# nsirons/DL-unet

Measured on AMD Instinct MI355X. Metric: 572x572 tiles/sec fwd+bwd, higher is better.
Workload: dtype f32; 1 GPU; batch=8/GPU 572x572x1 fwd+bwd+SGD fp32, 64-base-ch U-Net (BASELINE configs[1]); arithmetic=fp32 MFMA; 3x3 fwd/dgrad/wgrad as Winograd F(2x2,3x3), global_batch=8, tile=572, parallelism=dp1, loss=unweighted BCE-with-logits

## Files before the change

dl-unet_amd/_hip.py:

```python
import ctypes as C
import os
import subprocess

import torch

_HERE = os.path.dirname(os.path.abspath(__file__))
_SO = os.environ.get("UNET_SO") or os.path.join(_HERE, "libunet_hip.so")
_lib = None

N_PARAMS = 46
MAX_CLASSES = 16

vp = C.c_void_p
_SIGS = {
    "unet_last_error": (C.c_char_p, []),
    "unet_abi_version": (C.c_int, []),
    "unet_set_math": (C.c_int, [C.c_int]),
    "unet_get_math": (C.c_int, []),
    "unet_set_lds_dma": (C.c_int, [C.c_int]),
    "unet_set_grad_scale": (C.c_int, [vp, C.c_float]),
    "unet_set_overlap": (C.c_int, [C.c_int]),
    "unet_dp_unique_id": (C.c_int, [vp]),
    "unet_dp_init": (C.c_int, [vp, C.c_int, C.c_int, vp]),
    "unet_dp_destroy": (C.c_int, [vp]),
    "unet_dp_world": (C.c_int, [vp]),
    "unet_dp_rccl_version": (C.c_int, []),
    "unet_dp_allreduce": (C.c_int, [vp, vp, C.c_size_t, vp]),
    "unet_dp_broadcast": (C.c_int, [vp, vp, C.c_size_t, C.c_int, vp]),
    "unet_dp_join": (C.c_int, [vp, vp]),
    "unet_create": (C.c_int, [C.POINTER(vp), vp]),
    "unet_create_classes": (C.c_int, [C.POINTER(vp), vp, C.c_int]),
    "unet_n_classes": (C.c_int, [vp]),
    "unet_destroy": (C.c_int, [vp]),
    "unet_output_size": (C.c_int, [C.c_int, C.POINTER(C.c_int)]),
    "unet_param_count": (C.c_int, [vp, C.c_int, C.POINTER(C.c_size_t)]),
    "unet_workspace_bytes": (C.c_size_t, [vp, C.c_int, C.c_int, C.c_int]),
    "unet_forward": (C.c_int, [vp, vp, vp, vp, C.c_int, C.c_int, vp, C.c_size_t, C.c_int, vp]),
    "unet_backward": (C.c_int, [vp, vp, vp, vp, vp, C.c_size_t, vp]),
    "unet_backward_stages": (C.c_int, []),
    "unet_backward_stage": (C.c_int, [vp, C.c_int, vp, vp, vp, vp, C.c_size_t, vp]),
    "unet_backward_stage_params": (C.c_int, [C.c_int, C.POINTER(C.c_int), C.c_int]),
    "unet_backward_input": (C.c_int, [vp, vp, vp, vp, C.c_size_t, vp]),
    "unet_flops": (C.c_double, [vp, C.c_int, C.c_int, C.c_int]),
    "unet_activation_bytes": (C.c_int, [vp]),
    "unet_debug_buffer": (C.c_int, [vp, C.c_int, C.c_int, C.c_int, C.c_char_p, C.POINTER(C.c_size_t), C.POINTER(C.c_int), C.POINTER(C.c_int)]),
    "unet_profile_enable": (C.c_int, [C.c_int]),
    "unet_profile_select": (C.c_int, [C.c_uint]),
    "unet_profile_reset": (C.c_int, []),
    "unet_profile_read": (C.c_int, [C.c_int, C.POINTER(C.c_double), C.POINTER(C.c_long), C.POINTER(C.c_double),
                                    C.POINTER(C.c_double), C.POINTER(C.c_double)]),
    "unet_profile_dump": (C.c_int, [C.c_char_p]),
    "unet_bce_scratch_bytes": (C.c_size_t, [C.c_size_t]),
    "unet_bce_logits": (C.c_int, [vp, vp, vp, C.c_long, C.c_long, C.c_long, C.c_long, C.c_int, C.c_int, C.c_int,
                                  vp, vp, C.c_float, vp, vp]),
    "unet_bce_step_scratch_bytes": (C.c_size_t, [C.c_size_t]),
    "unet_bce_step": (C.c_int, [vp, C.c_long, C.c_long, C.c_long, vp, vp, C.c_long, C.c_long, C.c_long, C.c_long, C.c_int, C.c_int, C.c_int,
                                vp, vp, C.c_float, vp, vp, vp]),
    "unet_onehot2": (C.c_int, [vp, vp, C.c_int, C.c_int, C.c_int, vp]),
    "unet_argmax2": (C.c_int, [vp, C.c_long, C.c_long, C.c_long, vp, C.c_int, C.c_int, C.c_int, vp]),
    "unet_softmax_ce_scratch_bytes": (C.c_size_t, [C.c_size_t]),
    "unet_softmax_ce_step": (C.c_int, [vp, C.c_long, C.c_long, C.c_long, C.c_int, vp, vp, C.c_long, C.c_long, C.c_long, C.c_int, C.c_int,
                                       C.c_int, vp, vp, C.c_float, vp, vp, vp, vp]),
    "unet_argmaxk": (C.c_int, [vp, C.c_long, C.c_long, C.c_long, C.c_int, vp, C.c_int, C.c_int, C.c_int, vp]),
    "unet_sgd_momentum": (C.c_int, [vp, vp, vp, C.POINTER(C.c_size_t), C.c_int, C.c_float, C.c_float, C.c_int, vp]),
    "unet_minmax": (C.c_int, [vp, C.c_int, C.c_size_t, vp, vp]),
    "unet_mirror_pad": (C.c_int, [vp, C.c_int, C.c_int, C.c_int, vp, vp, vp]),
    "unet_tile_gather": (C.c_int, [vp, C.c_int, C.c_int, C.c_int, vp, C.c_int, C.c_int, C.c_int, C.c_int, C.c_int, C.c_long,
                                   C.c_int, vp, vp]),
    "unet_tile_stitch": (C.c_int, [vp, C.c_int, C.c_int, C.c_int, C.c_int, C.c_int, C.c_long, C.c_int, C.c_int, C.c_int, C.c_int,
                                   vp, vp, vp]),
    "unet_tile_stitch_k": (C.c_int, [vp, C.c_int, C.c_int, C.c_int, C.c_int, C.c_int, C.c_int, C.c_long, C.c_int, C.c_int, C.c_int,
                                     C.c_int, vp, vp, vp]),
    "unet_eval_masks": (C.c_int, [vp, C.c_long, C.c_long, C.c_long, C.c_int, vp, vp, C.c_int, C.c_int, vp, vp]),
    "unet_eval_confusion": (C.c_int, [vp, C.c_long, C.c_long, C.c_long, C.c_int, C.c_int, vp, vp, C.c_int, C.c_int, vp, vp, vp]),
    "unet_class_balance": (C.c_int, [vp, C.c_int, C.c_int, C.c_int, vp, vp, vp]),
    "unet_weighted_map_scratch_bytes": (C.c_size_t, [C.c_int, C.c_int, C.c_int]),
    "unet_weighted_map": (C.c_int, [vp, C.c_int, C.c_int, C.c_int, C.c_int, C.c_float, C.c_float, vp, vp, vp, vp, vp]),
    "unet_gaussian_filter": (C.c_int, [vp, C.c_int, C.c_int, C.c_int, vp, C.c_int, C.c_float, vp, vp, vp]),
    "unet_warp_bilinear": (C.c_int, [vp, vp, vp, C.c_int, C.c_int, C.c_int, vp, vp]),
    "unet_rotate_scratch_bytes": (C.c_size_t, [C.c_int, C.c_int]),
    "unet_reflect_rotate_crop": (C.c_int, [vp, C.c_int, C.c_int, C.c_int, C.c_int, C.POINTER(C.c_float), C.c_int, vp, vp, vp]),
    "unet_conv3x3_scratch_bytes": (C.c_size_t, [C.c_int, C.c_int]),
    "unet_conv3x3_fwd": (C.c_int, [vp, C.c_int, C.c_int, C.c_int, C.c_int, vp, C.c_int, C.c_int, C.c_int, C.c_int,
                                   vp, vp, C.c_int, C.c_int, vp, vp, vp]),
    "unet_conv3x3_bwd_scratch_bytes": (C.c_size_t, [C.c_int] * 5),
    "unet_conv3x3_bwd": (C.c_int, [vp, C.c_int, C.c_int, C.c_int, C.c_int, vp, C.c_int, C.c_int, C.c_int, C.c_int,
                                   vp, C.c_int, vp, vp, vp, vp, vp, vp, vp, vp, vp, vp]),
    "unet_maxpool2_fwd": (C.c_int, [vp, vp, C.c_int, C.c_int, C.c_int, C.c_int, vp]),
    "unet_maxpool2_bwd": (C.c_int, [vp, vp, vp, C.c_int, C.c_int, C.c_int, C.c_int, vp]),
    "unet_upconv2_scratch_bytes": (C.c_size_t, [C.c_int] * 5),
    "unet_upconv2_fwd": (C.c_int, [vp, C.c_int, C.c_int, C.c_int, C.c_int, vp, vp, C.c_int, vp, vp, vp]),
    "unet_upconv2_bwd": (C.c_int, [vp, C.c_int, C.c_int, C.c_int, C.c_int, vp, C.c_int, vp, vp, vp, vp, vp, vp, vp]),
    "unet_head1x1_fwd": (C.c_int, [vp, C.c_int, C.c_int, C.c_int, C.c_int, vp, vp, vp, vp]),
    "unet_head1x1_bwd_scratch_bytes": (C.c_size_t, [C.c_int] * 4),
    "unet_head1x1_bwd": (C.c_int, [vp, C.c_int, C.c_int, C.c_int, C.c_int, vp, vp, vp, vp, vp, vp, vp]),
    "unet_head1xk_fwd": (C.c_int, [vp, C.c_int, C.c_int, C.c_int, C.c_int, C.c_int, vp, vp, vp, vp]),
    "unet_head1xk_bwd_scratch_bytes": (C.c_size_t, [C.c_int] * 5),
    "unet_head1xk_bwd": (C.c_int, [vp, C.c_int, C.c_int, C.c_int, C.c_int, C.c_int, vp, vp, vp, vp, vp, vp, vp]),
    "unet_conv1ch_fwd": (C.c_int, [vp, C.c_int, C.c_int, vp, vp, C.c_int, vp, vp]),
    "unet_conv1ch_bwd_scratch_bytes": (C.c_size_t, [C.c_int] * 3),
    "unet_conv1ch_bwd": (C.c_int, [vp, C.c_int, C.c_int, C.c_int, vp, vp, vp, vp, vp]),
}
EXPORTS = tuple(_SIGS.keys())


class UnetConfig(C.Structure):
    _fields_ = [("base_ch", C.c_int), ("device", C.c_int), ("math", C.c_int)]


def build(force=False):
    csrc = os.path.join(_HERE, "csrc")
    if force and os.path.exists(_SO):
        os.remove(_SO)
    subprocess.check_call(["make", "-s", "-C", csrc, "-j4"])
    return _SO


def lib():
    global _lib
    if _lib is None:
        if not os.path.exists(_SO):
            raise RuntimeError(
                "libunet_hip.so is not built (%s). Run `python -c 'import __graft_entry__ as g; g.build()'` "
                "or `make -C dl-unet_amd/csrc`. There is no CPU fallback for the HIP path." % _SO)
        L = C.CDLL(_SO)
        for name, (res, args) in _SIGS.items():
            fn = getattr(L, name)
            fn.restype = res
            fn.argtypes = args
        _lib = L
    return _lib


def check(rc, what=""):
    if rc != 0:
        msg = lib().unet_last_error().decode("utf-8", "replace")
        raise RuntimeError("%s failed (rc=%d): %s" % (what or "libunet_hip", rc, msg))


def ptr(t):
    if t is None:
        return None
    if not t.is_cuda:
        raise RuntimeError("the HIP path needs tensors on a HIP device (got %s); there is no CPU fallback" % t.device)
    return C.c_void_p(t.data_ptr())


def stream(device=None):
    return C.c_void_p(torch.cuda.current_stream(device).cuda_stream)


def run(name, device, *args):
    with torch.cuda.device(device):
        check(getattr(lib(), name)(*args, stream(device)), name)


def ptr_table(tensors):
    arr = (C.c_void_p * len(tensors))()
    for i, t in enumerate(tensors):
        if not t.is_cuda:
            raise RuntimeError("parameter %d is on %s; move the module to a HIP device" % (i, t.device))
        arr[i] = t.data_ptr()
    return arr


class Handle:

    def __init__(self, base_ch=64, device=0, math=-1, n_classes=2):
        self._h = C.c_void_p()
        cfg = UnetConfig(base_ch, device, math)
        if n_classes == 2:
            check(lib().unet_create(C.byref(self._h), C.byref(cfg)), "unet_create")
        else:
            check(lib().unet_create_classes(C.byref(self._h), C.byref(cfg), int(n_classes)), "unet_create_classes")
        self.base_ch = base_ch
        self.device = device
        self.math = math
        self.n_classes = n_classes

    def __del__(self):
        try:
            if self._h:
                lib().unet_destroy(self._h)
                self._h = None
        except Exception:
            pass

    @property
    def h(self):
        return self._h

    def workspace_bytes(self, B, S, training):
        n = lib().unet_workspace_bytes(self._h, B, S, int(training))
        if n == 0:
            check(-1, "unet_workspace_bytes")
        return n

    def buffer_view(self, ws, B, S, training, name):
        off, e, c = C.c_size_t(), C.c_int(), C.c_int()
        check(lib().unet_debug_buffer(self._h, B, S, int(training), name.encode(), C.byref(off), C.byref(e), C.byref(c)),
              "unet_debug_buffer")
        n = B * e.value * e.value * c.value
        eb = 4 if name == "xin" else lib().unet_activation_bytes(self._h)
        return ws[off.value:off.value + eb * n].view(torch.bfloat16 if eb == 2 else torch.float32).view(B, e.value, e.value, c.value)

    def flops(self, B, S, backward):
        return lib().unet_flops(self._h, B, S, int(backward))
```

dl-unet_amd/csrc/common.hpp:

```cpp
#pragma once
#include <hip/hip_runtime.h>
#include <cstddef>
#include <cstdint>

namespace unet {

typedef float f32x4 __attribute__((ext_vector_type(4)));
typedef float f32x16 __attribute__((ext_vector_type(16)));

void set_error(const char *fmt, ...);
const float *zero_page();

#define HIP_TRY(expr)                                                              \
    do {                                                                           \
        hipError_t e_ = (expr);                                                    \
        if (e_ != hipSuccess) {                                                    \
            unet::set_error("%s failed: %s", #expr, hipGetErrorString(e_));        \
            return (int)e_;                                                        \
        }                                                                          \
    } while (0)

#define ARG_CHECK(cond, ...)                                                       \
    do {                                                                           \
        if (!(cond)) { unet::set_error(__VA_ARGS__); return -2; }                  \
    } while (0)

enum { PK_IGEMM = 0, PK_WGRAD = 1, PK_REDUCE = 2, PK_WINO = 3, PK_STENCIL = 4, PK_ELEMWISE = 5, PK_COMM = 6, PK_KINDS = 7 };
void prof_scope(const char *row);
void prof_begin(int kind, const char *tag, hipStream_t st, double alg_flops, double exec_flops, double alg_bytes);
void prof_end(hipStream_t st);
bool prof_active();
struct ProfScope {
    explicit ProfScope(const char *row) { prof_scope(row); }
    ~ProfScope() { prof_scope(nullptr); }
};

template <class F>
static inline int profiled(int kind, const char *tag, hipStream_t st, double alg_flops, double exec_flops, double alg_bytes, F launches)
{
    prof_begin(kind, tag, st, alg_flops, exec_flops, alg_bytes);
    launches();
    prof_end(st);
    HIP_TRY(hipGetLastError());
    return 0;
}
template <auto Kern, class Arg>
static inline int launch_profiled(int grid, int threads, int lds, hipStream_t st, int kind, const char *tag, double alg_flops,
                                  double exec_flops, double alg_bytes, const Arg &arg)
{
    static bool attr_done[64] = {false};
    int dev = 0;
    if (hipGetDevice(&dev) != hipSuccess || dev < 0 || dev >= 64) { set_error("bad device"); return -2; }
    if (!attr_done[dev]) {
        HIP_TRY(hipFuncSetAttribute((const void *)Kern, hipFuncAttributeMaxDynamicSharedMemorySize, lds));
        attr_done[dev] = true;
    }
    return profiled(kind, tag, st, alg_flops, exec_flops, alg_bytes,
                    [&] { hipLaunchKernelGGL(Kern, dim3(grid), dim3(threads), lds, st, arg); });
}
int device_cu_count();

static inline int cdiv(int a, int b) { return (a + b - 1) / b; }
static inline size_t align_up(size_t v, size_t a) { return (v + a - 1) / a * a; }

constexpr size_t LIMIT_31BIT = 0x7FFFFFFFull;
static inline size_t tensor_elems(int NB, int H, int W, int C) { return (size_t)NB * H * W * C; }
static inline size_t tensor_bytes(int NB, int H, int W, int C, size_t es) { return tensor_elems(NB, H, W, C) * es; }
static inline bool fits_buffer(size_t bytes) { return bytes < LIMIT_31BIT; }

struct FastDiv { unsigned long long mul; int shift; };
static inline FastDiv make_fastdiv(unsigned d)
{
    int s = 0;
    while ((1ull << s) < d) ++s;
    FastDiv f;
    f.shift = 32 + s;
    f.mul = ((1ull << f.shift) + d - 1) / d;
    return f;
}

struct GSrc {
    const float *p;
    int H, W, C;
    int c0, nch;
    int pad;
};

struct IgemmP {
    GSrc src[2];
    int nsrc;
    const float *wt;
    int Kd, ldw;
    int T, TX;
    int stride, oy0, ox0;
    int NB, OH, OW, M, Nn;
    float *dst;
    int DH, DW, DC, dn0;
    int scatter;
    int dwy0, dwx0;
    int rw0, rw1;
    int cout;
    const float *bias;
    int relu;
    const float *mask;
    const float *add;
    const float *zeros;
    int buf_bytes[3];
    float *pool_dst;
    const float *wino_u;
    int math;
    int mtiles, ntiles;
    FastDiv d_ohw, d_ow;
};
int launch_igemm(IgemmP p, hipStream_t st);
static inline int igemm_source_bytes(const IgemmP &p, size_t es, int out[2])
{
    int big = -1;
    for (int i = 0; i < 2; ++i) {
        const size_t b = i < p.nsrc ? tensor_bytes(p.NB, p.src[i].H, p.src[i].W, p.src[i].C, es) : 0;
        if (!fits_buffer(b) && big < 0) big = i;
        out[i] = (int)b;
    }
    return big;
}
bool wino_applicable(const IgemmP &p);
bool wino_fuses_pool(const IgemmP &p);
size_t wino_u_floats(int Kc, int Nn);
int wino_transform_ref(const float *w_oihw, int I, int dgrad, int n0, int Nn, int k0, int Kc, float *U, hipStream_t st);
int get_math_mode();
void set_math_mode(int m);
static inline int op_es() { return get_math_mode() == 2 ? 2 : 4; }
int get_lds_dma_mode();
void set_lds_dma_mode(int m);
double igemm_alg_flops(const IgemmP &p);
double igemm_alg_bytes(const IgemmP &p);

struct WgradP {
    const float *X; int XH, XW, XC, xc0, xpad;
    const float *Y; int YH, YW, YC, yc0;
    int NB, stride, TY, TX, oy0, ox0;
    int ywin0, ywin1, xwin0, xwin1;
    int Ci, Cj;
    float *out; long si, sj, st;
    float *db;
    int db_on_x;
    float *slab; size_t slab_bytes;
    const float *zeros;
    int math;
};
size_t wgrad_slab_need(const WgradP &p);
double wgrad_alg_flops(const WgradP &p);
double wgrad_alg_bytes(const WgradP &p);
int launch_wgrad(WgradP p, hipStream_t st);

int pack_conv_fwd(const float *w_oihw, void *wt, int K, int C1, int C2, int es, hipStream_t st);
int pack_conv_dgrad(const float *w_oihw, void *wt, int K, int C, int es, hipStream_t st);
int pack_upconv_fwd(const float *w_iohw, void *wt, int Ci, int Co, int es, hipStream_t st);
int pack_upconv_dgrad(const float *w_iohw, void *wt, int Ci, int Co, int es, hipStream_t st);
int bias_grad(const void *dz, size_t M, int K, float *db, float *scratch, int es, hipStream_t st);
size_t bias_grad_scratch_bytes(size_t M, int K);

int conv1ch_fwd(const float *x, int B, int S, const float *w, const float *bias, int K, void *y, int es, hipStream_t st);
int conv1ch_bwd(const float *x, int B, int S, int K, const void *dz, float *dw, float *db, float *scratch, int es, hipStream_t st);
int conv1ch_dgrad(const void *dz, int B, int S, int K, const float *w, float *dx, int es, hipStream_t st);
int head1x1_fwd(const void *x, int B, int H, int W, int C, const float *w, const float *bias, float *logits, int es, hipStream_t st);
int head1x1_bwd(const void *x, int B, int H, int W, int C, const float *w, const float *dlogits, float dl_scale, void *dz, float *dw,
                float *db, float *scratch, int es, hipStream_t st);
int headk_fwd(const void *x, int B, int H, int W, int C, int K, const float *w, const float *bias, float *logits, int es, hipStream_t st);
int headk_bwd(const void *x, int B, int H, int W, int C, int K, const float *w, const float *dlogits, float dl_scale, void *dz, float *dw,
              float *db, float *scratch, int es, hipStream_t st);
size_t headk_bwd_scratch_bytes(int B, int H, int W, int C, int K);
static inline int class_pad(int K) { return K <= 2 ? 2 : K <= 4 ? 4 : K <= 8 ? 8 : 16; }
#define CLASS_DISPATCH(K, LAUNCH)                                                                                      \
    do {                                                                                                           \
        switch (unet::class_pad(K)) {                                                                              \
        case 2: { constexpr int KP_ = 2; LAUNCH; } break;                                                          \
        case 4: { constexpr int KP_ = 4; LAUNCH; } break;                                                          \
        case 8: { constexpr int KP_ = 8; LAUNCH; } break;                                                          \
        default: { constexpr int KP_ = 16; LAUNCH; } break;                                                        \
        }                                                                                                          \
    } while (0)
int maxpool2_fwd(const void *x, void *y, int B, int H, int W, int C, int es, hipStream_t st);
int maxpool2_bwd(const void *pre, const void *dy, void *dpre, int B, int H, int W, int C, int es, hipStream_t st);

}
```

dl-unet_amd/csrc/net.hip:

```cpp
#include "common.hpp"
#include "../../include/unet_hip.h"

#include <cstdarg>
#include <cstdio>
#include <cstdlib>
#include <cstring>
#include <mutex>
#include <utility>
#include <vector>

namespace unet {

static thread_local char g_err[512] = "";
void set_error(const char *fmt, ...)
{
    va_list ap;
    va_start(ap, fmt);
    vsnprintf(g_err, sizeof(g_err), fmt, ap);
    va_end(ap);
}

static float *g_zero[64] = {nullptr};
static std::mutex g_zero_mu;
const float *zero_page()
{
    int dev = 0;
    if (hipGetDevice(&dev) != hipSuccess || dev < 0 || dev >= 64) { set_error("zero_page: bad device"); return nullptr; }
    std::lock_guard<std::mutex> lk(g_zero_mu);
    if (!g_zero[dev]) {
        float *p = nullptr;
        if (hipMalloc((void **)&p, 4096) != hipSuccess || hipMemset(p, 0, 4096) != hipSuccess) {
            set_error("zero_page: hipMalloc failed");
            return nullptr;
        }
        g_zero[dev] = p;
    }
    return g_zero[dev];
}

enum { K_CONV1, K_CONV, K_CAT, K_UP, K_HEAD };
enum { T_A1, T_A2, T_T, T_U, T_D1, T_D2, N_TENSORS, T_NONE = N_TENSORS };
struct Layer {
    const char *name;
    int kind, level;
    int ci, co;
    int stage;
    int in, out;
};
static const Layer LAYERS[UNET_N_LAYERS] = {
    {"conv11c", K_CONV1, 0, -1, 0, 5, T_NONE, T_A1}, {"conv12c", K_CONV, 0, 0, 0, 5, T_A1, T_A2},
    {"conv21c", K_CONV, 1, 0, 1, 5, T_T, T_A1},      {"conv22c", K_CONV, 1, 1, 1, 5, T_A1, T_A2},
    {"conv31c", K_CONV, 2, 1, 2, 5, T_T, T_A1},      {"conv32c", K_CONV, 2, 2, 2, 5, T_A1, T_A2},
    {"conv41c", K_CONV, 3, 2, 3, 5, T_T, T_A1},      {"conv42c", K_CONV, 3, 3, 3, 5, T_A1, T_A2},
    {"conv51c", K_CONV, 4, 3, 4, 4, T_T, T_A1},      {"conv52c", K_CONV, 4, 4, 4, 4, T_A1, T_A2},
    {"upconv4", K_UP, 3, 4, 3, 3, T_A2, T_U}, {"conv41e", K_CAT, 3, 4, 3, 3, T_T, T_D1}, {"conv42e", K_CONV, 3, 3, 3, 3, T_D1, T_D2},
    {"upconv3", K_UP, 2, 3, 2, 2, T_D2, T_U}, {"conv31e", K_CAT, 2, 3, 2, 2, T_T, T_D1}, {"conv32e", K_CONV, 2, 2, 2, 2, T_D1, T_D2},
    {"upconv2", K_UP, 1, 2, 1, 1, T_D2, T_U}, {"conv21e", K_CAT, 1, 2, 1, 1, T_T, T_D1}, {"conv22e", K_CONV, 1, 1, 1, 1, T_D1, T_D2},
    {"upconv1", K_UP, 0, 1, 0, 0, T_D2, T_U}, {"conv11e", K_CAT, 0, 1, 0, 0, T_T, T_D1}, {"conv12e", K_CONV, 0, 0, 0, 0, T_D1, T_D2},
    {"finalconv", K_HEAD, 0, 0, -1, 0, T_D2, T_NONE}};
enum { C11C = 0, FINAL = UNET_N_LAYERS - 1 };
static const int N_STAGES = 6;
static const struct { const char *name; int levels; } TENSOR_NAME[N_TENSORS] = {{"a1", 5}, {"a2", 5}, {"t", 4}, {"u", 4}, {"d1", 4}, {"d2", 4}};

struct Act { size_t off = 0, g = 0; int e = 0, c = 0; };

struct Plan {
    int B = 0, S = 0, base = 0, So = 0, training = 0;
    int ncls = 2;
    int math = 3;
    int ch[5], pad[4];
    Act a1[5], a2[5], t[4], u[4], d1[4], d2[4];
    size_t g_ts[4];
    size_t wt_fwd[UNET_N_LAYERS], wt_bwd[UNET_N_LAYERS];
    size_t wu_fwd[UNET_N_LAYERS], wu_bwd[UNET_N_LAYERS];
    size_t slab = 0, slab_bytes = 0, small = 0, small_bytes = 0, xin = 0;
    size_t total = 0;
    const Act &act(int tensor, int l) const { const Act *const v[N_TENSORS] = {a1, a2, t, u, d1, d2}; return v[tensor][l]; }
    const Act &in(const Layer &L) const { return act(L.in, L.kind == K_CAT ? L.level : L.ci); }
    const Act &out(const Layer &L) const { return act(L.out, L.level); }
};

}

using namespace unet;

struct unet_dp;
int unet_dp_free(unet_dp *d);

struct unet_handle {
    int base_ch;
    int device;
    int math;
    int n_classes = 2;
    unet_dp *dp = nullptr;
    float grad_scale = 1.f;
    hipStream_t aux = nullptr;
    hipEvent_t ev_fork = nullptr, ev_join = nullptr;
    std::mutex mu;
    std::vector<std::pair<void *, Plan>> live;
    void remember(void *ws, const Plan &pl)
    {
        std::lock_guard<std::mutex> lk(mu);
        for (auto &e : live) if (e.first == ws) { e.second = pl; return; }
        if (live.size() >= 16) live.erase(live.begin());
        live.emplace_back(ws, pl);
    }
    bool lookup(void *ws, Plan &pl)
    {
        std::lock_guard<std::mutex> lk(mu);
        for (auto &e : live) if (e.first == ws) { pl = e.second; return true; }
        return false;
    }
};

unet_dp **unet_handle_dp_slot(unet_handle *h) { return &h->dp; }
int unet_handle_device(const unet_handle *h) { return h->device; }

namespace unet {

static thread_local int t_math = 3;
static thread_local int t_es = 4;
struct MathScope {
    int prev;
    explicit MathScope(int m) : prev(t_math) { t_math = m; t_es = m == 2 ? 2 : 4; }
    ~MathScope() { t_math = prev; t_es = prev == 2 ? 2 : 4; }
};
static inline float *adv(float *p, size_t elems) { return (float *)((char *)p + elems * t_es); }


static int layer_ci(int base, const Layer &L) { return L.ci < 0 ? 1 : base << L.ci; }
static int layer_co(int base, const Layer &L, int ncls) { return L.co < 0 ? ncls : base << L.co; }
static int layer_taps(const Layer &L) { return L.kind == K_UP ? 2 : L.kind == K_HEAD ? 1 : 3; }

static size_t layer_numel(int base, int layer, bool bias, int ncls = 2)
{
    const Layer &L = LAYERS[layer];
    const int k = layer_taps(L);
    return bias ? (size_t)layer_co(base, L, ncls) : (size_t)layer_ci(base, L) * layer_co(base, L, ncls) * k * k;
}

static size_t layer_wino_floats(int base, int layer)
{
    const Layer &L = LAYERS[layer];
    if (L.kind != K_CONV && L.kind != K_CAT) return 0;
    const int ci = layer_ci(base, L), co = layer_co(base, L, 2);
    const size_t fwd = wino_u_floats(ci, co);
    const size_t bwd = L.kind == K_CAT ? 2 * wino_u_floats(co, ci / 2) : wino_u_floats(co, ci);
    return fwd > bwd ? fwd : bwd;
}

struct WLayer {
    const float *w; int O, I;
    bool dgrad;
    float *wt; int C1, C2;
    bool packed = false;
    int ensure_packed(hipStream_t st)
    {
        if (packed) return 0;
        packed = true;
        return dgrad ? pack_conv_dgrad(w, wt, O, I, t_es, st) : pack_conv_fwd(w, wt, O, C1, C2, t_es, st);
    }
};

static int with_wino(IgemmP &p, float *wu, WLayer &L, int n0, int k0, hipStream_t st)
{
    if (p.math != 3 || !wu || !wino_applicable(p)) return L.ensure_packed(st);
    int kc = 0;
    for (int i = 0; i < p.nsrc; ++i) kc += p.src[i].nch;
    int rc = wino_transform_ref(L.w, L.I, L.dgrad ? 1 : 0, n0, p.Nn, k0, kc, wu, st);
    if (rc) return rc;
    p.wino_u = wu;
    return 0;
}

static int check_size(int S)
{
    if (S < 60 + 16 * 8 || (S - 60) % 16 != 0 || ((S - 60) / 16) % 2 != 0) {
        set_error("input size %d is not 16L+60 with L even >= 8: the reference's crop_and_concat/torch.cat "
                  "raises on it (network.py:124-127)", S);
        return UNET_E_BADSIZE;
    }
    return 0;
}

struct RowScope : ProfScope {
    static const char *make(char (&buf)[40], int layer, const char *what) { snprintf(buf, sizeof(buf), "%s.%s", LAYERS[layer].name, what); return buf; }
    char buf[40];
    RowScope(int layer, const char *what) : ProfScope(make(buf, layer, what)) {}
};

static IgemmP conv_fwd_desc(const float *x1, int H1, int W1, int C1, int pad1, const float *x2, int C2,
                            int B, int H, int W, const float *wt, const float *bias, int K, int relu, float *y)
{
    IgemmP p{};
    p.nsrc = x2 ? 2 : 1;
    p.src[0] = GSrc{x1, H1, W1, C1, 0, C1, pad1};
    if (x2) p.src[1] = GSrc{x2, H, W, C2, 0, C2, 0};
    p.wt = wt; p.Kd = 9 * (C1 + C2);
    p.T = 9; p.TX = 3; p.stride = 1; p.oy0 = 0; p.ox0 = 0;
    p.NB = B; p.OH = H - 2; p.OW = W - 2; p.M = B * p.OH * p.OW; p.Nn = K;
    p.dst = y; p.DH = p.OH; p.DW = p.OW; p.DC = K; p.dn0 = 0;
    p.bias = bias; p.relu = relu;
    p.math = t_math;
    return p;
}

static int conv_fwd_launch(const float *x1, int H1, int C1, int pad1, const float *x2, int C2, int B, int H,
                           const float *w_oihw, float *wt, const float *bias, int K, int relu, float *y, hipStream_t st, float *wu = nullptr,
                           float *pool_dst = nullptr, bool *pool_fused = nullptr)
{
    const int Ho = H - 2;
    if (!x2) C2 = 0;
    WLayer L{w_oihw, K, C1 + C2, false, wt, C1, C2};
    int rc;
    int w0 = pad1 - 2; if (w0 < 0) w0 = 0;
    int w1 = pad1 + H1; if (w1 > Ho) w1 = Ho;
    static const double split_thr = [] { const char *e = getenv("UNET_SPLIT_THR"); return e ? atof(e) : 0.85; }();
    const bool split = x2 && pad1 > 0 && t_math != 2 && (double)(w1 - w0) * (w1 - w0) < split_thr * (double)Ho * Ho;
    if (!split) {
        IgemmP p = conv_fwd_desc(x1, H1, H1, C1, pad1, x2, C2, B, H, H, wt, bias, K, relu, y);
        if ((rc = with_wino(p, wu, L, 0, 0, st))) return rc;
        if (pool_dst && p.wino_u && wino_fuses_pool(p)) { p.pool_dst = pool_dst; *pool_fused = true; }
        return launch_igemm(p, st);
    }
    const int ldw = 9 * (C1 + C2);
    IgemmP a = conv_fwd_desc(x2, H, H, C2, 0, nullptr, 0, B, H, H, adv(wt, 9 * C1), bias, K, relu, y);
    a.ldw = ldw;
    if (relu) { a.rw0 = w0; a.rw1 = w1; }
    if ((rc = with_wino(a, wu, L, 0, C1, st))) return rc;
    if ((rc = launch_igemm(a, st))) return rc;
    IgemmP b = conv_fwd_desc(x1, H1, H1, C1, pad1, nullptr, 0, B, H, H, wt, nullptr, K, relu, y);
    b.ldw = ldw;
    b.OH = b.OW = w1 - w0; b.M = B * b.OH * b.OW; b.oy0 = b.ox0 = w0;
    b.scatter = 2; b.dwy0 = b.dwx0 = w0; b.DH = b.DW = Ho;
    b.add = y;
    if ((rc = with_wino(b, wu ? wu + wino_u_floats(C2, K) : nullptr, L, 0, 0, st))) return rc;
    return launch_igemm(b, st);
}

static IgemmP upconv_fwd_desc(const float *x, int B, int H, int W, int Ci, const float *wt, const float *bias, int Co, float *y)
{
    IgemmP u{};
    u.nsrc = 1; u.src[0] = GSrc{x, H, W, Ci, 0, Ci, 0};
    u.wt = wt; u.Kd = Ci;
    u.T = 1; u.TX = 1; u.stride = 1;
    u.NB = B; u.OH = H; u.OW = W; u.M = B * H * W; u.Nn = 4 * Co;
    u.dst = y; u.DH = 2 * H; u.DW = 2 * W; u.DC = Co; u.scatter = 1; u.cout = Co;
    u.bias = bias;
    u.math = t_math;
    return u;
}

static IgemmP upconv_dgrad_desc(const float *dy, int B, int H, int W, int Ci, const float *wt, int Co, float *dx, const float *mask)
{
    IgemmP d{};
    d.nsrc = 1; d.src[0] = GSrc{dy, 2 * H, 2 * W, Co, 0, Co, 0};
    d.wt = wt; d.Kd = 4 * Co;
    d.T = 4; d.TX = 2; d.stride = 2;
    d.NB = B; d.OH = H; d.OW = W; d.M = B * H * W; d.Nn = Ci;
    d.dst = dx; d.DH = H; d.DW = W; d.DC = Ci;
    d.mask = mask;
    d.math = t_math;
    return d;
}

static IgemmP conv_dgrad_desc(const float *dz, int Ho, int Wo, int K, int B, int OHW, int o0,
                              const float *wt_rows, int Nn, float *dx, const float *mask, const float *add)
{
    IgemmP p{};
    p.nsrc = 1;
    p.src[0] = GSrc{dz, Ho, Wo, K, 0, K, 2};
    p.wt = wt_rows; p.Kd = 9 * K;
    p.T = 9; p.TX = 3; p.stride = 1; p.oy0 = o0; p.ox0 = o0;
    p.NB = B; p.OH = OHW; p.OW = OHW; p.M = B * OHW * OHW; p.Nn = Nn;
    p.dst = dx; p.DH = OHW; p.DW = OHW; p.DC = Nn; p.dn0 = 0;
    p.mask = mask; p.add = add;
    p.math = t_math;
    return p;
}

static WgradP conv_wgrad_desc(const float *X, int XH, int XC, int xpad, const float *dz, int Ho, int K, int B,
                              float *dw, int Ctot, int c_off, float *slab, size_t slab_bytes, float *db = nullptr)
{
    WgradP p{};
    p.X = X; p.XH = XH; p.XW = XH; p.XC = XC; p.xc0 = 0; p.xpad = xpad;
    p.Y = dz; p.YH = Ho; p.YW = Ho; p.YC = K; p.yc0 = 0;
    p.NB = B; p.stride = 1; p.TY = 3; p.TX = 3; p.oy0 = 0; p.ox0 = 0;
    int w0 = xpad - 2; if (w0 < 0) w0 = 0;
    int w1 = xpad + XH; if (w1 > Ho) w1 = Ho;
    p.ywin0 = w0; p.ywin1 = w1; p.xwin0 = w0; p.xwin1 = w1;
    p.Ci = XC; p.Cj = K;
    p.out = dw ? dw + (size_t)c_off * 9 : nullptr; p.si = 9; p.sj = (long)Ctot * 9; p.st = 1;
    p.slab = slab; p.slab_bytes = slab_bytes; p.db = db;
    p.math = t_math;
    return p;
}

static WgradP upconv_wgrad_desc(const float *x, int H, int Ci, const float *dy, int Co, int B, float *dw,
                                float *slab, size_t slab_bytes, float *db = nullptr)
{
    WgradP p{};
    p.X = dy; p.XH = 2 * H; p.XW = 2 * H; p.XC = Co; p.xc0 = 0; p.xpad = 0;
    p.Y = x; p.YH = H; p.YW = H; p.YC = Ci; p.yc0 = 0;
    p.NB = B; p.stride = 2; p.TY = 2; p.TX = 2; p.oy0 = 0; p.ox0 = 0;
    p.ywin0 = 0; p.ywin1 = H; p.xwin0 = 0; p.xwin1 = H;
    p.Ci = Co; p.Cj = Ci;
    p.out = dw; p.si = 4; p.sj = (long)Co * 4; p.st = 1;
    p.slab = slab; p.slab_bytes = slab_bytes;
    p.db = db; p.db_on_x = db ? 1 : 0;
    p.math = t_math;
    return p;
}

static int conv_dgrad_launch(const float *dz, int Ho, int K, int B, const float *w_oihw, float *wt, float *wu, int H1, int C1, int pad1,
                             float *dx1, const float *mask1, const float *add1, int H, int C2, float *dx2, const float *mask2, hipStream_t st)
{
    WLayer L{w_oihw, K, C1 + C2, true, wt, 0, 0};
    int rc;
    if (dx1) {
        IgemmP d = conv_dgrad_desc(dz, Ho, Ho, K, B, H1, pad1, L.wt, C1, dx1, mask1, add1);
        if ((rc = with_wino(d, wu, L, 0, 0, st))) return rc;
        if ((rc = launch_igemm(d, st))) return rc;
    }
    if (dx2) {
        IgemmP d = conv_dgrad_desc(dz, Ho, Ho, K, B, H, 0, adv(L.wt, (size_t)C1 * 9 * K), C2, dx2, mask2, nullptr);
        if ((rc = with_wino(d, wu + wino_u_floats(K, C1), L, C1, 0, st))) return rc;
        if ((rc = launch_igemm(d, st))) return rc;
    }
    return 0;
}

struct WgradStream {
    unet_handle *h; hipStream_t main; bool overlap; bool used;
    hipError_t err = hipSuccess;
    hipStream_t get()
    {
        if (!overlap) return main;
        hipError_t e = hipEventRecord(h->ev_fork, main);
        if (e == hipSuccess) e = hipStreamWaitEvent(h->aux, h->ev_fork, 0);
        if (e != hipSuccess) { if (err == hipSuccess) err = e; overlap = false; return main; }
        used = true;
        return h->aux;
    }
    hipStream_t same() const { return overlap && used ? h->aux : main; }
    void join()
    {
        if (!used) return;
        hipError_t e = hipEventRecord(h->ev_join, h->aux);
        if (e == hipSuccess) e = hipStreamWaitEvent(main, h->ev_join, 0);
        if (e != hipSuccess) {
            (void)hipStreamSynchronize(h->aux);
            if (err == hipSuccess) err = e;
        }
        used = false;
    }
};

struct Ctx {
    unet_handle *h; const Plan &pl; char *base; hipStream_t st;
    const void *const *params; void *const *grads;
    WgradStream wst;
    Ctx(unet_handle *h, const Plan &pl, void *workspace, void *stream, const void *const *params, void *const *grads, bool overlap = false)
        : h(h), pl(pl), base((char *)workspace), st((hipStream_t)stream), params(params), grads(grads), wst{h, st, overlap, false} {}
    float *ws(size_t off) const { return base ? (float *)(base + off) : nullptr; }
    const float *w(int layer) const { return params ? (const float *)params[2 * layer] : nullptr; }
    const float *b(int layer) const { return params ? (const float *)params[2 * layer + 1] : nullptr; }
    float *dw(int layer) const { return grads ? (float *)grads[2 * layer] : nullptr; }
    float *db(int layer) const { return grads ? (float *)grads[2 * layer + 1] : nullptr; }
};

static int layer_wgrad(const Ctx &cx, int layer, WgradP w[2])
{
    const Plan &pl = cx.pl;
    const Layer &L = LAYERS[layer];
    if (L.kind == K_CONV1 || L.kind == K_HEAD) return 0;
    const Act &x = pl.in(L), &y = pl.out(L);
    const float *dz = cx.ws(y.g);
    float *dw = cx.dw(layer), *db = cx.db(layer), *slab = cx.ws(pl.slab);
    if (L.kind == K_UP) w[0] = upconv_wgrad_desc(cx.ws(x.off), x.e, x.c, dz, y.c, pl.B, dw, slab, pl.slab_bytes, db);
    if (L.kind == K_CONV) w[0] = conv_wgrad_desc(cx.ws(x.off), x.e, x.c, 0, dz, y.e, y.c, pl.B, dw, x.c, 0, slab, pl.slab_bytes, db);
    if (L.kind != K_CAT) return 1;
    const Act &u = pl.u[L.level];
    w[0] = conv_wgrad_desc(cx.ws(x.off), x.e, x.c, pl.pad[L.level], dz, y.e, y.c, pl.B, dw, x.c + u.c, 0, slab, pl.slab_bytes);
    w[1] = conv_wgrad_desc(cx.ws(u.off), u.e, u.c, 0, dz, y.e, y.c, pl.B, dw, x.c + u.c, x.c, slab, pl.slab_bytes, db);
    return 2;
}

static int make_plan(Plan &pl, int base, int B, int S, int training, int math, int ncls = 2)
{
    int rc = check_size(S);
    if (rc) return rc;
    if (B <= 0) { set_error("batch must be positive"); return UNET_E_BADARG; }
    pl = Plan();
    pl.B = B; pl.S = S; pl.base = base; pl.training = training; pl.math = math; pl.ncls = ncls;
    MathScope ms(math);
    for (int l = 0; l < 5; ++l) pl.ch[l] = base << l;
    Act *acts[26];
    int n = 0, cur = S;
    for (int l = 0; l < 5; ++l) {
        pl.a1[l].e = cur - 2; pl.a2[l].e = cur - 4;
        pl.a1[l].c = pl.a2[l].c = pl.ch[l];
        acts[n++] = &pl.a1[l]; acts[n++] = &pl.a2[l];
        if (l < 4) cur = pl.a2[l].e / 2;
    }
    int d = pl.a2[4].e;
    for (int l = 3; l >= 0; --l) {
        pl.t[l].e = pl.a2[l].e / 2;
        pl.u[l].e = 2 * d; pl.pad[l] = (pl.u[l].e - pl.t[l].e) / 2;
        if ((pl.u[l].e - pl.t[l].e) % 2) { set_error("internal: odd skip difference"); return UNET_E_BADSIZE; }
        pl.d1[l].e = pl.u[l].e - 2; pl.d2[l].e = pl.u[l].e - 4; d = pl.d2[l].e;
        pl.t[l].c = pl.u[l].c = pl.d1[l].c = pl.d2[l].c = pl.ch[l];
    }
    for (int l = 0; l < 4; ++l) { acts[n++] = &pl.t[l]; acts[n++] = &pl.u[l]; acts[n++] = &pl.d1[l]; acts[n++] = &pl.d2[l]; }
    pl.So = d;
    if (math == 2 && base % 64 != 0) { set_error("arithmetic mode 2 (bf16 tensors) needs base_ch %% 64 == 0 (got %d)", base); return UNET_E_UNSUPPORTED; }
    const size_t es = math == 2 ? 2 : 4;
    size_t off = 0;
    auto take_b = [&](size_t bytes) { size_t o = off; off = align_up(off + bytes, 256); return o; };
    auto take = [&](size_t elems) { return take_b(elems * es); };
    auto sq = [&](int e, int c) { return (size_t)B * e * e * c; };
    for (int i = 0; i < n; ++i) acts[i]->off = take(sq(acts[i]->e, acts[i]->c));
    for (int i = 0; i < UNET_N_LAYERS; ++i) pl.wt_fwd[i] = take(layer_numel(base, i, false, ncls));
    for (int i = 0; i < UNET_N_LAYERS; ++i) pl.wu_fwd[i] = take_b(math == 3 ? layer_wino_floats(base, i) * 4 : 0);
    if (training) {
        pl.xin = take_b((size_t)B * S * S * 4);
        for (int i = 0; i < UNET_N_LAYERS; ++i) pl.wt_bwd[i] = take(layer_numel(base, i, false, ncls));
        for (int i = 0; i < UNET_N_LAYERS; ++i) pl.wu_bwd[i] = take_b(math == 3 ? layer_wino_floats(base, i) * 4 : 0);
        for (int i = 0; i < n; ++i) {
            Act *a = acts[i];
            a->g = take(sq(a->e, a->c));
            if (a >= pl.t && a < pl.t + 4) pl.g_ts[a - pl.t] = take(sq(a->e, a->c));
        }
        size_t need = 0;
        const Ctx sizing(nullptr, pl, nullptr, nullptr, nullptr, nullptr);
        for (int i = 0; i < UNET_N_LAYERS; ++i) {
            WgradP w[2];
            const int nw = layer_wgrad(sizing, i, w);
            for (int j = 0; j < nw; ++j) { const size_t s = wgrad_slab_need(w[j]); if (s > need) need = s; }
        }
        pl.slab_bytes = need;
        pl.slab = take_b(need);
        size_t sm = 0;
        auto upds = [&](size_t s) { if (s > sm) sm = s; };
        for (int l = 0; l < 5; ++l) { upds(bias_grad_scratch_bytes(sq(pl.a1[l].e, 1), pl.ch[l])); upds(bias_grad_scratch_bytes(sq(pl.a2[l].e, 1), pl.ch[l])); }
        for (int l = 0; l < 4; ++l) { upds(bias_grad_scratch_bytes(sq(pl.u[l].e, 1), pl.ch[l])); upds(bias_grad_scratch_bytes(sq(pl.d1[l].e, 1), pl.ch[l])); }
        upds(unet_conv1ch_bwd_scratch_bytes(B, S, base));
        upds(headk_bwd_scratch_bytes(B, pl.So, pl.So, base, ncls));
        pl.small_bytes = sm;
        pl.small = take_b(sm + 4);
    }
    pl.total = off;
    return 0;
}

}

extern "C" {

const char *unet_last_error(void) { return g_err; }
int unet_abi_version(void) { return 4; }

int unet_set_math(int mode)
{
    ARG_CHECK(mode >= 0 && mode <= 3, "unet_set_math: mode must be 0 (fp32 MFMA), 1 (bf16x3), 2 (bf16) or 3 (fp32 Winograd)");
    set_math_mode(mode);
    return 0;
}
int unet_get_math(void) { return get_math_mode(); }

int unet_set_lds_dma(int mode)
{
    ARG_CHECK(mode == 0 || mode == 1, "unet_set_lds_dma: mode must be 0 (global_load_lds) or 1 (buffer descriptors when tensors fit)");
    set_lds_dma_mode(mode);
    return 0;
}

#define CHECK_DEVICE(h, what)                                                                                          \
    do {                                                                                                               \
        int cur_ = -1;                                                                                                 \
        HIP_TRY(hipGetDevice(&cur_));                                                                                  \
        ARG_CHECK(cur_ == (h)->device, what ": the handle belongs to device %d but device %d is current "               \
                  "(one process per GPU: hipSetDevice / torch.cuda.set_device first)", (h)->device, cur_);             \
    } while (0)

int unet_create(unet_handle **out, const unet_config *cfg) { return unet_create_classes(out, cfg, 2); }

int unet_create_classes(unet_handle **out, const unet_config *cfg, int n_classes)
{
    ARG_CHECK(out && cfg, "unet_create: null argument");
    ARG_CHECK(n_classes >= 2 && n_classes <= UNET_MAX_CLASSES, "unet_create_classes: n_classes %d unsupported (2..%d)", n_classes,
              UNET_MAX_CLASSES);
    ARG_CHECK(cfg->base_ch == 64 || cfg->base_ch == 32, "unet_create: base_ch %d unsupported (32 or 64)", cfg->base_ch);
    ARG_CHECK(cfg->math >= -1 && cfg->math <= 3, "unet_create: math %d unsupported (-1 = process default, 0..3)", cfg->math);
    int prev = -1;
    HIP_TRY(hipGetDevice(&prev));
    HIP_TRY(hipSetDevice(cfg->device));
    const bool ok = zero_page() != nullptr;
    HIP_TRY(hipSetDevice(prev));
    if (!ok) return UNET_E_BADARG;
    unet_handle *h = new unet_handle();
    h->base_ch = cfg->base_ch;
    h->device = cfg->device;
    h->math = cfg->math;
    h->n_classes = n_classes;
    *out = h;
    return 0;
}

int unet_n_classes(const unet_handle *h) { return h ? h->n_classes : 0; }

int unet_destroy(unet_handle *h)
{
    if (h && h->dp) (void)unet_dp_free(h->dp);
    if (h) {
        if (h->aux) { (void)hipStreamSynchronize(h->aux); (void)hipStreamDestroy(h->aux); }
        if (h->ev_fork) (void)hipEventDestroy(h->ev_fork);
        if (h->ev_join) (void)hipEventDestroy(h->ev_join);
    }
    delete h;
    return 0;
}

int unet_set_grad_scale(unet_handle *h, float scale)
{
    ARG_CHECK(h, "unet_set_grad_scale: null handle");
    ARG_CHECK(scale > 0.f && scale <= 1.f, "unet_set_grad_scale: scale must be in (0, 1] (1/world), got %g", (double)scale);
    h->grad_scale = scale;
    return 0;
}

static int g_overlap = [] { const char *e = getenv("UNET_OVERLAP"); return e ? atoi(e) : -1; }();
int unet_set_overlap(int on)
{
    ARG_CHECK(on >= -1 && on <= 1, "unet_set_overlap: -1 (per arithmetic mode), 0 or 1");
    g_overlap = on;
    return 0;
}

static int handle_math(const unet_handle *h) { return h->math >= 0 ? h->math : get_math_mode(); }

int unet_output_size(int S, int *out_size)
{
    int rc = check_size(S);
    if (rc) return rc;
    if (out_size) *out_size = S - 184;
    return 0;
}

int unet_param_count(const unet_handle *h, int idx, size_t *numel)
{
    ARG_CHECK(h && numel && idx >= 0 && idx < UNET_N_PARAMS, "unet_param_count: bad argument");
    *numel = layer_numel(h->base_ch, idx / 2, idx & 1, h->n_classes);
    return 0;
}

size_t unet_workspace_bytes(const unet_handle *h, int B, int S, int training)
{
    if (!h) { set_error("null handle"); return 0; }
    Plan pl;
    if (make_plan(pl, h->base_ch, B, S, training, handle_math(h), h->n_classes)) return 0;
    return pl.total;
}

double unet_flops(const unet_handle *h, int B, int S, int backward)
{
    if (!h) return 0.0;
    Plan pl;
    if (make_plan(pl, h->base_ch, B, S, 0, handle_math(h), h->n_classes)) return 0.0;
    double f = 0.0, f11c = 0.0, first = 0.0;
    for (int i = 0; i < UNET_N_LAYERS; ++i) {
        const Layer &L = LAYERS[i];
        const int k = layer_taps(L);
        const int eo = L.kind == K_UP || L.kind == K_HEAD ? pl.in(L).e : pl.out(L).e;
        const double a = 2.0 * B * (double)eo * eo * layer_ci(pl.base, L) * layer_co(pl.base, L, pl.ncls) * k * k;
        if (L.kind == K_CONV1) f11c = a;
        if (L.out == T_A1 || L.out == T_D1) first = a;
        else if (L.out == T_A2 || L.out == T_D2) f += first + a;
        else f += a;
    }
    return backward ? 3.0 * f - f11c : f;
}

static int pool_launch(const Ctx &cx, int l, bool bwd)
{
    char nm[40]; snprintf(nm, sizeof(nm), "pool%d.%s", l + 1, bwd ? "bwd" : "fwd");
    ProfScope ps(nm);
    const Act &a2 = cx.pl.a2[l], &t = cx.pl.t[l];
    return bwd ? maxpool2_bwd(cx.ws(a2.off), cx.ws(t.g), cx.ws(a2.g), cx.pl.B, a2.e, a2.e, a2.c, t_es, cx.st)
               : maxpool2_fwd(cx.ws(a2.off), cx.ws(t.off), cx.pl.B, a2.e, a2.e, a2.c, t_es, cx.st);
}

static int conv_forward(const Ctx &cx, int layer)
{
    const Plan &pl = cx.pl;
    const Layer &L = LAYERS[layer];
    const bool cat = L.kind == K_CAT, pools = L.out == T_A2 && L.level < 4;
    const Act &x1 = pl.in(L), &y = pl.out(L), *x2 = cat ? &pl.u[L.level] : nullptr;
    bool pool_fused = false;
    {
        RowScope rs(layer, "fwd");
        int rc = conv_fwd_launch(cx.ws(x1.off), x1.e, x1.c, cat ? pl.pad[L.level] : 0, cat ? cx.ws(x2->off) : nullptr, cat ? x2->c : 0, pl.B, y.e + 2,
                                 cx.w(layer), cx.ws(pl.wt_fwd[layer]), cx.b(layer), y.c, 1, cx.ws(y.off), cx.st, cx.ws(pl.wu_fwd[layer]),
                                 pools ? cx.ws(pl.t[L.level].off) : nullptr, &pool_fused);
        if (rc) return rc;
    }
    return pools && !pool_fused ? pool_launch(cx, L.level, false) : 0;
}

int unet_forward(unet_handle *h, const void *const *params, const void *x, void *logits, int B, int S,
                 void *workspace, size_t workspace_bytes, int training, void *stream)
{
    ARG_CHECK(h && params && x && logits && workspace, "unet_forward: null argument");
    CHECK_DEVICE(h, "unet_forward");
    Plan pl;
    int rc = make_plan(pl, h->base_ch, B, S, training, handle_math(h), h->n_classes);
    if (rc) return rc;
    MathScope ms(pl.math);
    ARG_CHECK(workspace_bytes >= pl.total, "unet_forward: workspace too small (%zu < %zu)", workspace_bytes, pl.total);
    ARG_CHECK(((uintptr_t)workspace & 255) == 0, "unet_forward: workspace must be 256-byte aligned");
    const Ctx cx(h, pl, workspace, stream, params, nullptr);
    hipStream_t st = cx.st;

    for (int i = UNET_N_LAYERS - 1; i >= 0; --i) {
        if (LAYERS[i].kind != K_UP) continue;
        RowScope rs(i, "fwd");
        if ((rc = pack_upconv_fwd(cx.w(i), cx.ws(pl.wt_fwd[i]), pl.ch[LAYERS[i].ci], pl.ch[LAYERS[i].co], t_es, st))) return rc;
    }

    for (int i = 0; i < UNET_N_LAYERS; ++i) {
        const Layer &L = LAYERS[i];
        switch (L.kind) {
        case K_CONV1: {
            RowScope rs(i, "fwd");
            if (training) HIP_TRY(hipMemcpyAsync(cx.ws(pl.xin), x, (size_t)B * S * S * sizeof(float), hipMemcpyDeviceToDevice, st));
            if ((rc = conv1ch_fwd((const float *)x, B, S, cx.w(i), cx.b(i), pl.ch[0], cx.ws(pl.a1[0].off), t_es, st))) return rc;
            break;
        }
        case K_CONV:
        case K_CAT:
            if ((rc = conv_forward(cx, i))) return rc;
            break;
        case K_UP: {
            RowScope rs(i, "fwd");
            const Act &in = pl.in(L), &u = pl.u[L.level];
            IgemmP p = upconv_fwd_desc(cx.ws(in.off), B, in.e, in.e, in.c, cx.ws(pl.wt_fwd[i]), cx.b(i), u.c, cx.ws(u.off));
            if ((rc = launch_igemm(p, st))) return rc;
            break;
        }
        case K_HEAD: {
            RowScope rs(i, "fwd");
            const Act &in = pl.in(L);
            if ((rc = headk_fwd(cx.ws(in.off), B, in.e, in.e, in.c, pl.ncls, cx.w(i), cx.b(i), (float *)logits, t_es, st))) return rc;
            break;
        }
        }
    }
    if (training) h->remember(workspace, pl);
    return 0;
}

int unet_activation_bytes(const unet_handle *h)
{
    if (!h) return 0;
    return handle_math(h) == 2 ? 2 : 4;
}

int unet_debug_buffer(const unet_handle *h, int B, int S, int training, const char *name,
                      size_t *offset, int *extent, int *channels)
{
    ARG_CHECK(h && name && offset && extent && channels, "unet_debug_buffer: null argument");
    Plan pl;
    int rc = make_plan(pl, h->base_ch, B, S, training, handle_math(h), h->n_classes);
    if (rc) return rc;
    char kind[16];
    const char *us = strrchr(name, '_');
    if (!strcmp(name, "xin")) { ARG_CHECK(training, "xin exists only with training=1"); *offset = pl.xin; *extent = S; *channels = 1; return 0; }
    ARG_CHECK(us && (size_t)(us - name) < sizeof(kind), "unet_debug_buffer: bad name %s", name);
    memcpy(kind, name, us - name); kind[us - name] = 0;
    const int l = atoi(us + 1);
    ARG_CHECK(l >= 0 && l < 5, "unet_debug_buffer: bad level in %s", name);
    const bool g = !strncmp(kind, "g_", 2);
    ARG_CHECK(!g || training, "gradient buffers exist only with training=1");
    const char *k = g ? kind + 2 : kind;
    const bool ts = g && !strcmp(k, "ts");
    int id = ts ? T_T : 0;
    while (!ts && id < N_TENSORS && strcmp(k, TENSOR_NAME[id].name)) ++id;
    ARG_CHECK(l < (id < N_TENSORS ? TENSOR_NAME[id].levels : 4), "unet_debug_buffer: bad level in %s", name);
    if (id == N_TENSORS) { set_error("unet_debug_buffer: unknown buffer %s", name); return UNET_E_BADARG; }
    const Act &a = pl.act(id, l);
    *offset = ts ? pl.g_ts[l] : g ? a.g : a.off; *extent = a.e; *channels = a.c;
    return 0;
}

int unet_backward_stages(void) { return N_STAGES; }

int unet_backward_stage_params(int stage, int *idx, int cap)
{
    int k = 0;
    for (int i = UNET_N_LAYERS - 1; i >= 0; --i)
        for (int b = 0; b < 2 && LAYERS[i].stage == stage; ++b, ++k)
            if (idx && k < cap) idx[k] = 2 * i + b;
    return k;
}

static int wgrad_backward(Ctx &cx, int layer)
{
    RowScope rs(layer, "wgrad");
    WgradP w[2];
    const int n = layer_wgrad(cx, layer, w);
    for (int j = 0; j < n; ++j) {
        int rc = launch_wgrad(w[j], j ? cx.wst.same() : cx.wst.get());
        if (rc) return rc;
    }
    return 0;
}

static int conv_backward(Ctx &cx, int layer)
{
    const Plan &pl = cx.pl;
    const Layer &L = LAYERS[layer];
    const Act &x = pl.in(L), &y = pl.out(L);
    const bool pooled = L.in == T_T;
    int rc;
    if ((rc = wgrad_backward(cx, layer))) return rc;
    {
        RowScope rs(layer, "dgrad");
        if ((rc = conv_dgrad_launch(cx.ws(y.g), y.e, y.c, pl.B, cx.w(layer), cx.ws(pl.wt_bwd[layer]), cx.ws(pl.wu_bwd[layer]), x.e, x.c, 0, cx.ws(x.g),
                                    pooled ? nullptr : cx.ws(x.off), pooled ? cx.ws(pl.g_ts[L.ci]) : nullptr, 0, 0, nullptr, nullptr, cx.st))) return rc;
    }
    return pooled ? pool_launch(cx, L.ci, true) : 0;
}

static int backward_stage_body(Ctx &cx, int stage, const void *dlogits)
{
    const Plan &pl = cx.pl;
    hipStream_t st = cx.st;
    const int B = pl.B;
    int rc;
    for (int i = UNET_N_LAYERS - 1; i >= 0; --i) {
        const Layer &L = LAYERS[i];
        if (L.stage != stage) continue;
        switch (L.kind) {
        case K_HEAD: {
            ARG_CHECK(dlogits, "unet_backward: null dlogits");
            RowScope rs(i, "bwd");
            const Act &x = pl.in(L);
            if ((rc = headk_bwd(cx.ws(x.off), B, x.e, x.e, x.c, pl.ncls, cx.w(i), (const float *)dlogits, cx.h->grad_scale, cx.ws(x.g),
                                cx.dw(i), cx.db(i), cx.ws(pl.small), t_es, st))) return rc;
            break;
        }
        case K_CONV:
            if ((rc = conv_backward(cx, i))) return rc;
            break;
        case K_CAT: {
            const int l = L.level;
            const Act &t = pl.t[l], &u = pl.u[l], &y = pl.d1[l];
            if ((rc = wgrad_backward(cx, i))) return rc;
            RowScope rs(i, "dgrad");
            if ((rc = conv_dgrad_launch(cx.ws(y.g), y.e, y.c, B, cx.w(i), cx.ws(pl.wt_bwd[i]), cx.ws(pl.wu_bwd[i]), t.e, t.c, pl.pad[l], cx.ws(pl.g_ts[l]), nullptr, nullptr,
                                        u.e, u.c, cx.ws(u.g), nullptr, st))) return rc;
            break;
        }
        case K_UP: {
            const Act &x = pl.in(L), &u = pl.u[L.level];
            if ((rc = wgrad_backward(cx, i))) return rc;
            RowScope rs(i, "dgrad");
            if ((rc = pack_upconv_dgrad(cx.w(i), cx.ws(pl.wt_bwd[i]), x.c, u.c, t_es, st))) return rc;
            IgemmP d = upconv_dgrad_desc(cx.ws(u.g), B, x.e, x.e, x.c, cx.ws(pl.wt_bwd[i]), u.c, cx.ws(x.g), cx.ws(x.off));
            if ((rc = launch_igemm(d, st))) return rc;
            break;
        }
        case K_CONV1: {
            RowScope rs(i, "wgrad");
            if ((rc = conv1ch_bwd(cx.ws(pl.xin), B, pl.S, pl.ch[0], cx.ws(pl.a1[0].g), cx.dw(i), cx.db(i), cx.ws(pl.small), t_es, st))) return rc;
            break;
        }
        }
    }
    return 0;
}

int unet_backward_stage(unet_handle *h, int stage, const void *const *params, const void *dlogits, void *const *grads,
                        void *workspace, size_t workspace_bytes, void *stream)
{
    ARG_CHECK(h && params && grads && workspace, "unet_backward: null argument");
    CHECK_DEVICE(h, "unet_backward");
    Plan pl;
    if (!h->lookup(workspace, pl)) {
        set_error("unet_backward: no training forward has been run on this workspace");
        return UNET_E_NOTREADY;
    }
    ARG_CHECK(workspace_bytes >= pl.total, "unet_backward: workspace too small");
    ARG_CHECK(stage >= 0 && stage < N_STAGES, "unet_backward: bad stage %d", stage);
    MathScope ms(pl.math);
    const bool overlap = (g_overlap < 0 ? (pl.math == 2 || pl.B <= 4) : g_overlap != 0) && !prof_active();
    if (overlap && !h->aux) {
        HIP_TRY(hipStreamCreateWithFlags(&h->aux, hipStreamNonBlocking));
        HIP_TRY(hipEventCreateWithFlags(&h->ev_fork, hipEventDisableTiming));
        HIP_TRY(hipEventCreateWithFlags(&h->ev_join, hipEventDisableTiming));
    }
    Ctx cx(h, pl, workspace, stream, params, grads, overlap);
    int rc = backward_stage_body(cx, stage, dlogits);
    cx.wst.join();
    if (rc == 0 && cx.wst.err != hipSuccess) {
        set_error("unet_backward: ordering the weight-gradient stream against the caller's failed: %s", hipGetErrorString(cx.wst.err));
        rc = (int)cx.wst.err;
    }
    return rc;
}

int unet_backward_input(unet_handle *h, const void *const *params, void *dx, void *workspace, size_t workspace_bytes, void *stream)
{
    ARG_CHECK(h && params && dx && workspace, "unet_backward_input: null argument");
    CHECK_DEVICE(h, "unet_backward_input");
    Plan pl;
    if (!h->lookup(workspace, pl)) {
        set_error("unet_backward_input: no training forward has been run on this workspace");
        return UNET_E_NOTREADY;
    }
    ARG_CHECK(workspace_bytes >= pl.total, "unet_backward_input: workspace too small");
    MathScope ms(pl.math);
    const Ctx cx(h, pl, workspace, stream, params, nullptr);
    RowScope rs(C11C, "dgrad");
    return conv1ch_dgrad(cx.ws(pl.a1[0].g), pl.B, pl.S, pl.ch[0], cx.w(C11C), (float *)dx, t_es, cx.st);
}

int unet_backward(unet_handle *h, const void *const *params, const void *dlogits, void *const *grads,
                  void *workspace, size_t workspace_bytes, void *stream)
{
    for (int s = 0; s < N_STAGES; ++s) {
        int rc = unet_backward_stage(h, s, params, dlogits, grads, workspace, workspace_bytes, stream);
        if (rc) return rc;
    }
    return 0;
}

static size_t conv_bwd_slab_bound(int B, int H, int C, int K)
{
    size_t need = 0;
    for (int math = 0; math <= 2; math += 2) {
        MathScope ms(math);
        for (int ci = 64; ci <= (C + 63) / 64 * 64; ci *= 2) {
            WgradP w = conv_wgrad_desc(nullptr, H, ci, 0, nullptr, H - 2, K, B, nullptr, ci, 0, nullptr, 0);
            const size_t n = wgrad_slab_need(w);
            if (n > need) need = n;
        }
    }
    return align_up(2 * need, 256);
}

static size_t upconv_slab_bound(int B, int H, int Ci, int Co)
{
    size_t need = 0;
    for (int math = 0; math <= 2; math += 2) {
        MathScope ms(math);
        WgradP w = upconv_wgrad_desc(nullptr, H, Ci, nullptr, Co, B, nullptr, nullptr, 0);
        const size_t n = wgrad_slab_need(w);
        if (n > need) need = n;
    }
    return align_up(need, 256);
}

static size_t wino_scratch_bytes(int C, int K)
{
    const size_t fwd = wino_u_floats(C, K), bwd = wino_u_floats(K, C) + wino_u_floats(K, 64);
    return align_up((fwd > bwd ? fwd : bwd) * sizeof(float), 256);
}
size_t unet_conv3x3_scratch_bytes(int C, int K) { return align_up((size_t)K * C * 9 * sizeof(float), 256) + wino_scratch_bytes(C, K); }

int unet_conv3x3_fwd(const void *x1, int H1, int W1, int C1, int pad1, const void *x2, int C2, int B, int H, int W,
                     const void *w_oihw, const void *bias, int K, int relu, void *y, void *scratch, void *stream)
{
    ARG_CHECK(x1 && w_oihw && y && scratch, "conv3x3_fwd: null argument");
    MathScope ms(get_math_mode());
    ProfScope ps("op.conv3x3_fwd");
    ARG_CHECK(x2 || (H1 + 2 * pad1 == H && W1 + 2 * pad1 == W), "conv3x3_fwd: single source must match the input extent");
    hipStream_t st = (hipStream_t)stream;
    ARG_CHECK(H == W && H1 == W1, "conv3x3_fwd: square tiles only");
    float *wu = (float *)((char *)scratch + align_up((size_t)K * (C1 + (x2 ? C2 : 0)) * 9 * sizeof(float), 256));
    return conv_fwd_launch((const float *)x1, H1, C1, pad1, (const float *)x2, C2, B, H, (const float *)w_oihw, (float *)scratch,
                           (const float *)bias, K, relu, (float *)y, st, wu);
}

size_t unet_conv3x3_bwd_scratch_bytes(int B, int H, int W, int C, int K)
{
    return align_up((size_t)K * C * 9 * sizeof(float), 256) + conv_bwd_slab_bound(B, H, C, K) +
           align_up(bias_grad_scratch_bytes((size_t)B * (H - 2) * (W - 2), K), 256) + wino_scratch_bytes(C, K);
}

int unet_conv3x3_bwd(const void *x1, int H1, int W1, int C1, int pad1, const void *x2, int C2, int B, int H, int W,
                     const void *w_oihw, int K, const void *dz, void *dx1, const void *mask1, const void *add1,
                     void *dx2, const void *mask2, void *dw, void *db, void *scratch, void *stream)
{
    ARG_CHECK(x1 && w_oihw && dz && scratch, "conv3x3_bwd: null argument");
    MathScope ms(get_math_mode());
    ProfScope ps("op.conv3x3_bwd");
    ARG_CHECK(H == W && H1 == W1, "conv3x3_bwd: square tiles only");
    hipStream_t st = (hipStream_t)stream;
    const int C = C1 + (x2 ? C2 : 0);
    const int Ho = H - 2;
    float *wt = (float *)scratch;
    const size_t wt_bytes = align_up((size_t)K * C * 9 * sizeof(float), 256);
    const size_t slab_bytes = conv_bwd_slab_bound(B, H, C, K);
    float *slab = (float *)((char *)scratch + wt_bytes);
    float *small = (float *)((char *)scratch + wt_bytes + slab_bytes);
    float *wu = (float *)((char *)scratch + wt_bytes + slab_bytes + align_up(bias_grad_scratch_bytes((size_t)B * Ho * Ho, K), 256));
    int rc;
    if ((rc = conv_dgrad_launch((const float *)dz, Ho, K, B, (const float *)w_oihw, wt, wu, H1, C1, pad1, (float *)dx1, (const float *)mask1,
                                (const float *)add1, H, C - C1, x2 ? (float *)dx2 : nullptr, (const float *)mask2, st))) return rc;
    bool db_done = false;
    if (dw) {
        const bool full1 = !x2 && pad1 == 0;
        WgradP w1 = conv_wgrad_desc((const float *)x1, H1, C1, pad1, (const float *)dz, Ho, K, B, (float *)dw, C, 0, slab, slab_bytes,
                                    full1 ? (float *)db : nullptr);
        if ((rc = launch_wgrad(w1, st))) return rc;
        db_done = full1 && db;
        if (x2) {
            WgradP w2 = conv_wgrad_desc((const float *)x2, H, C2, 0, (const float *)dz, Ho, K, B, (float *)dw, C, C1, slab, slab_bytes, (float *)db);
            if ((rc = launch_wgrad(w2, st))) return rc;
            db_done = db != nullptr;
        }
    }
    if (db && !db_done && (rc = bias_grad(dz, (size_t)B * Ho * Ho, K, (float *)db, small, t_es, st))) return rc;
    return 0;
}

size_t unet_upconv2_scratch_bytes(int B, int H, int W, int Ci, int Co)
{
    (void)W;
    return align_up((size_t)Ci * Co * 4 * sizeof(float), 256) + upconv_slab_bound(B, H, Ci, Co) +
           align_up(bias_grad_scratch_bytes((size_t)B * 4 * H * W, Co), 256);
}

int unet_upconv2_fwd(const void *x, int B, int H, int W, int Ci, const void *w_iohw, const void *bias, int Co,
                     void *y, void *scratch, void *stream)
{
    ARG_CHECK(x && w_iohw && y && scratch, "upconv2_fwd: null argument");
    MathScope ms(get_math_mode());
    ProfScope ps("op.upconv2_fwd");
    hipStream_t st = (hipStream_t)stream;
    int rc = pack_upconv_fwd((const float *)w_iohw, scratch, Ci, Co, t_es, st);
    if (rc) return rc;
    return launch_igemm(upconv_fwd_desc((const float *)x, B, H, W, Ci, (const float *)scratch, (const float *)bias, Co, (float *)y), st);
}

int unet_upconv2_bwd(const void *x, int B, int H, int W, int Ci, const void *w_iohw, int Co, const void *dy,
                     void *dx, const void *mask, void *dw, void *db, void *scratch, void *stream)
{
    ARG_CHECK(x && w_iohw && dy && scratch, "upconv2_bwd: null argument");
    ARG_CHECK(H == W, "upconv2_bwd: square tiles only");
    MathScope ms(get_math_mode());
    ProfScope ps("op.upconv2_bwd");
    hipStream_t st = (hipStream_t)stream;
    float *wt = (float *)scratch;
    const size_t wt_bytes = align_up((size_t)Ci * Co * 4 * sizeof(float), 256);
    const size_t slab_bytes = upconv_slab_bound(B, H, Ci, Co);
    float *slab = (float *)((char *)scratch + wt_bytes);
    float *small = (float *)((char *)scratch + wt_bytes + slab_bytes);
    int rc;
    if (dx) {
        if ((rc = pack_upconv_dgrad((const float *)w_iohw, wt, Ci, Co, t_es, st))) return rc;
        if ((rc = launch_igemm(upconv_dgrad_desc((const float *)dy, B, H, W, Ci, wt, Co, (float *)dx, (const float *)mask), st))) return rc;
    }
    if (dw) {
        WgradP w = upconv_wgrad_desc((const float *)x, H, Ci, (const float *)dy, Co, B, (float *)dw, slab, slab_bytes, (float *)db);
        if ((rc = launch_wgrad(w, st))) return rc;
    } else if (db && (rc = bias_grad(dy, (size_t)B * 4 * H * W, Co, (float *)db, small, t_es, st))) return rc;
    return 0;
}

}
```

dl-unet_amd/csrc/wgrad.hip:

```cpp
#include "kernel_parts.hpp"
#include <array>
#include <cstdio>
#include <cstdlib>
#include <map>
#include <mutex>
#include <type_traits>

namespace unet {

bool wgradw_applicable(const WgradP &p);
size_t wgradw_slab_need(const WgradP &p);
int launch_wgradw(const WgradP &p, hipStream_t st);

constexpr int PWMAX = 32;

struct WgradK {
    WgradP p;
    int pw, nstrips, rows_per_chunk, nchunks, ntile_i, ntile_j;
    int xbytes, ybytes;
    int ci_real, cj_real;
    int nparts, ngroups;
    size_t pstride;
    int up_npix, up_nchunks, up_per;
    FastDiv d_yw;
};

template <int TY, int TX, int S>
struct WgradGeom {
    static constexpr int T = TY * TX;
    static constexpr int XPX = ((PWMAX - 1) * S + TX + 3) / 4 * 4;
    static constexpr int XGROUPS = XPX / 4;
    static constexpr int YGROUPS = PWMAX / 4;
    static constexpr int RING = 4;
    static constexpr int XSLOT = XPX * 256;
    static constexpr int YBUF = PWMAX * 256;
    static constexpr int LDS = RING * XSLOT + 2 * YBUF;
    static constexpr int NI = (S * XGROUPS + YGROUPS + 3) / 4;
    static_assert(TY + S <= RING, "ring too small");
};

template <int TY, int TX, int S, int NSPLIT, bool BUF>
__global__ __launch_bounds__(256, ((TY * TX == 9 && NSPLIT == 0) ? 3 : 2)) void wgrad_f32_kernel(const WgradK k)
{
    using G = WgradGeom<TY, TX, S>;
    constexpr int T = G::T;
    extern __shared__ __attribute__((aligned(16))) unsigned char smem[];
    unsigned char *xs = smem;
    unsigned char *ys = smem + G::RING * G::XSLOT;
    const WgradP &p = k.p;

    const int tid = threadIdx.x, lane = tid & 63;
    const int wave = __builtin_amdgcn_readfirstlane(tid >> 6);
    const int wi = wave >> 1, wj = wave & 1;

    const int logical = xcd_slot();
    const int ntile = k.ntile_i * k.ntile_j;
    const int grp = logical / ntile;
    const int tile = logical - grp * ntile;
    const int it = tile / k.ntile_j, jt = tile - it * k.ntile_j;

    const int l15 = lane & 15, lq = lane >> 4;
    const float *zsrc = p.zeros + 4 * l15;

    f32x16 acc[T];
#pragma unroll
    for (int t = 0; t < T; ++t)
#pragma unroll
        for (int r = 0; r < 16; ++r) acc[t][r] = 0.f;
    const bool do_bias = p.db != nullptr && !p.db_on_x && it == 0;
    const bool do_xbias = p.db != nullptr && p.db_on_x && jt == 0;
    float bsum = 0.f;
    const int bch = tid & 63, bpg = tid >> 6;

    const int l31 = lane & 31, lh = lane >> 5;
    const int a_lane = (wi * 32 + l31) * 4;
    const int b_lane = (wj * 32 + l31) * 4;
    const __amdgpu_buffer_rsrc_t rs_x = make_rsrc(p.X, BUF ? k.xbytes : 0);
    const __amdgpu_buffer_rsrc_t rs_y = make_rsrc(p.Y, BUF ? k.ybytes : 0);

    for (int P = grp; P < k.nparts; P += k.ngroups) {
    const int strip = P % k.nstrips;
    const int pc = P / k.nstrips;
    const int chunk = pc % k.nchunks;
    const int img = pc / k.nchunks;
    const int x0 = p.xwin0 + strip * k.pw;
    int pwv = p.xwin1 - x0; pwv = pwv < k.pw ? pwv : k.pw;
    const int ya = p.ywin0 + chunk * k.rows_per_chunk;
    int yb = ya + k.rows_per_chunk; yb = yb < p.ywin1 ? yb : p.ywin1;
    const int npairs = (pwv + 1) >> 1;
    const int xcol0 = (x0 + p.ox0) * S - p.xpad;

    auto stage_x = [&](int xr, int g) {
        const int px = 4 * g + lq;
        const int xc = xcol0 + px;
        const bool ok = (unsigned)xr < (unsigned)p.XH && (unsigned)xc < (unsigned)p.XW && it * 64 + 4 * l15 < k.ci_real;
        const float *src = p.X + ((size_t)((img * p.XH + xr) * p.XW + xc) * p.XC + p.xc0 + it * 64 + 4 * l15);
        GLDS16(ok ? src : zsrc, xs + (xr & (G::RING - 1)) * G::XSLOT + g * 1024);
    };
    auto stage_y = [&](int y, int buf, int g) {
        const int px = 4 * g + lq;
        const bool ok = px < pwv && jt * 64 + 4 * l15 < k.cj_real;
        const float *src = p.Y + ((size_t)((img * p.YH + y) * p.YW + x0 + px) * p.YC + p.yc0 + jt * 64 + 4 * l15);
        GLDS16(ok ? src : zsrc, ys + buf * G::YBUF + g * 1024);
    };
    auto stage_step = [&](int y, int buf, int first_row, int nrows) {
        const int xr_base = (y + p.oy0) * S - p.xpad;
        const int nx = nrows * G::XGROUPS;
        for (int e = wave; e < nx + G::YGROUPS; e += 4) {
            if (e < nx) {
                const int rr = e / G::XGROUPS;
                stage_x(xr_base + first_row + rr, e - rr * G::XGROUPS);
            } else {
                stage_y(y, buf, e - nx);
            }
        }
    };

    int iv[G::NI], il[G::NI], irr[G::NI];
    if (BUF) {
#pragma unroll
        for (int i = 0; i < G::NI; ++i) {
            const int e = wave + 4 * i;
            iv[i] = LDS_DMA_OOB; il[i] = 0; irr[i] = -1;
            if (e < S * G::XGROUPS) {
                const int rr = (S == 2 && e >= G::XGROUPS) ? 1 : 0;
                const int g = e - rr * G::XGROUPS;
                const int xc = xcol0 + 4 * g + lq;
                const bool ok = (unsigned)xc < (unsigned)p.XW && it * 64 + 4 * l15 < k.ci_real;
                iv[i] = ok ? (xc * p.XC + p.xc0 + it * 64 + 4 * l15) * 4 : LDS_DMA_OOB;
                il[i] = g * 1024; irr[i] = rr;
            } else if (e < S * G::XGROUPS + G::YGROUPS) {
                const int g = e - S * G::XGROUPS;
                const int px = 4 * g + lq;
                const bool ok = px < pwv && jt * 64 + 4 * l15 < k.cj_real;
                iv[i] = ok ? ((x0 + px) * p.YC + p.yc0 + jt * 64 + 4 * l15) * 4 : LDS_DMA_OOB;
                il[i] = g * 1024;
            }
        }
    }
    auto stage_fast = [&](int y, int buf) {
        const int xr_base = (y + p.oy0) * S - p.xpad + (TY - S);
        const int ysoff = ((img * p.YH + y) * p.YW) * p.YC * 4;
#pragma unroll
        for (int i = 0; i < G::NI; ++i) {
            if (wave + 4 * i < S * G::XGROUPS + G::YGROUPS) {
                if (irr[i] >= 0) {
                    const int xr = xr_base + irr[i];
                    const bool rok = (unsigned)xr < (unsigned)p.XH;
                    lds_dma16(rs_x, xs + (xr & (G::RING - 1)) * G::XSLOT + il[i], rok ? iv[i] : LDS_DMA_OOB, rok ? ((img * p.XH + xr) * p.XW) * p.XC * 4 : 0);
                } else {
                    lds_dma16(rs_y, ys + buf * G::YBUF + il[i], iv[i], ysoff);
                }
            }
        }
    };

    if (ya < yb) {
        stage_step(ya, 0, 0, TY);
        __syncthreads();
        for (int y = ya; y < yb; ++y) {
            const int cur = (y - ya) & 1;
            if (y + 1 < yb) {
                if (BUF) stage_fast(y + 1, cur ^ 1); else stage_step(y + 1, cur ^ 1, TY - S, S);
            }
            const int xr0 = (y + p.oy0) * S - p.xpad;
            if (do_bias) {
                const float *yb_ = (const float *)(ys + cur * G::YBUF) + bch;
                for (int px = bpg; px < pwv; px += 4) bsum += yb_[px * 64];
            }
            if (do_xbias) {
                for (int r = 0; r < S; ++r) {
                    const float *xb_ = (const float *)(xs + ((xr0 + TY - S + r) & (G::RING - 1)) * G::XSLOT) + bch;
                    for (int px = bpg; px < S * pwv; px += 4) bsum += xb_[px * 64];
                }
            }
            const unsigned char *yrow = ys + cur * G::YBUF + b_lane;
            if constexpr (NSPLIT == 0) {
            for (int q = 0; q < npairs; ++q) {
                const int pix = 2 * q + lh;
                const float b = *(const float *)(yrow + pix * 256);
#pragma unroll
                for (int ty = 0; ty < TY; ++ty) {
                    const unsigned char *xrow = xs + ((xr0 + ty) & (G::RING - 1)) * G::XSLOT + a_lane;
#pragma unroll
                    for (int tx = 0; tx < TX; ++tx) {
                        const float a = *(const float *)(xrow + (pix * S + tx) * 256);
                        acc[ty * TX + tx] = __builtin_amdgcn_mfma_f32_32x32x2f32(a, b, acc[ty * TX + tx], 0, 0, 0);
                    }
                }
            }
            } else {
                for (int g16 = 0; g16 * 16 < pwv; ++g16) {
                    const int pix0 = g16 * 16 + 8 * lh;
                    float yv[8];
#pragma unroll
                    for (int j = 0; j < 8; ++j) yv[j] = *(const float *)(yrow + (pix0 + j) * 256);
                    bf16x8 bh, bl;
#pragma unroll
                    for (int j = 0; j < 8; ++j) { bh[j] = (__bf16)yv[j]; if (NSPLIT == 3) bl[j] = (__bf16)(yv[j] - (float)bh[j]); }
#pragma unroll
                    for (int ty = 0; ty < TY; ++ty) {
                        const unsigned char *xrow = xs + ((xr0 + ty) & (G::RING - 1)) * G::XSLOT + a_lane;
                        constexpr int NV = 7 * S + TX;
                        float xv[NV];
                        __bf16 xh[NV], xl[NV];
#pragma unroll
                        for (int j = 0; j < NV; ++j) {
                            xv[j] = *(const float *)(xrow + (pix0 * S + j) * 256);
                            xh[j] = (__bf16)xv[j];
                            if (NSPLIT == 3) xl[j] = (__bf16)(xv[j] - (float)xh[j]);
                        }
#pragma unroll
                        for (int tx = 0; tx < TX; ++tx) {
                            bf16x8 ah, al;
#pragma unroll
                            for (int j = 0; j < 8; ++j) { ah[j] = xh[j * S + tx]; if (NSPLIT == 3) al[j] = xl[j * S + tx]; }
                            const int t = ty * TX + tx;
                            if (NSPLIT == 3) {
                                acc[t] = __builtin_amdgcn_mfma_f32_32x32x16_bf16(al, bh, acc[t], 0, 0, 0);
                                acc[t] = __builtin_amdgcn_mfma_f32_32x32x16_bf16(ah, bl, acc[t], 0, 0, 0);
                            }
                            acc[t] = __builtin_amdgcn_mfma_f32_32x32x16_bf16(ah, bh, acc[t], 0, 0, 0);
                        }
                    }
                }
            }
            __syncthreads();
        }
    }

    }

    float *slab = p.slab + (size_t)grp * k.pstride;
    if (do_bias || do_xbias) {
        float *red = (float *)smem;
        red[tid] = bsum;
        __syncthreads();
        if (tid < 64) slab[(size_t)T * p.Ci * p.Cj + (do_xbias ? it : jt) * 64 + tid] = (red[tid] + red[tid + 64]) + (red[tid + 128] + red[tid + 192]);
    }
    f32x4 *dst4 = (f32x4 *)(slab + ((size_t)(tile * 4 + wave) * T) * 1024) + lane;
#pragma unroll
    for (int t = 0; t < T; ++t)
#pragma unroll
        for (int rq = 0; rq < 4; ++rq)
            dst4[(t * 4 + rq) * 64] = f32x4{acc[t][4 * rq], acc[t][4 * rq + 1], acc[t][4 * rq + 2], acc[t][4 * rq + 3]};
}

constexpr int PWB = 64;
template <int TY, int TX, int S>
struct WgradBGeom {
    static constexpr int T = TY * TX;
    static constexpr int XPX = (PWB + TX - 1 + 7) / 8 * 8;
    static constexpr int XG = XPX / 8, YG = PWB / 8;
    static constexpr int RING = TY + S, NY = 2;
    static constexpr int XSLOT = XPX * 128, YBUF = PWB * 128;
    static constexpr int LDS = RING * XSLOT + NY * YBUF;
    static constexpr int NI = (S * XG + YG + 3) / 4;
    static_assert(2 * LDS <= 160 * 1024, "two workgroups per CU");
    static_assert(S == 1, "stride-1 layers only: the up-conv weight gradient is wgrad_up_kernel");
};

typedef short s16x4 __attribute__((ext_vector_type(4)));
__device__ __forceinline__ bf16x8 tr_frag(const unsigned char *p0)
{
    const s16x4 lo = __builtin_amdgcn_ds_read_tr16_b64_v4i16((__attribute__((address_space(3))) s16x4 *)(p0));
    const s16x4 hi = __builtin_amdgcn_ds_read_tr16_b64_v4i16((__attribute__((address_space(3))) s16x4 *)(p0 + 4 * 128));
    return __builtin_bit_cast(bf16x8, __builtin_shufflevector(lo, hi, 0, 1, 2, 3, 4, 5, 6, 7));
}
__device__ __forceinline__ float frag_sum(const bf16x8 &v)
{
    float s = 0.f;
#pragma unroll
    for (int j = 0; j < 8; ++j) s += (float)v[j];
    return s;
}

template <int TY, int TX, int S>
__global__ __launch_bounds__(256, 2) void wgrad_bf16_kernel(const WgradK k)
{
    using G = WgradBGeom<TY, TX, S>;
    constexpr int T = G::T;
    extern __shared__ __attribute__((aligned(16))) unsigned char smem[];
    unsigned char *xs = smem;
    unsigned char *ys = smem + G::RING * G::XSLOT;
    const WgradP &p = k.p;

    const int tid = threadIdx.x, lane = tid & 63;
    const int wave = __builtin_amdgcn_readfirstlane(tid >> 6);
    const int wi = wave >> 1, wj = wave & 1;

    const int logical = xcd_slot();
    const int ntile = k.ntile_i * k.ntile_j;
    const int grp = logical / ntile;
    const int tile = logical - grp * ntile;
    const int it = tile / k.ntile_j, jt = tile - it * k.ntile_j;

    f32x16 acc[T];
#pragma unroll
    for (int t = 0; t < T; ++t)
#pragma unroll
        for (int r = 0; r < 16; ++r) acc[t][r] = 0.f;
    const bool do_bias = p.db != nullptr && !p.db_on_x && it == 0 && wi == 0;
    const bool do_xbias = p.db != nullptr && p.db_on_x && jt == 0 && wj == 0;
    float bsum = 0.f;

    const int d_px = lane >> 3;
    const int d_c = (lane & 7) ^ (((lane >> 4) & 1) << 2);
    const int f_q = (lane >> 2) & 3, f_pp = lane & 3, f_mh = (lane >> 4) & 1, f_h = lane >> 5;
    const int cA = wi * 4 + f_mh * 2 + (f_pp >> 1), cB = wj * 4 + f_mh * 2 + (f_pp >> 1);
    const int yoff = (8 * f_h + f_q) * 128 + ((cB ^ (((f_q >> 1) & 1) << 2)) * 16) + (f_pp & 1) * 8;
    int xoff[TX];
#pragma unroll
    for (int tx = 0; tx < TX; ++tx) {
        xoff[tx] = (8 * f_h + f_q + tx) * 128 + ((cA ^ ((((f_q + tx) >> 1) & 1) << 2)) * 16) + (f_pp & 1) * 8;
    }

    const __amdgpu_buffer_rsrc_t rs_x = make_rsrc(p.X, k.xbytes);
    const __amdgpu_buffer_rsrc_t rs_y = make_rsrc(p.Y, k.ybytes);

    auto run = [&](auto role_tag) {
    constexpr int ROLE = decltype(role_tag)::value;
    for (int P = grp; P < k.nparts; P += k.ngroups) {
    const int strip = P % k.nstrips;
    const int pc = P / k.nstrips;
    const int chunk = pc % k.nchunks;
    const int img = pc / k.nchunks;
    const int x0 = p.xwin0 + strip * k.pw;
    int pwv = p.xwin1 - x0; pwv = pwv < k.pw ? pwv : k.pw;
    const int ya = p.ywin0 + chunk * k.rows_per_chunk;
    int yb = ya + k.rows_per_chunk; yb = yb < p.ywin1 ? yb : p.ywin1;
    const int nks = (pwv + 15) >> 4;
    const int xcol0 = (x0 + p.ox0) * S - p.xpad;

    auto stage_x = [&](int xr, int slot, int g) {
        const int pos = 8 * g + d_px;
        const int xc = xcol0 + pos;
        const bool ok = (unsigned)xr < (unsigned)p.XH && (unsigned)xc < (unsigned)p.XW;
        const int off = (((img * p.XH + xr) * p.XW + xc) * p.XC + p.xc0 + it * 64 + d_c * 8) * 2;
        lds_dma16(rs_x, xs + slot * G::XSLOT + g * 1024, ok ? off : LDS_DMA_OOB, 0);
    };
    auto stage_y = [&](int y, int buf, int g) {
        const int px = 8 * g + d_px;
        const bool ok = px < pwv;
        const int off = (((img * p.YH + y) * p.YW + x0 + px) * p.YC + p.yc0 + jt * 64 + d_c * 8) * 2;
        lds_dma16(rs_y, ys + buf * G::YBUF + g * 1024, ok ? off : LDS_DMA_OOB, 0);
    };
    const int xg_used = (16 * nks + TX - 1 + 7) >> 3;
    const int yg_used = 2 * nks;
    auto stage_step = [&](int y, int j, int first_row, int nrows) {
        const int xr_base = (y + p.oy0) * S - p.xpad;
        const int nx = nrows * xg_used;
        const int buf = j % G::NY;
        for (int e = wave; e < nx + yg_used; e += 4) {
            if (e < nx) {
                const int rr = e / xg_used;
                stage_x(xr_base + first_row + rr, (j * S + first_row + rr) % G::RING, e - rr * xg_used);
            } else {
                stage_y(y, buf, e - nx);
            }
        }
    };
    const int n_items = S * xg_used + yg_used;
    int iv[G::NI], il[G::NI], irr[G::NI];
#pragma unroll
    for (int i = 0; i < G::NI; ++i) {
        const int e = wave + 4 * i;
        iv[i] = LDS_DMA_OOB; il[i] = 0; irr[i] = -1;
        if (e < S * xg_used) {
            const int rr = 0;
            const int g = e;
            const int pos = 8 * g + d_px;
            const int xc = xcol0 + pos;
            const bool ok = (unsigned)xc < (unsigned)p.XW;
            iv[i] = ok ? (xc * p.XC + p.xc0 + it * 64 + d_c * 8) * 2 : LDS_DMA_OOB;
            il[i] = g * 1024; irr[i] = rr;
        } else if (e < n_items) {
            const int g = e - S * xg_used;
            const int px = 8 * g + d_px;
            iv[i] = px < pwv ? ((x0 + px) * p.YC + p.yc0 + jt * 64 + d_c * 8) * 2 : LDS_DMA_OOB;
            il[i] = g * 1024;
        }
    }
    auto stage_fast = [&](int y, int j) {
        const int xr_base = (y + p.oy0) * S - p.xpad + (TY - S);
        unsigned char *yb_ = ys + (j % G::NY) * G::YBUF;
        const int ysoff = ((img * p.YH + y) * p.YW) * p.YC * 2;
#pragma unroll
        for (int i = 0; i < G::NI; ++i) {
            if (wave + 4 * i < n_items) {
                if (irr[i] >= 0) {
                    const int xr = xr_base + irr[i];
                    const bool rok = (unsigned)xr < (unsigned)p.XH;
                    unsigned char *dst = xs + ((j * S + (TY - S) + irr[i]) % G::RING) * G::XSLOT + il[i];
                    lds_dma16(rs_x, dst, rok ? iv[i] : LDS_DMA_OOB, rok ? ((img * p.XH + xr) * p.XW) * p.XC * 2 : 0);
                } else {
                    lds_dma16(rs_y, yb_ + il[i], iv[i], ysoff);
                }
            }
        }
    };

    if (ya < yb) {
        stage_step(ya, 0, 0, TY);
        __syncthreads();
        for (int y = ya, j = 0; y < yb; ++y, ++j) {
            if (y + 1 < yb) stage_fast(y + 1, j + 1);
            const unsigned char *yrow = ys + (j % G::NY) * G::YBUF + yoff;
            const unsigned char *xrow[TY];
#pragma unroll
            for (int ty = 0; ty < TY; ++ty) xrow[ty] = xs + ((j * S + ty) % G::RING) * G::XSLOT;
            {
                bf16x8 a[T], b;
                b = tr_frag(yrow);
#pragma unroll
                for (int ty = 0; ty < TY; ++ty)
#pragma unroll
                    for (int tx = 0; tx < TX; ++tx) a[ty * TX + tx] = tr_frag(xrow[ty] + xoff[tx]);
                for (int ks = 0; ks < nks; ++ks) {
                    const int kn = (ks + 1 < nks ? ks + 1 : ks) * (16 * 128);
                    const bf16x8 bn = tr_frag(yrow + kn);
                    if (ROLE == 1) bsum += frag_sum(b);
#pragma unroll
                    for (int ty = 0; ty < TY; ++ty)
#pragma unroll
                        for (int tx = 0; tx < TX; ++tx) {
                            const int t = ty * TX + tx;
                            if (ROLE == 2) bsum += frag_sum(a[t]);
                            acc[t] = __builtin_amdgcn_mfma_f32_32x32x16_bf16(a[t], b, acc[t], 0, 0, 0);
                            a[t] = tr_frag(xrow[ty] + kn + xoff[tx]);
                            __builtin_amdgcn_sched_barrier(0);
                        }
                    b = bn;
                }
            }
            __syncthreads();
        }
    }

    }
    };
    if (do_xbias) run(std::integral_constant<int, 2>{});
    else if (do_bias) run(std::integral_constant<int, 1>{});
    else run(std::integral_constant<int, 0>{});

    float *slab = p.slab + (size_t)grp * k.pstride;
    if (do_bias || do_xbias) {
        const float v = bsum + __shfl_xor(bsum, 32, 64);
        if (lane < 32) slab[(size_t)T * p.Ci * p.Cj + (do_xbias ? it * 64 + wi * 32 : jt * 64 + wj * 32) + lane] = v;
    }
    f32x4 *dst4 = (f32x4 *)(slab + ((size_t)(tile * 4 + wave) * T) * 1024) + lane;
#pragma unroll
    for (int t = 0; t < T; ++t)
#pragma unroll
        for (int rq = 0; rq < 4; ++rq)
            dst4[(t * 4 + rq) * 64] = f32x4{acc[t][4 * rq], acc[t][4 * rq + 1], acc[t][4 * rq + 2], acc[t][4 * rq + 3]};
}

template <bool BF>
struct UpGeom {
    static constexpr int ES = BF ? 2 : 4;
    static constexpr int PIX = BF ? 64 : 32;
    static constexpr int ROWB = 64 * ES;
    static constexpr int IMG = PIX * ROWB;
    static constexpr int STAGE = 5 * IMG;
    static constexpr int LDS = 2 * STAGE;
    static constexpr int PPI = 1024 / ROWB;
    static constexpr int NG = PIX / PPI;
    static_assert(NG == 8, "a wave stages pixel groups w and w + 4 of all five images");
};

template <bool BF>
__global__ __launch_bounds__(256, 2) void wgrad_up_kernel(const WgradK k)
{
    using G = UpGeom<BF>;
    constexpr int T = 4, ES = G::ES;
    extern __shared__ __attribute__((aligned(16))) unsigned char smem[];
    const WgradP &p = k.p;

    const int tid = threadIdx.x, lane = tid & 63;
    const int wave = __builtin_amdgcn_readfirstlane(tid >> 6);
    const int wi = wave >> 1, wj = wave & 1;

    const int logical = xcd_slot();
    const int ntile = k.ntile_i * k.ntile_j;
    const int grp = logical / ntile;
    const int tile = logical - grp * ntile;
    const int it = tile / k.ntile_j, jt = tile - it * k.ntile_j;

    f32x16 acc[T];
#pragma unroll
    for (int t = 0; t < T; ++t)
#pragma unroll
        for (int r = 0; r < 16; ++r) acc[t][r] = 0.f;
    const bool do_xbias = p.db != nullptr && jt == 0 && (BF ? wj == 0 : true);
    float bsum = 0.f;

    const int d_px = BF ? lane >> 3 : lane >> 4;
    const int d_ch = BF ? (((lane & 7) ^ (((lane >> 4) & 1) << 2)) * 8) : 4 * (lane & 15);
    const bool x_ch_ok = it * 64 + d_ch < k.ci_real, y_ch_ok = jt * 64 + d_ch < k.cj_real;
    const int x_lane = (p.xc0 + it * 64 + d_ch) * ES, y_lane = (p.yc0 + jt * 64 + d_ch) * ES;
    const __amdgpu_buffer_rsrc_t rs_x = make_rsrc(p.X, k.xbytes);
    const __amdgpu_buffer_rsrc_t rs_y = make_rsrc(p.Y, k.ybytes);
    const int YW = p.YW;
    int tap_off[T];
#pragma unroll
    for (int t = 0; t < T; ++t) tap_off[t] = ((t >> 1) * p.XW + (t & 1)) * p.XC * ES;

    auto stage = [&](int c, int buf) {
        unsigned char *sb = smem + buf * G::STAGE;
#pragma unroll
        for (int gg = 0; gg < 2; ++gg) {
            const int g = wave + 4 * gg;
            const int pix = c * G::PIX + g * G::PPI + d_px;
            const bool ok = pix < k.up_npix;
            const int r = fdiv(pix, k.d_yw);
            const int x = pix - r * YW;
            const int xo = ok && x_ch_ok ? ((4 * r * YW + 2 * x) * p.XC) * ES + x_lane : LDS_DMA_OOB;
            const int yo = ok && y_ch_ok ? pix * p.YC * ES + y_lane : LDS_DMA_OOB;
#pragma unroll
            for (int t = 0; t < T; ++t) lds_dma16(rs_x, sb + t * G::IMG + g * 1024, xo, tap_off[t]);
            lds_dma16(rs_y, sb + 4 * G::IMG + g * 1024, yo, 0);
        }
    };

    const int c0 = grp * k.up_per;
    int c1 = c0 + k.up_per;
    c1 = c1 < k.up_nchunks ? c1 : k.up_nchunks;

    if constexpr (BF) {
        const int f_q = (lane >> 2) & 3, f_pp = lane & 3, f_mh = (lane >> 4) & 1, f_h = lane >> 5;
        const int cA = wi * 4 + f_mh * 2 + (f_pp >> 1), cB = wj * 4 + f_mh * 2 + (f_pp >> 1);
        const int sw = ((f_q >> 1) & 1) << 2;
        const int xoff = (8 * f_h + f_q) * 128 + ((cA ^ sw) * 16) + (f_pp & 1) * 8;
        const int yoff = 4 * G::IMG + (8 * f_h + f_q) * 128 + ((cB ^ sw) * 16) + (f_pp & 1) * 8;
        if (c0 < c1) {
            stage(c0, 0);
            __syncthreads();
            for (int c = c0; c < c1; ++c) {
                const int cur = (c - c0) & 1;
                if (c + 1 < c1) stage(c + 1, cur ^ 1);
                const unsigned char *sb = smem + cur * G::STAGE;
                bf16x8 a[T], b;
                b = tr_frag(sb + yoff);
#pragma unroll
                for (int t = 0; t < T; ++t) a[t] = tr_frag(sb + t * G::IMG + xoff);
#pragma unroll
                for (int ks = 0; ks < 4; ++ks) {
                    const int kn = (ks + 1 < 4 ? ks + 1 : ks) * (16 * 128);
                    const bf16x8 bn = tr_frag(sb + yoff + kn);
#pragma unroll
                    for (int t = 0; t < T; ++t) {
                        if (do_xbias) bsum += frag_sum(a[t]);
                        acc[t] = __builtin_amdgcn_mfma_f32_32x32x16_bf16(a[t], b, acc[t], 0, 0, 0);
                        a[t] = tr_frag(sb + t * G::IMG + xoff + kn);
                        __builtin_amdgcn_sched_barrier(0);
                    }
                    b = bn;
                }
                __syncthreads();
            }
        }
    } else {
        const int l31 = lane & 31, lh = lane >> 5;
        const int a_lane = (wi * 32 + l31) * 4, b_lane = 4 * G::IMG + (wj * 32 + l31) * 4;
        const int bch = tid & 63, bpg = tid >> 6;
        if (c0 < c1) {
            stage(c0, 0);
            __syncthreads();
            for (int c = c0; c < c1; ++c) {
                const int cur = (c - c0) & 1;
                if (c + 1 < c1) stage(c + 1, cur ^ 1);
                const unsigned char *sb = smem + cur * G::STAGE;
                if (do_xbias) {
                    const float *xb_ = (const float *)sb + bch;
#pragma unroll
                    for (int t = 0; t < T; ++t)
                        for (int px = bpg; px < G::PIX; px += 4) bsum += xb_[(t * G::PIX + px) * 64];
                }
#pragma unroll 4
                for (int q = 0; q < G::PIX / 2; ++q) {
                    const int pix = 2 * q + lh;
                    const float b = *(const float *)(sb + b_lane + pix * 256);
#pragma unroll
                    for (int t = 0; t < T; ++t) {
                        const float a = *(const float *)(sb + t * G::IMG + a_lane + pix * 256);
                        acc[t] = __builtin_amdgcn_mfma_f32_32x32x2f32(a, b, acc[t], 0, 0, 0);
                    }
                }
                __syncthreads();
            }
        }
    }

    float *slab = p.slab + (size_t)grp * k.pstride;
    if constexpr (BF) {
        if (do_xbias) {
            const float v = bsum + __shfl_xor(bsum, 32, 64);
            if (lane < 32) slab[(size_t)T * p.Ci * p.Cj + it * 64 + wi * 32 + lane] = v;
        }
    } else {
        if (do_xbias) {
            float *red = (float *)smem;
            red[tid] = bsum;
            __syncthreads();
            if (tid < 64) slab[(size_t)T * p.Ci * p.Cj + it * 64 + tid] = (red[tid] + red[tid + 64]) + (red[tid + 128] + red[tid + 192]);
        }
    }
    f32x4 *dst4 = (f32x4 *)(slab + ((size_t)(tile * 4 + wave) * T) * 1024) + lane;
#pragma unroll
    for (int t = 0; t < T; ++t)
#pragma unroll
        for (int rq = 0; rq < 4; ++rq)
            dst4[(t * 4 + rq) * 64] = f32x4{acc[t][4 * rq], acc[t][4 * rq + 1], acc[t][4 * rq + 2], acc[t][4 * rq + 3]};
}

template <int PG>
__global__ __launch_bounds__(64 * PG) void wgrad_reduce_kernel(const float *__restrict__ slab, int nP, size_t pstride, int T, int Ci, int Cj,
                                                               int ci_real, int cj_real,
                                                               float *__restrict__ out, long si, long sj, long st, float *__restrict__ db, int ndb)
{
    const size_t nw = (size_t)T * Ci * Cj;
    const size_t total = nw + (db ? (size_t)ndb : 0);
    const int lane_e = threadIdx.x & 63, grp = threadIdx.x >> 6;
    __shared__ f32x4 red[PG][64];
    for (size_t base = (size_t)blockIdx.x * 256; base < total; base += (size_t)gridDim.x * 256) {
        const size_t e = base + 4 * lane_e;
        f32x4 s0 = {0.f, 0.f, 0.f, 0.f}, s1 = s0, s2 = s0, s3 = s0;
        if (e < total) {
            const float *src = slab + e;
            int P = grp;
            for (; P + 3 * PG < nP; P += 4 * PG) {
                s0 += *(const f32x4 *)(src + (size_t)P * pstride);
                s1 += *(const f32x4 *)(src + (size_t)(P + PG) * pstride);
                s2 += *(const f32x4 *)(src + (size_t)(P + 2 * PG) * pstride);
                s3 += *(const f32x4 *)(src + (size_t)(P + 3 * PG) * pstride);
            }
            for (; P < nP; P += PG) s0 += *(const f32x4 *)(src + (size_t)P * pstride);
        }
        red[grp][lane_e] = (s0 + s1) + (s2 + s3);
        __syncthreads();
        if (grp == 0 && e < total) {
            f32x4 v = red[0][lane_e];
#pragma unroll
            for (int g = 1; g < PG; ++g) v += red[g][lane_e];
            if (e < nw) {
                const int ln = (int)((e >> 2) & 63), rq = (int)((e >> 8) & 3);
                const size_t hi = e >> 10;
                const int t = (int)(hi % T);
                const int wv = (int)((hi / T) & 3);
                const int tile = (int)(hi / T / 4);
                const int ntj = Cj >> 6;
                const int it = tile / ntj, jt = tile - it * ntj;
                const int i0 = it * 64 + (wv >> 1) * 32 + 8 * rq + 4 * (ln >> 5);
                const int j = jt * 64 + (wv & 1) * 32 + (ln & 31);
#pragma unroll
                for (int ri = 0; ri < 4; ++ri)
                    if (i0 + ri < ci_real && j < cj_real) out[(i0 + ri) * si + j * sj + t * st] = v[ri];
            } else {
#pragma unroll
                for (int ri = 0; ri < 4; ++ri)
                    if (e - nw + ri < (size_t)ndb) db[e - nw + ri] = v[ri];
            }
        }
        __syncthreads();
    }
}

static void decompose(const WgradP &p, WgradK &k)
{
    const int wx = p.xwin1 - p.xwin0, wy = p.ywin1 - p.ywin0;
    const int pwmax = p.math == 2 ? PWB : PWMAX;
    k.nstrips = cdiv(wx, pwmax);
    int pw = cdiv(wx, k.nstrips);
    pw = p.math == 2 ? (pw + 15) & ~15 : (pw + 1) & ~1;
    if (pw > pwmax) pw = pwmax;
    k.pw = pw;
    k.nstrips = cdiv(wx, pw);
    k.ntile_i = p.Ci / 64;
    k.ntile_j = p.Cj / 64;
    k.ci_real = k.cj_real = 0;
    const int ntile = k.ntile_i * k.ntile_j;
    const int slots = 256 * ((p.TY == 3 && (p.math == 0 || p.math == 3)) ? 3 : 2);
    const long per_chunk = (long)p.NB * k.nstrips;
    static std::mutex mu;
    static std::map<std::array<long, 4>, std::pair<int, int>> cache;
    const std::array<long, 4> key = {per_chunk, (long)wy, (long)ntile, (long)slots};
    {
        std::lock_guard<std::mutex> lk(mu);
        auto itc = cache.find(key);
        if (itc != cache.end()) {
            k.rows_per_chunk = itc->second.first;
            k.nchunks = cdiv(wy, k.rows_per_chunk);
            k.nparts = (int)(per_chunk * k.nchunks);
            k.ngroups = itc->second.second;
            k.pstride = align_up((size_t)p.TY * p.TX * p.Ci * p.Cj + (p.Ci > p.Cj ? p.Ci : p.Cj), 64);
            return;
        }
    }
    double best = 1e300;
    int best_r = wy, best_g = 1;
    for (int r = 4; r <= wy; ++r) {
        const int nch = cdiv(wy, r);
        if (r > 4 && cdiv(wy, r - 1) == nch && r != wy) continue;
        const long nparts = per_chunk * nch;
        long gmax = nparts < 8L * slots / ntile + 1 ? nparts : 8L * slots / ntile + 1;
        if (gmax < 1) gmax = 1;
        for (long g = 1; g <= gmax; ++g) {
            const double frac = (double)(g * ntile) / (double)slots;
            const double rounds = frac <= 1.0 ? 1.0 : 0.5 * (frac + (double)((g * ntile + slots - 1) / slots));
            const double t = rounds * (double)((nparts + g - 1) / g) * (double)(r + 2);
            const double score = t * (1.0 + 0.02 * rounds);
            if (score < best - 1e-9) { best = score; best_r = r; best_g = (int)g; }
        }
        if (nch == 1) break;
    }
    k.rows_per_chunk = best_r;
    k.nchunks = cdiv(wy, best_r);
    k.nparts = (int)(per_chunk * k.nchunks);
    k.ngroups = best_g;
    {
        std::lock_guard<std::mutex> lk(mu);
        cache[key] = std::make_pair(best_r, best_g);
    }
    k.pstride = align_up((size_t)p.TY * p.TX * p.Ci * p.Cj + (p.Ci > p.Cj ? p.Ci : p.Cj), 64);
}

static bool up_applicable(const WgradP &p)
{
    static const int on = [] { const char *e = getenv("UNET_WGRAD_UP"); return e ? atoi(e) : 1; }();
    if ((!on && p.math != 2) || p.TY != 2 || p.TX != 2 || p.stride != 2 || p.xpad != 0 || p.oy0 != 0 || p.ox0 != 0) return false;
    if (p.math == 1 || (p.db && !p.db_on_x)) return false;
    if (p.ywin0 != 0 || p.xwin0 != 0 || p.ywin1 != p.YH || p.xwin1 != p.YW || p.XH != 2 * p.YH || p.XW != 2 * p.YW) return false;
    const size_t es = p.math == 2 ? 2 : 4;
    return fits_buffer(tensor_bytes(p.NB, p.XH, p.XW, p.XC, es)) && fits_buffer(tensor_bytes(p.NB, p.YH, p.YW, p.YC, es)) &&
           (p.math == 2 || get_lds_dma_mode() != 0);
}

static void up_decompose(const WgradP &p, WgradK &k)
{
    const int pix = p.math == 2 ? 64 : 32;
    k.ntile_i = p.Ci / 64; k.ntile_j = p.Cj / 64;
    k.up_npix = p.NB * p.YH * p.YW;
    k.up_nchunks = cdiv(k.up_npix, pix);
    const int ntile = k.ntile_i * k.ntile_j;
    int g = 512 / ntile;
    if (g < 1) g = 1;
    if (g > k.up_nchunks) g = k.up_nchunks;
    k.up_per = cdiv(k.up_nchunks, g);
    k.ngroups = cdiv(k.up_nchunks, k.up_per);
    k.d_yw = make_fastdiv((unsigned)p.YW);
    k.pstride = align_up((size_t)p.TY * p.TX * p.Ci * p.Cj + (p.Ci > p.Cj ? p.Ci : p.Cj), 64);
}

template <bool BF>
static int launch_wgrad_up(WgradK &k, hipStream_t st)
{
    using G = UpGeom<BF>;
    k.xbytes = (int)tensor_bytes(k.p.NB, k.p.XH, k.p.XW, k.p.XC, G::ES);
    k.ybytes = (int)tensor_bytes(k.p.NB, k.p.YH, k.p.YW, k.p.YC, G::ES);
    char tag[96];
    snprintf(tag, sizeof(tag), "wgrad_up<%s> Ci=%d Cj=%d Y=%dx%d chunks=%d per=%d groups=%d", BF ? "bf16" : "f32", k.p.Ci, k.p.Cj, k.p.YH, k.p.YW, k.up_nchunks, k.up_per, k.ngroups);
    return launch_profiled<wgrad_up_kernel<BF>>(k.ngroups * k.ntile_i * k.ntile_j, 256, G::LDS, st, PK_WGRAD, tag, wgrad_alg_flops(k.p),
                                                2.0 * (double)k.up_nchunks * G::PIX * 4.0 * k.p.Ci * k.p.Cj,
                                                BF ? wgrad_alg_bytes(k.p) / 2.0 + 2.0 * 4.0 * k.p.Ci * k.p.Cj : wgrad_alg_bytes(k.p), k);
}

static WgradP padded_tiles(const WgradP &p)
{
    WgradP q = p;
    q.Ci = (p.Ci + 63) / 64 * 64;
    q.Cj = (p.Cj + 63) / 64 * 64;
    return q;
}

size_t wgrad_slab_need(const WgradP &p0)
{
    const WgradP p = padded_tiles(p0);
    WgradK k{};
    decompose(p, k);
    size_t a = (size_t)k.ngroups * k.pstride * sizeof(float);
    const size_t b = wgradw_slab_need(p);
    if (p.TY == 2 && p.TX == 2 && p.stride == 2) {
        WgradK u{};
        up_decompose(p, u);
        const size_t c = (size_t)u.ngroups * u.pstride * sizeof(float);
        if (c > a) a = c;
    }
    return a > b ? a : b;
}

double wgrad_alg_flops(const WgradP &p)
{
    long cy = 0, cx = 0;
    for (int y = 0; y < p.YH; ++y)
        for (int t = 0; t < p.TY; ++t) { const int i = (y + p.oy0) * p.stride - p.xpad + t; cy += (i >= 0 && i < p.XH); }
    for (int x = 0; x < p.YW; ++x)
        for (int t = 0; t < p.TX; ++t) { const int i = (x + p.ox0) * p.stride - p.xpad + t; cx += (i >= 0 && i < p.XW); }
    return 2.0 * p.NB * (double)cy * (double)cx * p.Ci * p.Cj;
}

double wgrad_alg_bytes(const WgradP &p)
{
    int y0 = (p.ywin0 + p.oy0) * p.stride - p.xpad, y1 = (p.ywin1 - 1 + p.oy0) * p.stride - p.xpad + p.TY;
    int x0 = (p.xwin0 + p.ox0) * p.stride - p.xpad, x1 = (p.xwin1 - 1 + p.ox0) * p.stride - p.xpad + p.TX;
    y0 = y0 < 0 ? 0 : y0; x0 = x0 < 0 ? 0 : x0;
    y1 = y1 > p.XH ? p.XH : y1; x1 = x1 > p.XW ? p.XW : x1;
    double b = 0.0;
    if (y1 > y0 && x1 > x0) b += (double)p.NB * (y1 - y0) * (x1 - x0) * p.Ci * 4.0;
    b += (double)p.NB * (p.ywin1 - p.ywin0) * (p.xwin1 - p.xwin0) * p.Cj * 4.0;
    b += (double)p.TY * p.TX * p.Ci * p.Cj * 4.0;
    return b;
}

template <int TY, int TX, int S, int NSPLIT>
static int launch_wgrad_t(WgradK &k, hipStream_t st)
{
    using G = WgradGeom<TY, TX, S>;
    const size_t xb = tensor_bytes(k.p.NB, k.p.XH, k.p.XW, k.p.XC, 4), yb = tensor_bytes(k.p.NB, k.p.YH, k.p.YW, k.p.YC, 4);
    constexpr bool CAN_BUF = !(TY * TX == 9 && NSPLIT == 0);
    const bool buf = CAN_BUF && get_lds_dma_mode() != 0 && fits_buffer(xb) && fits_buffer(yb);
    k.xbytes = buf ? (int)xb : 0; k.ybytes = buf ? (int)yb : 0;
    const auto launch = buf ? launch_profiled<wgrad_f32_kernel<TY, TX, S, NSPLIT, CAN_BUF>, WgradK> : launch_profiled<wgrad_f32_kernel<TY, TX, S, NSPLIT, false>, WgradK>;
    char tag[96];
    snprintf(tag, sizeof(tag), "wgrad<%d;%d;%d;split%d> buf=%d Ci=%d Cj=%d Y=%dx%d win=%d parts=%d pw=%d rows=%d groups=%d", TY, TX, S, NSPLIT, (int)buf, k.p.Ci, k.p.Cj,
             k.p.YH, k.p.YW, k.p.ywin1 - k.p.ywin0, k.nparts, k.pw, k.rows_per_chunk, k.ngroups);
    const double rows = (double)k.p.NB * (k.p.ywin1 - k.p.ywin0) * k.nstrips;
    const double kpix = NSPLIT == 0 ? 2.0 * ((k.pw + 1) / 2) : 16.0 * ((k.pw + 15) / 16);
    return launch(k.ngroups * k.ntile_i * k.ntile_j, 256, G::LDS, st, PK_WGRAD, tag, wgrad_alg_flops(k.p),
                  2.0 * rows * kpix * G::T * k.p.Ci * k.p.Cj * (NSPLIT == 3 ? 3 : 1), wgrad_alg_bytes(k.p), k);
}

template <int TY, int TX, int S>
static int launch_wgrad_b(WgradK &k, hipStream_t st)
{
    using G = WgradBGeom<TY, TX, S>;
    const size_t xb = tensor_bytes(k.p.NB, k.p.XH, k.p.XW, k.p.XC, 2), yb = tensor_bytes(k.p.NB, k.p.YH, k.p.YW, k.p.YC, 2);
    ARG_CHECK(fits_buffer(xb) && fits_buffer(yb), "wgrad (bf16): tensor exceeds 2 GiB");
    k.xbytes = (int)xb; k.ybytes = (int)yb;
    char tag[96];
    snprintf(tag, sizeof(tag), "wgradb<%d;%d;%d> buf=1 Ci=%d Cj=%d Y=%dx%d win=%d parts=%d pw=%d rows=%d groups=%d", TY, TX, S, k.p.Ci, k.p.Cj, k.p.YH, k.p.YW,
             k.p.ywin1 - k.p.ywin0, k.nparts, k.pw, k.rows_per_chunk, k.ngroups);
    const double rows = (double)k.p.NB * (k.p.ywin1 - k.p.ywin0) * k.nstrips;
    return launch_profiled<wgrad_bf16_kernel<TY, TX, S>>(k.ngroups * k.ntile_i * k.ntile_j, 256, G::LDS, st, PK_WGRAD, tag, wgrad_alg_flops(k.p),
                                                         2.0 * rows * k.pw * G::T * k.p.Ci * k.p.Cj, wgrad_alg_bytes(k.p) / 2.0 + 2.0 * G::T * k.p.Ci * k.p.Cj, k);
}

int launch_wgrad(WgradP p, hipStream_t st)
{
    ARG_CHECK(p.Ci > 0 && p.Cj > 0 && p.Ci % 32 == 0 && p.Cj % 32 == 0, "wgrad: channel counts must be multiples of 32 (Ci=%d Cj=%d)", p.Ci, p.Cj);
    if (p.math == 2) ARG_CHECK(p.Ci % 64 == 0 && p.Cj % 64 == 0, "wgrad (bf16): channel counts must be multiples of 64 (Ci=%d Cj=%d)", p.Ci, p.Cj);
    const int ci_real = p.Ci, cj_real = p.Cj;
    const bool winograd = p.math == 3 && wgradw_applicable(p);
    p = padded_tiles(p);
    ARG_CHECK(p.XC % 4 == 0 && p.YC % 4 == 0 && p.xc0 % 4 == 0 && p.yc0 % 4 == 0, "wgrad: channel pitch/offset must be multiples of 4");
    if (p.math == 2) ARG_CHECK(p.XC % 8 == 0 && p.YC % 8 == 0 && p.xc0 % 8 == 0 && p.yc0 % 8 == 0, "wgrad (bf16): channel pitch/offset must be multiples of 8");
    ARG_CHECK(p.ywin0 >= 0 && p.ywin1 <= p.YH && p.xwin0 >= 0 && p.xwin1 <= p.YW && p.ywin0 < p.ywin1 && p.xwin0 < p.xwin1, "wgrad: bad window");
    ARG_CHECK(tensor_elems(p.NB, p.XH, p.XW, p.XC) < LIMIT_31BIT * 2 && tensor_elems(p.NB, p.YH, p.YW, p.YC) < LIMIT_31BIT * 2, "wgrad: tensor too large");
    p.zeros = zero_page();
    if (!p.zeros) return -2;
    ARG_CHECK(p.math >= 0 && p.math <= 3, "wgrad: bad arithmetic mode %d", p.math);
    if (p.db) ARG_CHECK(p.ywin0 == 0 && p.xwin0 == 0 && p.ywin1 == p.YH && p.xwin1 == p.YW, "wgrad: fused bias gradient needs the full Y window");
    if (p.db && p.db_on_x) ARG_CHECK(p.stride == p.TY && p.stride == p.TX && p.xpad == 0, "wgrad: bias-on-X needs stride == taps (every X pixel staged exactly once)");
    if (winograd) return launch_wgradw(p, st);
    WgradK k{};
    k.p = p;
    const bool up = up_applicable(p);
    if (up) up_decompose(p, k); else decompose(p, k);
    k.ci_real = ci_real; k.cj_real = cj_real;
    const int nP = k.ngroups;
    const int T = p.TY * p.TX;
    const size_t need = (size_t)nP * k.pstride * sizeof(float);
    ARG_CHECK(need <= p.slab_bytes, "wgrad: slab scratch too small (%zu < %zu)", p.slab_bytes, need);
    int rc;
    const int mode = p.math == 3 ? 0 : p.math;
    if (up)
        rc = mode == 2 ? launch_wgrad_up<true>(k, st) : launch_wgrad_up<false>(k, st);
    else if (p.TY == 3 && p.TX == 3 && p.stride == 1)
        rc = mode == 0 ? launch_wgrad_t<3, 3, 1, 0>(k, st) : mode == 1 ? launch_wgrad_t<3, 3, 1, 3>(k, st) : launch_wgrad_b<3, 3, 1>(k, st);
    else if (p.TY == 2 && p.TX == 2 && p.stride == 2) {
        if (mode == 2) { set_error("wgrad (bf16): the up-conv weight gradient needs tensors below 2 GiB and the full window"); return -4; }
        rc = mode == 0 ? launch_wgrad_t<2, 2, 2, 0>(k, st) : launch_wgrad_t<2, 2, 2, 3>(k, st);
    }
    else { set_error("wgrad: unsupported taps %dx%d stride %d", p.TY, p.TX, p.stride); return -4; }
    if (rc) return rc;
    const int ndb = p.db ? (p.db_on_x ? ci_real : cj_real) : 0;
    const size_t total = (size_t)T * p.Ci * p.Cj + ndb;
    size_t blocks = (total + 255) / 256;
    if (blocks > 16384) blocks = 16384;
    ARG_CHECK(k.pstride % 4 == 0 && ndb % 4 == 0 && ((uintptr_t)p.slab & 15) == 0, "wgrad: the reduce needs 16-byte aligned slabs");
    prof_begin(PK_REDUCE, "wgrad_reduce", st, 0.0, 0.0, (double)nP * k.pstride * 4.0 + (double)total * 4.0);
    if (nP >= 64)
        hipLaunchKernelGGL(wgrad_reduce_kernel<16>, dim3((unsigned)blocks), dim3(1024), 0, st, p.slab, nP, k.pstride, T, p.Ci, p.Cj, ci_real, cj_real, p.out, p.si, p.sj, p.st, p.db, ndb);
    else
        hipLaunchKernelGGL(wgrad_reduce_kernel<4>, dim3((unsigned)blocks), dim3(256), 0, st, p.slab, nP, k.pstride, T, p.Ci, p.Cj, ci_real, cj_real, p.out, p.si, p.sj, p.st, p.db, ndb);
    prof_end(st);
    HIP_TRY(hipGetLastError());
    return 0;
}

}
```

dl-unet_amd/csrc/wgradw.hip:

```cpp
#include "common.hpp"
#include "kernel_parts.hpp"
#include <cstdio>
#include <cstdlib>

namespace unet {

struct WgradWK {
    WgradP p;
    int TXn, TXg, TYn;
    int wy0, wx0;
    int NTg;
    int nsteps, steps_per;
    int ntile_i, ntile_j, nsplit;
    FastDiv d_spi, d_txg;
    size_t pstride;
    int xbytes, ybytes;
};

#ifndef WW_DBG
#define WW_DBG 0
#endif
constexpr int WW_PATCH = 32768, WW_EXTRA = 2048, WW_DY = 16384;
constexpr int WW_STAGE = WW_PATCH + WW_EXTRA + WW_DY;
constexpr int WW_NST = 3;
constexpr int WW_LDS = WW_NST * WW_STAGE;
constexpr int WW_SLAB = 9 * 64 * 64 + 64;

template <int N> __device__ __forceinline__ void ww_wait_vmcnt() { asm volatile("s_waitcnt vmcnt(%0)" ::"n"(N) : "memory"); }

__device__ __forceinline__ f32x2 wpk_add(f32x2 a, f32x2 b) { return a + b; }
__device__ __forceinline__ f32x2 wpk_sub(f32x2 a, f32x2 b) { return a - b; }

template <bool BUF>
__global__ __launch_bounds__(512, 1) void wgradw_f32_kernel(const WgradWK k)
{
    const WgradP &p = k.p;
    extern __shared__ __attribute__((aligned(16))) unsigned char smem[];

    const int tid = threadIdx.x, lane = tid & 63;
    const int wave = __builtin_amdgcn_readfirstlane(tid >> 6);
    const int wi = wave >> 1, wj = wave & 1;
    const int l15 = lane & 15, kg = lane >> 4;

    const int logical = xcd_slot();
    const int ntile = k.ntile_i * k.ntile_j;
    const int part = logical / ntile, tile = logical - part * ntile;
    const int it = tile / k.ntile_j, jt = tile - it * k.ntile_j;
    const int s0 = part * k.steps_per;
    int s1 = s0 + k.steps_per;
    s1 = s1 < k.nsteps ? s1 : k.nsteps;
    const int ns = s1 > s0 ? s1 - s0 : 0;

    const int d_cb = wave & 3, d_par = (wave >> 2) & 1;
    const int spi = k.TYn * k.TXg;

    const __amdgpu_buffer_rsrc_t rs_x = make_rsrc(p.X, BUF ? k.xbytes : 0);
    const __amdgpu_buffer_rsrc_t rs_y = make_rsrc(p.Y, BUF ? k.ybytes : 0);
    auto stage = [&](int buf, int step) {
        unsigned char *sb = smem + buf * WW_STAGE;
        int ln = lane;
        asm volatile("" : "+v"(ln));
        const int d_slot = ln >> 2, d_chunk = ln & 3;
        const int xch = p.xc0 + it * 64 + d_cb * 16 + d_chunk * 4;
        const int ych = p.yc0 + jt * 64 + d_cb * 16 + d_chunk * 4;
        const int Tb = step * 16;
        const bool tok = Tb + d_slot < k.NTg;
        const int img_b = fdiv(Tb, k.d_spi);
        const int rem_b = Tb - img_b * spi;
        const int ty_b = fdiv(rem_b, k.d_txg);
        int img = img_b, ty = ty_b, txg = rem_b - ty_b * k.TXg + d_slot;
        while (txg >= k.TXg) { txg -= k.TXg; ++ty; }
        while (ty >= k.TYn) { ty -= k.TYn; ++img; }
        img = img < p.NB ? img : p.NB - 1;
        {
            const int iy0 = (k.wy0 + 2 * ty + p.oy0) - p.xpad, ix = (k.wx0 + 2 * txg + p.ox0) - p.xpad + d_par;
            const bool xok = tok && (unsigned)ix < (unsigned)p.XW;
            const int base = ((img * p.XH + iy0) * p.XW + ix) * p.XC + xch;
#pragma unroll
            for (int qy = 0; qy < 4; ++qy) {
                const bool ok = xok && (unsigned)(iy0 + qy) < (unsigned)p.XH;
                unsigned char *dst = sb + ((qy * 2 + d_par) * 4 + d_cb) * 1024;
                if (BUF) {
                    lds_dma16(rs_x, dst, ok ? (base + qy * p.XW * p.XC) * 4 : LDS_DMA_OOB, 0);
                } else {
                    const float *g = ok ? p.X + (base + qy * p.XW * p.XC) : p.zeros;
                    GLDS16(g, dst);
                }
            }
        }
        {
            const int yy0 = k.wy0 + 2 * ty, xx = k.wx0 + 2 * txg + d_par;
            const bool xok = tok && txg < k.TXn && xx < p.YW;
            const int base = ((img * p.YH + yy0) * p.YW + xx) * p.YC + ych;
#pragma unroll
            for (int py = 0; py < 2; ++py) {
                const bool ok = xok && yy0 + py < p.YH;
                unsigned char *dst = sb + WW_PATCH + WW_EXTRA + ((py * 2 + d_par) * 4 + d_cb) * 1024;
                if (BUF) {
                    lds_dma16(rs_y, dst, ok ? (base + py * p.YW * p.YC) * 4 : LDS_DMA_OOB, 0);
                } else {
                    const float *g = ok ? p.Y + (base + py * p.YW * p.YC) : p.zeros;
                    GLDS16(g, dst);
                }
            }
        }
        if (wave < 2) {
            const int Te = step * 16 + 16;
            const bool eok = Te < k.NTg;
            const int Tec = eok ? Te : k.NTg - 1;
            const int eimg = fdiv(Tec, k.d_spi);
            const int erem = Tec - eimg * spi;
            const int ety = fdiv(erem, k.d_txg);
            const int etxg = erem - ety * k.TXg;
            const int e_row = (ln >> 4) + 4 * wave, e_cb = (ln >> 2) & 3;
            const int e_xch = p.xc0 + it * 64 + e_cb * 16 + d_chunk * 4;
            const int qy = e_row >> 1, par = e_row & 1;
            const int iy = (k.wy0 + 2 * ety + p.oy0) - p.xpad + qy, ix = (k.wx0 + 2 * etxg + p.ox0) - p.xpad + par;
            const bool ok = eok && (unsigned)iy < (unsigned)p.XH && (unsigned)ix < (unsigned)p.XW;
            const int eoff = ((eimg * p.XH + iy) * p.XW + ix) * p.XC + e_xch;
            if (BUF) {
                lds_dma16(rs_x, sb + WW_PATCH + wave * 1024, ok ? eoff * 4 : LDS_DMA_OOB, 0);
            } else {
                const float *g = ok ? p.X + eoff : p.zeros;
                GLDS16(g, sb + WW_PATCH + wave * 1024);
            }
        }
    };
    auto wait_landed = [&](bool one_in_flight) {
        if (!one_in_flight) ww_wait_vmcnt<0>();
        else if (wave < 2) ww_wait_vmcnt<7>();
        else ww_wait_vmcnt<6>();
    };

    f32x4 acc[16][2];
#pragma unroll
    for (int x = 0; x < 16; ++x)
#pragma unroll
        for (int j = 0; j < 2; ++j)
#pragma unroll
            for (int r = 0; r < 4; ++r) acc[x][j][r] = 0.f;
    f32x2 dbacc[2] = {{0.f, 0.f}, {0.f, 0.f}};

    const int a_base = wi * 1024 + l15 * 4;
    const int e_base = WW_PATCH + wi * 64 + l15 * 4;
    const bool last = kg == 3;
    const int y_base = WW_PATCH + WW_EXTRA + l15 * 4;

#define WW_SB() __builtin_amdgcn_sched_barrier(0)
    const int lv = a_base + kg * 64;
    const int lx = last ? e_base : lv + 9 * 64 + 256;
    const int lxs = last ? 512 : 8192;
    const int ly = y_base + 2 * wj * 1024 + kg * 64;
    auto v_read = [&](int buf, int pr, int j, f32x2 (&a)[4]) {
        if (WW_DBG & 4) { WW_SB(); return; }
        const unsigned char *pv = smem + buf * WW_STAGE + lv;
        if (j < 2 || pr == 0) {
#pragma unroll
            for (int qy = 0; qy < 4; ++qy) {
                const unsigned char *src = pv + ((2 * qy + (j & 1)) * 4096 + (8 * pr + (j >> 1)) * 64);
                a[qy][0] = *(const float *)(src);
                a[qy][1] = *(const float *)(src + 256);
            }
        } else {
            const unsigned char *px = smem + buf * WW_STAGE + lx + (j & 1) * (lxs >> 1);
#pragma unroll
            for (int qy = 0; qy < 4; ++qy) {
                a[qy][0] = *(const float *)(pv + ((2 * qy + (j & 1)) * 4096 + 9 * 64));
                a[qy][1] = *(const float *)(px + qy * lxs);
            }
        }
        WW_SB();
    };
    auto v_col = [&](int j, const f32x2 (&a)[4], f32x2 (&v)[16]) {
        if (WW_DBG & 8) { WW_SB(); return; }
        v[j] = wpk_sub(a[0], a[2]);
        v[4 + j] = wpk_add(a[1], a[2]);
        v[8 + j] = wpk_sub(a[2], a[1]);
        v[12 + j] = wpk_sub(a[1], a[3]);
        WW_SB();
    };
    auto v_row = [&](int i, f32x2 (&v)[16]) {
        if (WW_DBG & 8) { WW_SB(); return; }
        const f32x2 t0 = v[4 * i], t1 = v[4 * i + 1], t2 = v[4 * i + 2], t3 = v[4 * i + 3];
        v[4 * i + 0] = wpk_sub(t0, t2);
        v[4 * i + 1] = wpk_add(t1, t2);
        v[4 * i + 2] = wpk_sub(t2, t1);
        v[4 * i + 3] = wpk_sub(t1, t3);
        WW_SB();
    };
    auto z_read = [&](int buf, int pr, int c, f32x2 (&d)[4]) {
        if (WW_DBG & 4) { WW_SB(); return; }
        const unsigned char *ys = smem + buf * WW_STAGE + ly;
#pragma unroll
        for (int px = 0; px < 4; ++px) {
            d[px][0] = *(const float *)(ys + (px * 4096 + c * 1024 + pr * 512));
            d[px][1] = *(const float *)(ys + (px * 4096 + c * 1024 + pr * 512 + 256));
        }
        WW_SB();
    };
    auto group = [&](const f32x2 (&v)[16], const f32x2 (&d)[4], int c, bool RD, bool XF, int bufz, int prz, int cz, f32x2 (&dn)[4],
                     int bufv, int prv, f32x2 (&r)[4][4], f32x2 (&vn)[16]) {
        f32x2 zt[4];
        auto quad = [&](int b, int h) {
#pragma unroll
            for (int e = 0; e < 4; ++e)
                acc[4 * b + e][c] = __builtin_amdgcn_mfma_f32_16x16x4f32(v[4 * b + e][h], zt[e][h], acc[4 * b + e][c], 0, 0, 0);
            WW_SB();
        };
        zt[0] = d[0]; zt[1] = wpk_add(d[0], d[1]); zt[2] = wpk_sub(d[0], d[1]); zt[3] = d[1];
        WW_SB();
        quad(0, 0);
        z_read(bufz, prz, cz, dn);
        quad(0, 1);
        if (RD) v_read(bufv, prv, 0, r[0]);
        if (XF) { v_col(0, r[0], vn); v_col(1, r[1], vn); }
        zt[0] = wpk_add(d[0], d[2]); zt[3] = wpk_add(d[1], d[3]); zt[1] = wpk_add(zt[0], zt[3]); zt[2] = wpk_sub(zt[0], zt[3]);
        WW_SB();
        quad(1, 0);
        if (RD) v_read(bufv, prv, 1, r[1]);
        if (XF) { v_col(2, r[2], vn); v_col(3, r[3], vn); }
        quad(1, 1);
        if (RD) v_read(bufv, prv, 2, r[2]);
        if (XF) v_row(0, vn);
        zt[0] = wpk_sub(d[0], d[2]); zt[3] = wpk_sub(d[1], d[3]); zt[1] = wpk_add(zt[0], zt[3]); zt[2] = wpk_sub(zt[0], zt[3]);
        WW_SB();
        quad(2, 0);
        if (RD) v_read(bufv, prv, 3, r[3]);
        if (XF) v_row(1, vn);
        quad(2, 1);
        if (XF) v_row(2, vn);
        zt[0] = d[2]; zt[1] = wpk_add(d[2], d[3]); zt[2] = wpk_sub(d[2], d[3]); zt[3] = d[3];
        dbacc[c] = wpk_add(dbacc[c], wpk_add(wpk_add(d[0], d[1]), zt[1]));
        WW_SB();
        quad(3, 0);
        if (XF) {
            v_row(3, vn);
#pragma unroll
            for (int i = 0; i < 16; ++i) asm volatile("" : "+v"(vn[i]));
        }
        quad(3, 1);
    };
    if (ns > 0) {
        stage(0, s0);
        if (ns > 1) stage(1, s0 + 1);
        wait_landed(ns > 1);
        __builtin_amdgcn_s_barrier();
        const bool early = wave < 4;
        f32x2 va[16], vb[16], da[4], db_[4], r[4][4];
        {
#pragma unroll
            for (int j = 0; j < 4; ++j) { v_read(0, 0, j, r[j]); v_col(j, r[j], va); }
#pragma unroll
            for (int i = 0; i < 4; ++i) v_row(i, va);
        }
        z_read(0, 0, 0, da);
        for (int s = 0; s < ns; ++s) {
            const bool more = s + 2 < ns;
            const int buf = s % WW_NST, nbuf = (s + 1) % WW_NST;
            WW_SB();
            group(va, da, 0, true, false, buf, 0, 1, db_, buf, 1, r, vb);
            group(va, db_, 1, false, true, buf, 1, 0, da, buf, 1, r, vb);
            if (!(WW_DBG & 1)) ww_wait_vmcnt<0>();
            if (!(WW_DBG & 2)) __builtin_amdgcn_s_barrier();
            WW_SB();
            if (more && early && !(WW_DBG & 1)) stage((s + 2) % WW_NST, s0 + s + 2);
            WW_SB();
            group(vb, da, 0, true, false, buf, 1, 1, db_, nbuf, 0, r, va);
            group(vb, db_, 1, false, true, nbuf, 0, 0, da, nbuf, 0, r, va);
            if (more && !early && !(WW_DBG & 1)) stage((s + 2) % WW_NST, s0 + s + 2);
            WW_SB();
        }
    }
#undef WW_SB

    float *slab = p.slab + (size_t)(tile * k.nsplit + part) * k.pstride;
#pragma unroll
    for (int c = 0; c < 2; ++c) {
        f32x4 r[3][4];
#pragma unroll
        for (int b = 0; b < 4; ++b) {
            const f32x4 m0 = b == 3 ? -acc[b][c] : acc[b][c];
            const f32x4 m1 = b == 3 ? -acc[4 + b][c] : acc[4 + b][c];
            const f32x4 m2 = b == 3 ? -acc[8 + b][c] : acc[8 + b][c];
            const f32x4 m3 = b == 3 ? acc[12 + b][c] : -acc[12 + b][c];
            const f32x4 h = 0.5f * (m1 + m2);
            r[0][b] = m0 + h;
            r[1][b] = 0.5f * (m1 - m2);
            r[2][b] = h + m3;
        }
#pragma unroll
        for (int a = 0; a < 3; ++a) {
            const f32x4 h = 0.5f * (r[a][1] + r[a][2]);
            const f32x4 o0 = r[a][0] + h, o1 = 0.5f * (r[a][1] - r[a][2]), o2 = h + r[a][3];
            float *dst = slab + ((a * 3) * 64 + (2 * wj + c) * 16 + l15) * 64 + wi * 16 + 4 * kg;
            *(f32x4 *)(dst) = o0;
            *(f32x4 *)(dst + 4096) = o1;
            *(f32x4 *)(dst + 8192) = o2;
        }
    }
    if (wi == 0) {
#pragma unroll
        for (int c = 0; c < 2; ++c) {
            float v = dbacc[c][0] + dbacc[c][1];
            v += __shfl_xor(v, 16, 64);
            v += __shfl_xor(v, 32, 64);
            if (kg == 0) slab[9 * 64 * 64 + (2 * wj + c) * 16 + l15] = v;
        }
    }
}

template <int PG>
__global__ __launch_bounds__(64 * PG) void wgradw_reduce_kernel(const float *__restrict__ slab, int nsplit, size_t pstride, int ntile_j,
                                                            float *__restrict__ out, long si, long sj, long st,
                                                            float *__restrict__ db, int db_c0)
{
    const int tile = blockIdx.x >> 6, jb = blockIdx.x & 63;
    const int j = threadIdx.x & 63, grp = threadIdx.x >> 6;
    const float *src = slab + (size_t)tile * nsplit * pstride + (size_t)jb * 64 + j;
    float m[9];
#pragma unroll
    for (int x = 0; x < 9; ++x) m[x] = 0.f;
    for (int P = grp; P < nsplit; P += PG) {
        const float *s = src + (size_t)P * pstride;
#pragma unroll
        for (int x = 0; x < 9; ++x) m[x] += s[x * 4096];
    }
    __shared__ float red[PG][3][64];
#pragma unroll
    for (int xq = 0; xq < 3; ++xq) {
        if (xq) __syncthreads();
#pragma unroll
        for (int x = 0; x < 3; ++x) red[grp][x][j] = m[3 * xq + x];
        __syncthreads();
        if (grp == 0) {
#pragma unroll
            for (int x = 0; x < 3; ++x) {
                float v = red[0][x][j];
#pragma unroll
                for (int g = 1; g < PG; ++g) v += red[g][x][j];
                m[3 * xq + x] = v;
            }
        }
    }
    if (grp == 0) {
        const int it = tile / ntile_j, jt = tile - it * ntile_j;
        float *o = out + (size_t)(it * 64 + j) * si + (size_t)(jt * 64 + jb) * sj;
#pragma unroll
        for (int t = 0; t < 9; ++t) o[t * st] = m[t];
    }
    if (db && jb == 0 && (tile / ntile_j) == 0) {
        __syncthreads();
        const int jt = tile % ntile_j;
        float v = 0.f;
        for (int P = grp; P < nsplit; P += PG) v += slab[((size_t)tile * nsplit + P) * pstride + 9 * 64 * 64 + j];
        red[grp][0][j] = v;
        __syncthreads();
        if (grp == 0) {
            float t = red[0][0][j];
#pragma unroll
            for (int g = 1; g < PG; ++g) t += red[g][0][j];
            db[db_c0 + jt * 64 + j] = t;
        }
    }
}

bool wgradw_applicable(const WgradP &p)
{
    if (p.TY != 3 || p.TX != 3 || p.stride != 1) return false;
    if (p.Ci % 64 != 0 || p.Cj % 64 != 0 || p.db_on_x) return false;
    return true;
}

static void ww_decompose(const WgradP &p, WgradWK &k, int cus)
{
    k.p = p;
    k.wy0 = p.ywin0; k.wx0 = p.xwin0;
    k.TYn = cdiv(p.ywin1 - p.ywin0, 2);
    k.TXn = cdiv(p.xwin1 - p.xwin0, 2);
    k.TXg = k.TXn + 1;
    k.NTg = p.NB * k.TYn * k.TXg;
    k.nsteps = cdiv(k.NTg, 16);
    k.ntile_i = p.Ci / 64; k.ntile_j = p.Cj / 64;
    const int ntile = k.ntile_i * k.ntile_j;
    int nsplit = cus / ntile;
    if (nsplit < 1) nsplit = 1;
    if (nsplit > k.nsteps) nsplit = k.nsteps;
    k.nsplit = nsplit;
    k.steps_per = cdiv(k.nsteps, nsplit);
    k.d_spi = make_fastdiv((unsigned)(k.TYn * k.TXg));
    k.d_txg = make_fastdiv((unsigned)k.TXg);
    k.pstride = WW_SLAB;
}

size_t wgradw_slab_need(const WgradP &p)
{
    if (!wgradw_applicable(p)) return 0;
    WgradWK k;
    ww_decompose(p, k, 256);
    return (size_t)k.ntile_i * k.ntile_j * k.nsplit * k.pstride * sizeof(float);
}

int launch_wgradw(const WgradP &p, hipStream_t st)
{
    const size_t xb = tensor_bytes(p.NB, p.XH, p.XW, p.XC, sizeof(float)), yb = tensor_bytes(p.NB, p.YH, p.YW, p.YC, sizeof(float));
    const bool buf = get_lds_dma_mode() != 0 && fits_buffer(xb) && fits_buffer(yb);
    const auto launch = buf ? launch_profiled<wgradw_f32_kernel<true>, WgradWK> : launch_profiled<wgradw_f32_kernel<false>, WgradWK>;
    WgradWK k;
    int cus = device_cu_count();
    if (cus > 256) cus = 256;
    ww_decompose(p, k, cus);
    k.xbytes = buf ? (int)xb : 0; k.ybytes = buf ? (int)yb : 0;
    const int ntile = k.ntile_i * k.ntile_j;
    const size_t need = (size_t)ntile * k.nsplit * k.pstride * sizeof(float);
    ARG_CHECK(need <= p.slab_bytes, "wgradw: slab scratch too small (%zu < %zu)", p.slab_bytes, need);
    ARG_CHECK(tensor_elems(p.NB, p.XH, p.XW, p.XC) < LIMIT_31BIT && tensor_elems(p.NB, p.YH, p.YW, p.YC) < LIMIT_31BIT,
              "wgradw: tensor exceeds 31-bit element offsets");
    if (p.db) ARG_CHECK(p.ywin0 == 0 && p.xwin0 == 0 && p.ywin1 == p.YH && p.xwin1 == p.YW, "wgradw: fused bias gradient needs the full Y window");
    char tag[96];
    snprintf(tag, sizeof(tag), "wgradw<%d> Ci=%d Cj=%d Y=%dx%d tiles=%dx%d steps=%d split=%d", (int)buf, p.Ci, p.Cj, p.YH, p.YW, k.TYn, k.TXn, k.nsteps, k.nsplit);
    if (int rc_ = launch(ntile * k.nsplit, 512, WW_LDS, st, PK_WGRAD, tag, wgrad_alg_flops(p), 2.0 * k.nsteps * 16.0 * 16.0 * p.Ci * p.Cj, wgrad_alg_bytes(p), k)) return rc_;
    prof_begin(PK_REDUCE, "wgradw_reduce", st, 0.0, 0.0, (double)ntile * k.nsplit * k.pstride * 4.0 + 9.0 * p.Ci * p.Cj * 4.0);
    if (ntile <= 4 && k.nsplit >= 32)
        hipLaunchKernelGGL(wgradw_reduce_kernel<16>, dim3(ntile * 64), dim3(1024), 0, st, p.slab, k.nsplit, k.pstride, k.ntile_j,
                           p.out, p.si, p.sj, p.st, p.db, p.yc0);
    else
        hipLaunchKernelGGL(wgradw_reduce_kernel<4>, dim3(ntile * 64), dim3(256), 0, st, p.slab, k.nsplit, k.pstride, k.ntile_j,
                           p.out, p.si, p.sj, p.st, p.db, p.yc0);
    prof_end(st);
    HIP_TRY(hipGetLastError());
    return 0;
}

}
```

dl-unet_amd/csrc/wino.hip:

```cpp
#include "common.hpp"
#include "kernel_parts.hpp"
#include <cstdio>
#include <cstdlib>

namespace unet {

struct WinoP {
    IgemmP p;
    const float *U;
    int tiles_x, tiles_y;
    int MT;
    int nsteps;
    FastDiv d_tpi, d_tx;
    int xbytes[2], ubytes;
    int gn, gn_shift;
};


__global__ __launch_bounds__(256) void wino_transform_ref_kernel(const float *__restrict__ w, int I, int dgrad, int n0, int Nn, int k0, int Kc,
                                                                 float *__restrict__ U)
{
    const size_t total = (size_t)Nn * Kc;
    const size_t idx = (size_t)blockIdx.x * 256 + threadIdx.x;
    if (idx >= total) return;
    int n, c;
    if (dgrad) { c = (int)(idx / Nn); n = (int)(idx - (size_t)c * Nn); }
    else       { n = (int)(idx / Kc); c = (int)(idx - (size_t)n * Kc); }
    const int o = dgrad ? k0 + c : n0 + n, i = dgrad ? n0 + n : k0 + c;
    const float *src = w + ((size_t)o * I + i) * 9;
    float g[3][3];
#pragma unroll
    for (int t = 0; t < 9; ++t) g[t / 3][t % 3] = src[dgrad ? 8 - t : t];
    float r[4][3];
#pragma unroll
    for (int j = 0; j < 3; ++j) {
        r[0][j] = g[0][j];
        r[1][j] = 0.5f * (g[0][j] + g[1][j] + g[2][j]);
        r[2][j] = 0.5f * (g[0][j] - g[1][j] + g[2][j]);
        r[3][j] = g[2][j];
    }
    float u[16];
#pragma unroll
    for (int a = 0; a < 4; ++a) {
        u[4 * a + 0] = r[a][0];
        u[4 * a + 1] = 0.5f * (r[a][0] + r[a][1] + r[a][2]);
        u[4 * a + 2] = 0.5f * (r[a][0] - r[a][1] + r[a][2]);
        u[4 * a + 3] = r[a][2];
    }
    const int nsteps = Kc >> 3;
    const int nt = n >> 6, n16 = (n >> 4) & 3, nl = n & 15;
    const int step = c >> 3, kk = c & 7, kg = kk >> 1, h = kk & 1;
    float *blk = U + ((size_t)nt * nsteps + step) * 8192;
#pragma unroll
    for (int xg = 0; xg < 4; ++xg) {
        f32x4 v = {u[4 * xg], u[4 * xg + 1], u[4 * xg + 2], u[4 * xg + 3]};
        *(f32x4 *)(blk + ((n16 * 4 + xg) * 2 + h) * 256 + (kg * 16 + nl) * 4) = v;
    }
}

int wino_transform_ref(const float *w_oihw, int I, int dgrad, int n0, int Nn, int k0, int Kc, float *U, hipStream_t st)
{
    ARG_CHECK(w_oihw && U && Nn % 32 == 0 && Kc % 8 == 0 && Kc > 0, "wino_transform_ref: bad shape");
    const size_t total = (size_t)Nn * Kc;
    hipLaunchKernelGGL(wino_transform_ref_kernel, dim3((unsigned)((total + 255) / 256)), dim3(256), 0, st, w_oihw, I, dgrad, n0, Nn, k0, Kc, U);
    HIP_TRY(hipGetLastError());
    return 0;
}

constexpr int WINO_ROW = 72 * 32;
constexpr int WINO_PATCH = 8 * WINO_ROW;

template <int N> __device__ __forceinline__ void wino_wait_vmcnt() { asm volatile("s_waitcnt vmcnt(%0)" ::"n"(N) : "memory"); }

__device__ __forceinline__ f32x2 pk_add(f32x2 a, f32x2 b) { return a + b; }
__device__ __forceinline__ f32x2 pk_sub(f32x2 a, f32x2 b) { return a - b; }

constexpr int W32_UBASE = 2 * WINO_PATCH;
constexpr int W32_LDS = W32_UBASE + 2 * 16384;
constexpr int W32_TOTAL = W32_LDS + 1280 + 5 * 256 * 4;

template <bool BUF>
__global__ __launch_bounds__(256, 2) void wino32_f32_kernel(const WinoP k)
{
    const IgemmP &p = k.p;
    extern __shared__ __attribute__((aligned(16))) unsigned char smem[];

    const int tid = threadIdx.x, lane = tid & 63;
    const int wave = __builtin_amdgcn_readfirstlane(tid >> 6);
    const int l15 = lane & 15, kg = lane >> 4;
    const int tpi = k.tiles_x * k.tiles_y;
    const int ns = k.nsteps;
    int e_scatter = p.scatter, e_DH = p.DH, e_DW = p.DW, e_DC = p.DC, e_dwy0 = p.dwy0, e_dwx0 = p.dwx0, e_OH = p.OH, e_OW = p.OW;
    int e_rw0 = p.rw0, e_rw1 = p.rw1, e_dn0 = p.dn0, e_cout = p.cout, e_relu = p.relu, e_Nn = p.Nn, e_MT = k.MT;
    const float *e_add = p.add, *e_mask = p.mask, *e_bias = p.bias;
    float *e_dst = p.dst, *e_pool = p.pool_dst;
    asm volatile("" : "+s"(e_scatter), "+s"(e_DH), "+s"(e_DW), "+s"(e_DC), "+s"(e_dwy0), "+s"(e_dwx0), "+s"(e_OH), "+s"(e_OW));
    asm volatile("" : "+s"(e_rw0), "+s"(e_rw1), "+s"(e_dn0), "+s"(e_cout), "+s"(e_relu), "+s"(e_Nn), "+s"(e_MT));
    asm volatile("" : "+s"(e_add), "+s"(e_mask), "+s"(e_bias), "+s"(e_dst), "+s"(e_pool));
    typedef const float __attribute__((address_space(1))) *gcfp;
    typedef float __attribute__((address_space(1))) *gfp;
    const gcfp g_add = (gcfp)e_add, g_mask = (gcfp)e_mask, g_bias = (gcfp)e_bias;
    const gfp g_dst = (gfp)e_dst, g_pool = (gfp)e_pool;
    __builtin_amdgcn_s_setprio(3);

    const int slot = xcd_slot();
    int nt, mt;
    {
        const int per = p.mtiles << k.gn_shift;
        const int ng = slot / per, rem = slot - ng * per;
        mt = rem >> k.gn_shift;
        nt = (ng << k.gn_shift) + (rem & (k.gn - 1));
    }
    const int T0 = mt * 64, n0 = nt * 32;

    const float *ublk = k.U + (size_t)(nt >> 1) * ns * 8192 + (nt & 1) * 4096 + (4 * wave) * 256 + lane * 4;
    __amdgpu_buffer_rsrc_t rs_x = make_rsrc(p.src[0].p, BUF ? k.xbytes[0] : 0);
    __amdgpu_buffer_rsrc_t rs_u = make_rsrc(k.U, BUF ? k.ubytes : 0);
    const int u_voff = ((4 * wave) * 256 + lane * 4) * 4;
    const int u_soff0 = ((nt >> 1) * ns * 8192 + (nt & 1) * 4096) * 4;
    int uissued = 0;
    auto issue_u = [&]() {
        const int buf = uissued & 1;
        unsigned char *ub = smem + W32_UBASE + buf * 16384 + (4 * wave) * 1024;
        if (BUF) {
            const int us = u_soff0 + uissued * 32768;
#pragma unroll
            for (int i = 0; i < 4; ++i)
                lds_dma16(rs_u, ub + i * 1024, u_voff, us + i * 1024);
        } else {
            const float *us = ublk + (size_t)uissued * 8192;
#pragma unroll
            for (int i = 0; i < 4; ++i) GLDS16(us + i * 256, ub + i * 1024);
        }
        ++uissued;
    };
    constexpr int NPI = 5;
    const int npi = wave < 2 ? 5 : 4;
    int poff[NPI];
    int *poff1 = (int *)(smem + W32_LDS + 1280) + tid;
    const int tiles_x = k.tiles_x;
    const int img0 = fdiv(T0, k.d_tpi);
    const int trem0 = T0 - img0 * tpi;
    const int ty0 = fdiv(trem0, k.d_tx);
    const int tx0 = trem0 - ty0 * tiles_x;
    const float rtx = 1.0f / (float)tiles_x;
    {
        const int nsrc = p.nsrc, oy0 = p.oy0, ox0 = p.ox0, MT = k.MT;
        const int img0_ = img0;
        int sH[2], sW[2], sC[2], sc0[2], spad[2];
#pragma unroll
        for (int si = 0; si < 2; ++si) { sH[si] = p.src[si].H; sW[si] = p.src[si].W; sC[si] = p.src[si].C; sc0[si] = p.src[si].c0; spad[si] = p.src[si].pad; }
        int rowp[2], imgb[2][2];
#pragma unroll
        for (int si = 0; si < 2; ++si) { rowp[si] = sW[si] * sC[si]; imgb[si][0] = img0_ * sH[si] * rowp[si] + sc0[si]; imgb[si][1] = imgb[si][0] + sH[si] * rowp[si]; }
        const int lastrel = MT - 1 - T0;
#pragma unroll
        for (int ii = 0; ii < NPI; ++ii) {
            const int u = (wave + 4 * ii) * 64 + lane;
            const int row = (int)(((float)u + 0.5f) * (1.0f / 144.0f));
            const int rem = u - row * 144;
            const int idx = rem >> 1;
            const int qy = row >> 1, par = row & 1, half = (rem & 1) ^ ((idx >> 3) & 1);
            const bool tail = idx >= 64;
            const int j = idx - 64;
            const int erow = j * tiles_x - tx0;
            int e = tail ? erow + tiles_x - 1 : idx;
            e = e < 63 ? e : 63;
            e = e < lastrel ? e : lastrel;
            const bool ok = !tail | (erow <= 63);
            const int qx = tail ? 2 + par : par;
            const int t = tx0 + e;
            const int r = (int)(((float)t + 0.5f) * rtx);
            const int tx = t - r * tiles_x;
            int ty = ty0 + r;
            const bool wrap = ty >= k.tiles_y;
            ty = wrap ? ty - k.tiles_y : ty;
#pragma unroll
            for (int si = 0; si < 2; ++si) {
                const int iy = 2 * ty + oy0 - spad[si] + qy, ix = 2 * tx + ox0 - spad[si] + qx;
                const bool inb = ok & ((unsigned)iy < (unsigned)sH[si]) & ((unsigned)ix < (unsigned)sW[si]) & (si < nsrc) & (ii < npi);
                int o = (wrap ? imgb[si][1] : imgb[si][0]) + __mul24(iy, rowp[si]) + __mul24(ix, sC[si]) + 4 * half;
                o = inb ? o : -1;
                if (si == 0) poff[ii] = o; else if (nsrc > 1) poff1[ii * 256] = o;
            }
        }
    }
    const float *sp = p.src[0].p;
    int snch = p.src[0].nch, kc = 0, pissued = 0;
    if (BUF) {
#pragma unroll
        for (int ii = 0; ii < NPI; ++ii) poff[ii] = poff[ii] >= 0 ? poff[ii] * 4 : LDS_DMA_OOB;
    }
    const int tl = wave * 16 + l15;
    const int offA = tl * 32 + (((kg >> 1) ^ ((tl >> 3) & 1)) * 16) + (kg & 1) * 8;
    int offB;
    {
        const int t = tx0 + tl;
        const int r = (int)(((float)t + 0.5f) * rtx);
        const bool rowend = (t - r * tiles_x == tiles_x - 1) || tl == 63;
        int j = r;
        j = j < 7 ? j : 7;
        const int idxB = rowend ? 64 + j : tl + 1;
        offB = idxB * 32 + (((kg >> 1) ^ ((idxB >> 3) & 1)) * 16) + (kg & 1) * 8;
    }
    const int b_rd = W32_UBASE + lane * 16;

    auto issue_patch = [&]() {
        const int buf = pissued & 1;
        unsigned char *sb = smem + buf * WINO_PATCH + wave * 1024;
        if (BUF) {
#pragma unroll
            for (int ii = 0; ii < 4; ++ii)
                lds_dma16(rs_x, sb + ii * 4096, poff[ii], kc * 4);
            if (wave < 2)
                lds_dma16(rs_x, sb + 16384, poff[4], kc * 4);
        } else {
#pragma unroll
            for (int ii = 0; ii < 4; ++ii) {
                const float *g = poff[ii] >= 0 ? sp + (poff[ii] + kc) : p.zeros;
                GLDS16(g, sb + ii * 4096);
            }
            if (wave < 2) {
                const float *g = poff[4] >= 0 ? sp + (poff[4] + kc) : p.zeros;
                GLDS16(g, sb + 16384);
            }
        }
        ++pissued;
        kc += 8;
        if (kc == snch && pissued < ns) {
            kc = 0;
            sp = p.src[1].p; snch = p.src[1].nch;
            if (BUF) rs_x = make_rsrc(p.src[1].p, k.xbytes[1]);
#pragma unroll
            for (int ii = 0; ii < NPI; ++ii) { const int o = poff1[ii * 256]; poff[ii] = BUF ? (o >= 0 ? o * 4 : LDS_DMA_OOB) : o; }
        }
    };
    auto issue_stage = [&]() { issue_patch(); issue_u(); };

    f32x4 acc[16][2];
#pragma unroll
    for (int x = 0; x < 16; ++x)
#pragma unroll
        for (int j = 0; j < 2; ++j)
#pragma unroll
            for (int r = 0; r < 4; ++r) acc[x][j][r] = 0.f;
    f32x2 v0[16];
    f32x4 bf[2][2];

    auto load_v = [&](int buf) {
        const unsigned char *sa = smem + buf * WINO_PATCH + offA;
        const unsigned char *sb = smem + buf * WINO_PATCH + offB;
#pragma unroll
        for (int j = 0; j < 4; ++j) {
            const unsigned char *src = (j < 2 ? sa : sb) + (j & 1) * WINO_ROW;
            const f32x2 a0 = *(const f32x2 *)(src);
            const f32x2 a1 = *(const f32x2 *)(src + 2 * WINO_ROW);
            const f32x2 a2 = *(const f32x2 *)(src + 4 * WINO_ROW);
            const f32x2 a3 = *(const f32x2 *)(src + 6 * WINO_ROW);
            v0[j] = pk_sub(a0, a2);
            v0[4 + j] = pk_add(a1, a2);
            v0[8 + j] = pk_sub(a2, a1);
            v0[12 + j] = pk_sub(a1, a3);
        }
#pragma unroll
        for (int i = 0; i < 4; ++i) {
            const f32x2 t0 = v0[4 * i], t1 = v0[4 * i + 1], t2 = v0[4 * i + 2], t3 = v0[4 * i + 3];
            v0[4 * i + 0] = pk_sub(t0, t2);
            v0[4 * i + 1] = pk_add(t1, t2);
            v0[4 * i + 2] = pk_sub(t2, t1);
            v0[4 * i + 3] = pk_sub(t1, t3);
        }
    };
    auto read_b = [&](int buf, int c) {
        const unsigned char *sb = smem + buf * 16384 + b_rd;
        bf[c & 1][0] = *(const f32x4 *)(sb + c * 1024);
        bf[c & 1][1] = *(const f32x4 *)(sb + 8192 + c * 1024);
    };

    issue_stage();
    issue_stage();
    if (wave < 2) wino_wait_vmcnt<9>(); else wino_wait_vmcnt<8>();
    __builtin_amdgcn_s_barrier();
    read_b(0, 0);
    load_v(0);
    __builtin_amdgcn_s_setprio(0);
    for (int s = 0; s < ns; ++s) {
        const int ub = s & 1;
#pragma unroll
        for (int c = 0; c < 8; ++c) {
            const int xg = c >> 1, h = c & 1;
            if (c + 1 < 8) read_b(ub, c + 1);
#pragma unroll
            for (int e = 0; e < 4; ++e) {
                acc[4 * xg + e][0] = __builtin_amdgcn_mfma_f32_16x16x4f32(v0[4 * xg + e][h], bf[c & 1][0][e], acc[4 * xg + e][0], 0, 0, 0);
                acc[4 * xg + e][1] = __builtin_amdgcn_mfma_f32_16x16x4f32(v0[4 * xg + e][h], bf[c & 1][1][e], acc[4 * xg + e][1], 0, 0, 0);
            }
            __builtin_amdgcn_sched_barrier(0);
        }
        wino_wait_vmcnt<0>();
        __builtin_amdgcn_s_barrier();
        if (s + 2 < ns) issue_stage();
        if (s + 1 < ns) {
            read_b((s + 1) & 1, 0);
            load_v((s + 1) & 1);
        }
    }
    __builtin_amdgcn_s_setprio(3);
    float *stg = (float *)(smem + W32_UBASE);
    unsigned *rowoff = (unsigned *)(smem + W32_LDS);
    unsigned char *rflag = smem + W32_LDS + 1024;
    {
        const int tl2 = tid >> 2, py = (tid >> 1) & 1, px = tid & 1;
        const int lastrel = e_MT - 1 - T0;
        const bool tok = tl2 <= lastrel;
        const int t = tx0 + (tok ? tl2 : lastrel);
        const int r = (int)(((float)t + 0.5f) * rtx);
        const int tx = t - r * tiles_x;
        int ty = ty0 + r;
        const bool wrap = ty >= k.tiles_y;
        ty = wrap ? ty - k.tiles_y : ty;
        int oy = 2 * ty + py, ox = 2 * tx + px;
        const bool ok = tok & (oy < e_OH) & (ox < e_OW);
        oy = oy < e_OH ? oy : e_OH - 1; ox = ox < e_OW ? ox : e_OW - 1;
        const bool win = e_scatter == 2;
        const int PH = win ? e_DH : e_OH, PW = win ? e_DW : e_OW, py0 = win ? e_dwy0 : 0, px0 = win ? e_dwx0 : 0;
        const int rowp = PW * e_DC;
        const int ib = (img0 + (wrap ? 1 : 0)) * PH * rowp;
        const unsigned off = (unsigned)(ib + __mul24(oy + py0, rowp) + __mul24(ox + px0, e_DC));
        rowoff[tid] = off;
        const bool inwin = (e_rw1 > e_rw0) & (oy >= e_rw0) & (oy < e_rw1) & (ox >= e_rw0) & (ox < e_rw1);
        rflag[tid] = (ok ? 0 : 1) | (inwin ? 2 : 0);
    }
    __syncthreads();

    const bool relu_win = e_rw1 > e_rw0;
    const int c4 = tid & 7;
    const int ncol = n0 + 4 * c4;
    size_t eo[2][4];
    unsigned char efl[2][4];
    f32x4 eadd[2][4], emask[2][4];
#pragma unroll
    for (int h = 0; h < 2; ++h)
#pragma unroll
        for (int u = 0; u < 4; ++u) {
            const int row = (h * 32 + (tid >> 3)) * 4 + u;
            eo[h][u] = (size_t)rowoff[row] + (size_t)(e_dn0 + ncol);
            efl[h][u] = rflag[row];
        }
    if (e_add) {
#pragma unroll
        for (int h = 0; h < 2; ++h)
#pragma unroll
            for (int u = 0; u < 4; ++u) eadd[h][u] = *(const __attribute__((address_space(1))) f32x4 *)(g_add + eo[h][u]);
    }
    if (e_mask) {
#pragma unroll
        for (int h = 0; h < 2; ++h)
#pragma unroll
            for (int u = 0; u < 4; ++u) emask[h][u] = *(const __attribute__((address_space(1))) f32x4 *)(g_mask + eo[h][u]);
    }
#pragma unroll
    for (int nn = 0; nn < 2; ++nn) {
        const int n = nn * 16 + l15;
#pragma unroll
        for (int r = 0; r < 4; ++r) {
            float s0[4], s1[4];
#pragma unroll
            for (int j = 0; j < 4; ++j) {
                s0[j] = acc[j][nn][r] + acc[4 + j][nn][r] + acc[8 + j][nn][r];
                s1[j] = acc[4 + j][nn][r] - acc[8 + j][nn][r] - acc[12 + j][nn][r];
            }
            const int tile = wave * 16 + 4 * kg + r;
            float *o = stg + tile * 128 + (n ^ ((kg & 1) << 4));
            o[((0 ^ (r & 1))) * 32] = s0[0] + s0[1] + s0[2];
            o[((1 ^ (r & 1))) * 32] = s0[1] - s0[2] - s0[3];
            o[((2 ^ (r & 1))) * 32] = s1[0] + s1[1] + s1[2];
            o[((3 ^ (r & 1))) * 32] = s1[1] - s1[2] - s1[3];
        }
    }
    __syncthreads();
    f32x4 bv = {0.f, 0.f, 0.f, 0.f};
    if (e_bias) {
#pragma unroll
        for (int c = 0; c < 4; ++c) { const int n = ncol + c; bv[c] = g_bias[e_cout ? n % e_cout : n]; }
    }
#pragma unroll
    for (int h = 0; h < 2; ++h) {
        f32x4 v[4];
        const int tloc = h * 32 + (tid >> 3);
#pragma unroll
        for (int u = 0; u < 4; ++u)
            v[u] = *(const f32x4 *)(stg + tloc * 128 + (u ^ (tloc & 1)) * 32 + ((4 * c4) ^ (((tloc >> 2) & 1) << 4))) + bv;
        if (e_add) {
#pragma unroll
            for (int u = 0; u < 4; ++u) v[u] += eadd[h][u];
        }
        if (e_relu) {
#pragma unroll
            for (int u = 0; u < 4; ++u) {
                const bool defer = relu_win && (efl[h][u] & 2);
#pragma unroll
                for (int c = 0; c < 4; ++c) v[u][c] = (v[u][c] > 0.f || defer) ? v[u][c] : 0.f;
            }
        }
        if (e_mask) {
#pragma unroll
            for (int u = 0; u < 4; ++u)
#pragma unroll
                for (int c = 0; c < 4; ++c) v[u][c] = emask[h][u][c] > 0.f ? v[u][c] : 0.f;
        }
#pragma unroll
        for (int u = 0; u < 4; ++u)
            if (!(efl[h][u] & 1)) *(__attribute__((address_space(1))) f32x4 *)(g_dst + eo[h][u]) = v[u];
        if (e_pool) {
            const int T = T0 + tloc;
            if (T < e_MT) {
                f32x4 m;
#pragma unroll
                for (int c = 0; c < 4; ++c) m[c] = fmaxf(fmaxf(v[0][c], v[1][c]), fmaxf(v[2][c], v[3][c]));
                *(__attribute__((address_space(1))) f32x4 *)(g_pool + (size_t)T * e_Nn + ncol) = m;
            }
        }
    }
}


bool wino_applicable(const IgemmP &p)
{
    if (p.T != 9 || p.TX != 3 || p.stride != 1 || p.scatter == 1) return false;
    if (p.Nn % 32 != 0) return false;
    if (cdiv(p.OW, 2) < 9) return false;
    if (cdiv(p.OH, 2) < 7) return false;
    for (int i = 0; i < p.nsrc; ++i)
        if (p.src[i].nch % 8 != 0) return false;
    for (int i = 0; i < p.nsrc; ++i)
        if ((long)p.src[i].W * p.src[i].C >= (1l << 23) || p.src[i].H >= (1 << 22)) return false;
    if ((long)(p.scatter == 2 ? p.DW : p.OW) * p.DC >= (1l << 23)) return false;
    if (cdiv(p.OW, 2) >= (1 << 12)) return false;
    return true;
}

size_t wino_u_floats(int Kc, int Nn) { return (size_t)16 * Kc * ((Nn + 63) / 64 * 64); }

bool wino_fuses_pool(const IgemmP &p)
{
    return p.math == 3 && wino_applicable(p) && !p.scatter && !(p.OH & 1) && !(p.OW & 1) && !p.dn0 && p.DC == p.Nn;
}

int launch_wino(const IgemmP &p, const float *U, hipStream_t st)
{
    WinoP q;
    q.p = p;
    q.U = U;
    q.tiles_x = cdiv(p.OW, 2);
    q.tiles_y = cdiv(p.OH, 2);
    q.MT = p.NB * q.tiles_x * q.tiles_y;
    int kc = 0;
    for (int i = 0; i < p.nsrc; ++i) kc += p.src[i].nch;
    q.nsteps = kc / 8;
    q.d_tpi = make_fastdiv((unsigned)(q.tiles_x * q.tiles_y));
    q.d_tx = make_fastdiv((unsigned)q.tiles_x);
    q.p.mtiles = cdiv(q.MT, 64);
    for (int i = 0; i < p.nsrc; ++i)
        ARG_CHECK((long)p.src[i].W * p.src[i].C < (1l << 23) && p.src[i].H < (1 << 22), "wino: source row pitch %ld exceeds the 24-bit multiply range", (long)p.src[i].W * p.src[i].C);
    ARG_CHECK((long)(p.scatter == 2 ? p.DW : p.OW) * p.DC < (1l << 23), "wino: destination row pitch exceeds the 24-bit multiply range");
    ARG_CHECK(q.tiles_x < (1 << 12), "wino: %d tile columns exceed the exact range of the float-floor tile decomposition", q.tiles_x);
    q.p.ntiles = p.Nn / 32;
    const size_t ub = wino_u_floats(kc, p.Nn) * sizeof(float);
    const bool buf = igemm_source_bytes(p, sizeof(float), q.xbytes) < 0 && fits_buffer(ub) && get_lds_dma_mode() != 0;
    q.ubytes = (int)ub;
    static const int gn_env = [] { const char *e = getenv("UNET_WINO_GN"); return e ? atoi(e) : 4; }();
    q.gn = 1; q.gn_shift = 0;
    while (q.gn * 2 <= gn_env && q.p.ntiles % (q.gn * 2) == 0) { q.gn *= 2; ++q.gn_shift; }
    char tag32[96];
    snprintf(tag32, sizeof(tag32), "wino32<%d> M=%d N=%d Kd=%d nsrc=%d tiles=%d", (int)buf, p.M, p.Nn, p.Kd, p.nsrc, q.MT);
    const auto launch = buf ? launch_profiled<wino32_f32_kernel<true>, WinoP> : launch_profiled<wino32_f32_kernel<false>, WinoP>;
    return launch(q.p.mtiles * q.p.ntiles, 256, W32_TOTAL, st, PK_WINO, tag32, igemm_alg_flops(p), igemm_alg_flops(p) * (16.0 / 36.0), igemm_alg_bytes(p), q);
}

}
```

include/unet_hip.h:

```cpp
#ifndef UNET_HIP_H
#define UNET_HIP_H

#include <stddef.h>
#include <stdint.h>

#ifdef __cplusplus
extern "C" {
#endif

#define UNET_N_PARAMS 46
#define UNET_N_LAYERS 23
#define UNET_MAX_CLASSES 16

enum {
    UNET_E_BADSIZE  = -1,
    UNET_E_BADARG   = -2,
    UNET_E_NOTREADY = -3,
    UNET_E_UNSUPPORTED = -4,
    UNET_E_COMM     = -5
};

typedef struct unet_handle unet_handle;

typedef struct unet_config {
    int base_ch;
    int device;
    int math;
} unet_config;

const char *unet_last_error(void);
int unet_abi_version(void);

int unet_set_math(int mode);
int unet_get_math(void);
int unet_set_lds_dma(int mode);

int unet_create(unet_handle **out, const unet_config *cfg);
int unet_create_classes(unet_handle **out, const unet_config *cfg, int n_classes);
int unet_n_classes(const unet_handle *h);
int unet_destroy(unet_handle *h);

int unet_output_size(int S, int *out_size);
int unet_param_count(const unet_handle *h, int idx, size_t *numel);

size_t unet_workspace_bytes(const unet_handle *h, int B, int S, int training);

int unet_forward(unet_handle *h, const void *const *params, const void *x, void *logits,
                 int B, int S, void *workspace, size_t workspace_bytes, int training,
                 void *stream);

int unet_backward(unet_handle *h, const void *const *params, const void *dlogits,
                  void *const *grads, void *workspace, size_t workspace_bytes, void *stream);
int unet_set_overlap(int on);
int unet_backward_stages(void);
int unet_backward_stage(unet_handle *h, int stage, const void *const *params,
                        const void *dlogits, void *const *grads, void *workspace,
                        size_t workspace_bytes, void *stream);
int unet_backward_input(unet_handle *h, const void *const *params, void *dx, void *workspace, size_t workspace_bytes, void *stream);
int unet_backward_stage_params(int stage, int *idx, int cap);

double unet_flops(const unet_handle *h, int B, int S, int backward);

int unet_activation_bytes(const unet_handle *h);

int unet_debug_buffer(const unet_handle *h, int B, int S, int training, const char *name,
                      size_t *offset, int *extent, int *channels);

#define UNET_DP_ID_BYTES 128
int unet_set_grad_scale(unet_handle *h, float scale);
int unet_dp_unique_id(void *id_out_host);
int unet_dp_init(unet_handle *h, int rank, int world, const void *id_host);
int unet_dp_destroy(unet_handle *h);
int unet_dp_world(unet_handle *h);
int unet_dp_rccl_version(void);
int unet_dp_allreduce(unet_handle *h, void *buf, size_t count, void *stream);
int unet_dp_broadcast(unet_handle *h, void *buf, size_t count, int root, void *stream);
int unet_dp_join(unet_handle *h, void *stream);

int unet_profile_enable(int on);
int unet_profile_select(unsigned kinds);
int unet_profile_reset(void);
int unet_profile_read(int kind, double *ms_total, long *launches, double *flops_total, double *exec_flops_total,
                      double *bytes_total);
int unet_profile_dump(const char *path);

size_t unet_bce_scratch_bytes(size_t numel);
int unet_bce_logits(const void *logits, const void *target, const void *weight,
                    long wsB, long wsC, long wsH, long wsW, int B, int H, int W,
                    void *loss_out, void *dlogits, float grad_scale, void *scratch, void *stream);
size_t unet_bce_step_scratch_bytes(size_t npix);
int unet_bce_step(const void *logits, long xsB, long xsC, long xsH, const void *labels_i64, const void *weight,
                  long wsB, long wsC, long wsH, long wsW, int B, int H, int W, void *loss_out, void *dlogits,
                  float grad_scale, void *mask_i64, void *scratch, void *stream);
int unet_onehot2(const void *labels_i64, void *target, int B, int H, int W, void *stream);
size_t unet_softmax_ce_scratch_bytes(size_t npix);
int unet_softmax_ce_step(const void *logits, long xsB, long xsC, long xsH, int K, const void *labels_i64, const void *weight,
                         long wsB, long wsH, long wsW, int B, int H, int W, void *loss_out, void *dlogits, float grad_scale,
                         void *mask_i64, void *invalid_u64, void *scratch, void *stream);

int unet_argmax2(const void *logits, long batch_stride, long plane_stride, long row_stride,
                 void *out_i64, int B, int H, int W, void *stream);
int unet_argmaxk(const void *logits, long batch_stride, long plane_stride, long row_stride, int K, void *out_i64, int B, int H, int W,
                 void *stream);

int unet_sgd_momentum(void *const *params, const void *const *grads, void *const *bufs,
                      const size_t *numel, int n, float lr, float mu, int first_step,
                      void *stream);

int unet_minmax(const void *x, int B, size_t n_per_image, void *out_minmax, void *stream);
int unet_mirror_pad(const void *x, int B, int n, int S, const void *minmax, void *out, void *stream);
int unet_tile_gather(const void *img, int B, int H, int W, const void *minmax, int S, int oy0, int ox0, int ny, int nx, long t0, int nt,
                     void *tiles_out, void *stream);
int unet_tile_stitch(const void *logits, int So, int oy0, int ox0, int ny, int nx, long t0, int nt, int B, int H, int W, void *mask_i64,
                     void *prob_f32, void *stream);
int unet_tile_stitch_k(const void *logits, int So, int K, int oy0, int ox0, int ny, int nx, long t0, int nt, int B, int H, int W,
                       void *mask_i64, void *prob_f32, void *stream);
int unet_eval_masks(const void *logits, long batch_stride, long plane_stride, long row_stride, int pad,
                    const void *labels_i64, void *mask_i64, int B, int n, void *stats_u64, void *stream);
int unet_eval_confusion(const void *logits, long batch_stride, long plane_stride, long row_stride, int pad, int K,
                        const void *labels_i64, void *mask_i64, int B, int n, void *conf_u64, void *invalid_u64, void *stream);
int unet_class_balance(const void *labels_i64, int B, int H, int W, void *weights, void *counts_u64, void *stream);
size_t unet_weighted_map_scratch_bytes(int B, int H, int W);
int unet_weighted_map(const void *labels, int labels_dtype, int B, int H, int W, float w0, float sig2, void *weights_f32,
                      void *counts_u64, void *n_objects_i32, void *scratch, void *stream);
int unet_gaussian_filter(const void *field, int B, int H, int W, const void *weights, int radius, float scale,
                         void *tmp, void *out, void *stream);
int unet_warp_bilinear(const void *img, const void *dy, const void *dx, int B, int H, int W, void *out, void *stream);
size_t unet_rotate_scratch_bytes(int B, int S);
int unet_reflect_rotate_crop(const void *img, int B, int n, int pad, int S, const float *angles_deg_host, int levels,
                             void *out, void *scratch, void *stream);

size_t unet_conv3x3_scratch_bytes(int C, int K);
int unet_conv3x3_fwd(const void *x1, int H1, int W1, int C1, int pad1, const void *x2, int C2,
                     int B, int H, int W, const void *w_oihw, const void *bias, int K, int relu,
                     void *y, void *scratch, void *stream);
size_t unet_conv3x3_bwd_scratch_bytes(int B, int H, int W, int C, int K);
int unet_conv3x3_bwd(const void *x1, int H1, int W1, int C1, int pad1, const void *x2, int C2,
                     int B, int H, int W, const void *w_oihw, int K, const void *dz,
                     void *dx1, const void *mask1, const void *add1, void *dx2, const void *mask2,
                     void *dw, void *db, void *scratch, void *stream);
int unet_maxpool2_fwd(const void *x, void *y, int B, int H, int W, int C, void *stream);
int unet_maxpool2_bwd(const void *pre, const void *dy, void *dpre, int B, int H, int W, int C,
                      void *stream);
size_t unet_upconv2_scratch_bytes(int B, int H, int W, int Ci, int Co);
int unet_upconv2_fwd(const void *x, int B, int H, int W, int Ci, const void *w_iohw,
                     const void *bias, int Co, void *y, void *scratch, void *stream);
int unet_upconv2_bwd(const void *x, int B, int H, int W, int Ci, const void *w_iohw, int Co,
                     const void *dy, void *dx, const void *mask, void *dw, void *db,
                     void *scratch, void *stream);
int unet_head1x1_fwd(const void *x, int B, int H, int W, int C, const void *w, const void *bias,
                     void *logits, void *stream);
size_t unet_head1x1_bwd_scratch_bytes(int B, int H, int W, int C);
int unet_head1x1_bwd(const void *x, int B, int H, int W, int C, const void *w,
                     const void *dlogits, void *dz, void *dw, void *db, void *scratch,
                     void *stream);
int unet_head1xk_fwd(const void *x, int B, int H, int W, int C, int K, const void *w, const void *bias, void *logits, void *stream);
size_t unet_head1xk_bwd_scratch_bytes(int B, int H, int W, int C, int K);
int unet_head1xk_bwd(const void *x, int B, int H, int W, int C, int K, const void *w, const void *dlogits, void *dz, void *dw, void *db,
                     void *scratch, void *stream);
int unet_conv1ch_fwd(const void *x, int B, int S, const void *w, const void *bias, int K,
                     void *y, void *stream);
size_t unet_conv1ch_bwd_scratch_bytes(int B, int S, int K);
int unet_conv1ch_bwd(const void *x, int B, int S, int K, const void *dz, void *dw, void *db,
                     void *scratch, void *stream);

#ifdef __cplusplus
}
#endif
#endif
```

Measured before the change: 255.1 tiles/s.

## Batch Winograd weight transforms and wgrad reductions into grouped launches per stage

Weight Winograd transforms are no longer launched once per layer. A collect pass gathers them into a table, and one table-driven kernel per forward group or backward stage runs them all, with LDS staging so the stores to U are coalesced. Wgrad split-K reductions are likewise deferred into a per-stage table and issued as one combined launch, so slabs are sub-allocated within each stage and the slab is sized to the largest per-stage sum. The aim is to cut many small kernel launches and their serialization, at the cost of a larger slab and extra host-side collect passes. The behaviour is on by default through UNET_BATCH_PREP.

```diff
diff --git a/dl-unet_amd/_hip.py b/dl-unet_amd/_hip.py
--- a/dl-unet_amd/_hip.py
+++ b/dl-unet_amd/_hip.py
@@ -20,6 +20,7 @@
     "unet_set_lds_dma": (C.c_int, [C.c_int]),
     "unet_set_grad_scale": (C.c_int, [vp, C.c_float]),
     "unet_set_overlap": (C.c_int, [C.c_int]),
+    "unet_set_batch_prep": (C.c_int, [C.c_int]),
     "unet_dp_unique_id": (C.c_int, [vp]),
     "unet_dp_init": (C.c_int, [vp, C.c_int, C.c_int, vp]),
     "unet_dp_destroy": (C.c_int, [vp]),
diff --git a/dl-unet_amd/csrc/common.hpp b/dl-unet_amd/csrc/common.hpp
--- a/dl-unet_amd/csrc/common.hpp
+++ b/dl-unet_amd/csrc/common.hpp
@@ -126,7 +126,11 @@
 bool wino_applicable(const IgemmP &p);
 bool wino_fuses_pool(const IgemmP &p);
 size_t wino_u_floats(int Kc, int Nn);
-int wino_transform_ref(const float *w_oihw, int I, int dgrad, int n0, int Nn, int k0, int Kc, float *U, hipStream_t st);
+struct WinoXform { const float *w; float *U; int I, dgrad, n0, Nn, k0, Kc; unsigned b0; };
+constexpr int WINO_XF_MAX = 24;
+struct WinoXformTable { WinoXform e[WINO_XF_MAX]; unsigned nblocks = 0; int n = 0; double bytes = 0.0; };
+int wino_transform_add(WinoXformTable &tb, const float *w_oihw, int I, int dgrad, int n0, int Nn, int k0, int Kc, float *U);
+int wino_transform_launch(const WinoXformTable &tb, hipStream_t st);
 int get_math_mode();
 void set_math_mode(int m);
 static inline int op_es() { return get_math_mode() == 2 ? 2 : 4; }
@@ -148,6 +152,24 @@
     const float *zeros;
     int math;
 };
+struct ReduceEntry {
+    const float *slab; float *out, *db;
+    size_t pstride;
+    long si, sj, st;
+    int wino;
+    int pg;
+    int nP;
+    int ntile_j, db_c0;
+    int T, Ci, Cj, ci_real, cj_real;
+    int ndb;
+    unsigned units;
+    unsigned b0;
+};
+constexpr int REDUCE_MAX = 12;
+struct ReduceTable { ReduceEntry e[REDUCE_MAX]; unsigned nblocks = 0; int n = 0; double bytes = 0.0; };
+void wgrad_reduce_defer(ReduceTable *tb);
+int wgrad_reduce_submit(const ReduceEntry &e, double bytes, hipStream_t st);
+int wgrad_reduce_launch(ReduceTable &tb, hipStream_t st);
 size_t wgrad_slab_need(const WgradP &p);
 double wgrad_alg_flops(const WgradP &p);
 double wgrad_alg_bytes(const WgradP &p);
diff --git a/dl-unet_amd/csrc/net.hip b/dl-unet_amd/csrc/net.hip
--- a/dl-unet_amd/csrc/net.hip
+++ b/dl-unet_amd/csrc/net.hip
@@ -162,15 +162,29 @@
     }
 };
 
+enum { PREP_COLLECT, PREP_READY };
+struct Prep { int mode = PREP_COLLECT; WinoXformTable tab; };
+static thread_local Prep *t_prep = nullptr;
+static inline bool collecting() { return t_prep && t_prep->mode == PREP_COLLECT; }
+struct PrepScope {
+    Prep *prev;
+    explicit PrepScope(Prep *p) : prev(t_prep) { t_prep = p; }
+    ~PrepScope() { t_prep = prev; }
+};
+static inline int run_igemm(const IgemmP &p, hipStream_t st) { return collecting() ? 0 : launch_igemm(p, st); }
+
 static int with_wino(IgemmP &p, float *wu, WLayer &L, int n0, int k0, hipStream_t st)
 {
-    if (p.math != 3 || !wu || !wino_applicable(p)) return L.ensure_packed(st);
+    if (p.math != 3 || !wu || !wino_applicable(p)) return collecting() ? 0 : L.ensure_packed(st);
+    p.wino_u = wu;
+    if (t_prep && t_prep->mode == PREP_READY) return 0;
     int kc = 0;
     for (int i = 0; i < p.nsrc; ++i) kc += p.src[i].nch;
-    int rc = wino_transform_ref(L.w, L.I, L.dgrad ? 1 : 0, n0, p.Nn, k0, kc, wu, st);
-    if (rc) return rc;
-    p.wino_u = wu;
-    return 0;
+    WinoXformTable one;
+    WinoXformTable &tb = t_prep ? t_prep->tab : one;
+    int rc = wino_transform_add(tb, L.w, L.I, L.dgrad ? 1 : 0, n0, p.Nn, k0, kc, wu);
+    if (rc || t_prep) return rc;
+    return wino_transform_launch(one, st);
 }
 
 static int check_size(int S)
@@ -221,21 +235,21 @@
         IgemmP p = conv_fwd_desc(x1, H1, H1, C1, pad1, x2, C2, B, H, H, wt, bias, K, relu, y);
         if ((rc = with_wino(p, wu, L, 0, 0, st))) return rc;
         if (pool_dst && p.wino_u && wino_fuses_pool(p)) { p.pool_dst = pool_dst; *pool_fused = true; }
-        return launch_igemm(p, st);
+        return run_igemm(p, st);
     }
     const int ldw = 9 * (C1 + C2);
     IgemmP a = conv_fwd_desc(x2, H, H, C2, 0, nullptr, 0, B, H, H, adv(wt, 9 * C1), bias, K, relu, y);
     a.ldw = ldw;
     if (relu) { a.rw0 = w0; a.rw1 = w1; }
     if ((rc = with_wino(a, wu, L, 0, C1, st))) return rc;
-    if ((rc = launch_igemm(a, st))) return rc;
+    if ((rc = run_igemm(a, st))) return rc;
     IgemmP b = conv_fwd_desc(x1, H1, H1, C1, pad1, nullptr, 0, B, H, H, wt, nullptr, K, relu, y);
     b.ldw = ldw;
     b.OH = b.OW = w1 - w0; b.M = B * b.OH * b.OW; b.oy0 = b.ox0 = w0;
     b.scatter = 2; b.dwy0 = b.dwx0 = w0; b.DH = b.DW = Ho;
     b.add = y;
     if ((rc = with_wino(b, wu ? wu + wino_u_floats(C2, K) : nullptr, L, 0, 0, st))) return rc;
-    return launch_igemm(b, st);
+    return run_igemm(b, st);
 }
 
 static IgemmP upconv_fwd_desc(const float *x, int B, int H, int W, int Ci, const float *wt, const float *bias, int Co, float *y)
@@ -320,12 +334,12 @@
     if (dx1) {
         IgemmP d = conv_dgrad_desc(dz, Ho, Ho, K, B, H1, pad1, L.wt, C1, dx1, mask1, add1);
         if ((rc = with_wino(d, wu, L, 0, 0, st))) return rc;
-        if ((rc = launch_igemm(d, st))) return rc;
+        if ((rc = run_igemm(d, st))) return rc;
     }
     if (dx2) {
         IgemmP d = conv_dgrad_desc(dz, Ho, Ho, K, B, H, 0, adv(L.wt, (size_t)C1 * 9 * K), C2, dx2, mask2, nullptr);
         if ((rc = with_wino(d, wu + wino_u_floats(K, C1), L, C1, 0, st))) return rc;
-        if ((rc = launch_igemm(d, st))) return rc;
+        if ((rc = run_igemm(d, st))) return rc;
     }
     return 0;
 }
@@ -360,6 +374,8 @@
     unet_handle *h; const Plan &pl; char *base; hipStream_t st;
     const void *const *params; void *const *grads;
     WgradStream wst;
+    bool batch_reduce = false; int stage = 0;
+    ReduceTable red; size_t slab_used = 0;
     Ctx(unet_handle *h, const Plan &pl, void *workspace, void *stream, const void *const *params, void *const *grads, bool overlap = false)
         : h(h), pl(pl), base((char *)workspace), st((hipStream_t)stream), params(params), grads(grads), wst{h, st, overlap, false} {}
     float *ws(size_t off) const { return base ? (float *)(base + off) : nullptr; }
@@ -385,6 +401,8 @@
     w[1] = conv_wgrad_desc(cx.ws(u.off), u.e, u.c, 0, dz, y.e, y.c, pl.B, dw, x.c + u.c, x.c, slab, pl.slab_bytes, db);
     return 2;
 }
+
+static size_t slab_take(const WgradP &w) { return align_up(wgrad_slab_need(w), 256); }
 
 static int make_plan(Plan &pl, int base, int B, int S, int training, int math, int ncls = 2)
 {
@@ -431,15 +449,16 @@
             a->g = take(sq(a->e, a->c));
             if (a >= pl.t && a < pl.t + 4) pl.g_ts[a - pl.t] = take(sq(a->e, a->c));
         }
-        size_t need = 0;
+        size_t need[N_STAGES] = {0}, most = 0;
         const Ctx sizing(nullptr, pl, nullptr, nullptr, nullptr, nullptr);
         for (int i = 0; i < UNET_N_LAYERS; ++i) {
             WgradP w[2];
             const int nw = layer_wgrad(sizing, i, w);
-            for (int j = 0; j < nw; ++j) { const size_t s = wgrad_slab_need(w[j]); if (s > need) need = s; }
-        }
-        pl.slab_bytes = need;
-        pl.slab = take_b(need);
+            for (int j = 0; j < nw; ++j) need[LAYERS[i].stage] += slab_take(w[j]);
+        }
+        for (int s = 0; s < N_STAGES; ++s) if (need[s] > most) most = need[s];
+        pl.slab_bytes = most;
+        pl.slab = take_b(most);
         size_t sm = 0;
         auto upds = [&](size_t s) { if (s > sm) sm = s; };
         for (int l = 0; l < 5; ++l) { upds(bias_grad_scratch_bytes(sq(pl.a1[l].e, 1), pl.ch[l])); upds(bias_grad_scratch_bytes(sq(pl.a2[l].e, 1), pl.ch[l])); }
@@ -537,6 +556,14 @@
     return 0;
 }
 
+static int g_batch_prep = [] { const char *e = getenv("UNET_BATCH_PREP"); const int v = e ? atoi(e) : 1; return v < 0 || v > 2 ? 1 : v; }();
+int unet_set_batch_prep(int on)
+{
+    ARG_CHECK(on >= 0 && on <= 2, "unet_set_batch_prep: 0 (one launch per layer), 1 (batched) or 2 (batched, one forward group)");
+    g_batch_prep = on;
+    return 0;
+}
+
 static int handle_math(const unet_handle *h) { return h->math >= 0 ? h->math : get_math_mode(); }
 
 int unet_output_size(int S, int *out_size)
@@ -604,7 +631,24 @@
                                  pools ? cx.ws(pl.t[L.level].off) : nullptr, &pool_fused);
         if (rc) return rc;
     }
-    return pools && !pool_fused ? pool_launch(cx, L.level, false) : 0;
+    return pools && !pool_fused && !collecting() ? pool_launch(cx, L.level, false) : 0;
+}
+
+static int fwd_group(int layer, int batch) { return batch == 2 ? 0 : (layer >= 10 ? 5 : 0) + LAYERS[layer].level; }
+
+static int forward_transforms(const Ctx &cx, int first, int batch, Prep &prep)
+{
+    prep = Prep();
+    PrepScope scope(&prep);
+    for (int i = first; i < UNET_N_LAYERS && fwd_group(i, batch) == fwd_group(first, batch); ++i)
+        if (LAYERS[i].kind == K_CONV || LAYERS[i].kind == K_CAT)
+            if (int rc = conv_forward(cx, i)) return rc;
+    prep.mode = PREP_READY;
+    char nm[40];
+    if (batch == 2) snprintf(nm, sizeof(nm), "fwd.transform");
+    else snprintf(nm, sizeof(nm), "fwd.l%d%s.transform", LAYERS[first].level, first >= 10 ? "e" : "c");
+    ProfScope ps(nm);
+    return wino_transform_launch(prep.tab, cx.st);
 }
 
 int unet_forward(unet_handle *h, const void *const *params, const void *x, void *logits, int B, int S,
@@ -627,8 +671,12 @@
         if ((rc = pack_upconv_fwd(cx.w(i), cx.ws(pl.wt_fwd[i]), pl.ch[LAYERS[i].ci], pl.ch[LAYERS[i].co], t_es, st))) return rc;
     }
 
+    const int batch = g_batch_prep;
+    Prep prep;
+    PrepScope scope(batch ? &prep : nullptr);
     for (int i = 0; i < UNET_N_LAYERS; ++i) {
         const Layer &L = LAYERS[i];
+        if (batch && (i == 0 || fwd_group(i, batch) != fwd_group(i - 1, batch)) && (rc = forward_transforms(cx, i, batch, prep))) return rc;
         switch (L.kind) {
         case K_CONV1: {
             RowScope rs(i, "fwd");
@@ -703,14 +751,28 @@
     return k;
 }
 
+static int stage_reduce(Ctx &cx)
+{
+    char nm[40]; snprintf(nm, sizeof(nm), "stage%d.reduce", cx.stage);
+    ProfScope ps(nm);
+    cx.slab_used = 0;
+    return wgrad_reduce_launch(cx.red, cx.wst.same());
+}
+
 static int wgrad_backward(Ctx &cx, int layer)
 {
-    RowScope rs(layer, "wgrad");
     WgradP w[2];
     const int n = layer_wgrad(cx, layer, w);
     for (int j = 0; j < n; ++j) {
-        int rc = launch_wgrad(w[j], j ? cx.wst.same() : cx.wst.get());
-        if (rc) return rc;
+        int rc;
+        if (cx.batch_reduce) {
+            const size_t take = slab_take(w[j]);
+            if ((cx.slab_used + take > cx.pl.slab_bytes || cx.red.n == REDUCE_MAX) && (rc = stage_reduce(cx))) return rc;
+            w[j].slab = (float *)((char *)w[j].slab + cx.slab_used); w[j].slab_bytes = take;
+            cx.slab_used += take;
+        }
+        RowScope rs(layer, "wgrad");
+        if ((rc = launch_wgrad(w[j], j ? cx.wst.same() : cx.wst.get()))) return rc;
     }
     return 0;
 }
@@ -722,13 +784,39 @@
     const Act &x = pl.in(L), &y = pl.out(L);
     const bool pooled = L.in == T_T;
     int rc;
-    if ((rc = wgrad_backward(cx, layer))) return rc;
+    if (!collecting() && (rc = wgrad_backward(cx, layer))) return rc;
     {
         RowScope rs(layer, "dgrad");
         if ((rc = conv_dgrad_launch(cx.ws(y.g), y.e, y.c, pl.B, cx.w(layer), cx.ws(pl.wt_bwd[layer]), cx.ws(pl.wu_bwd[layer]), x.e, x.c, 0, cx.ws(x.g),
                                     pooled ? nullptr : cx.ws(x.off), pooled ? cx.ws(pl.g_ts[L.ci]) : nullptr, 0, 0, nullptr, nullptr, cx.st))) return rc;
     }
-    return pooled ? pool_launch(cx, L.ci, true) : 0;
+    return pooled && !collecting() ? pool_launch(cx, L.ci, true) : 0;
+}
+
+static int cat_backward(Ctx &cx, int layer)
+{
+    const Plan &pl = cx.pl;
+    const int l = LAYERS[layer].level;
+    const Act &t = pl.t[l], &u = pl.u[l], &y = pl.d1[l];
+    int rc;
+    if (!collecting() && (rc = wgrad_backward(cx, layer))) return rc;
+    RowScope rs(layer, "dgrad");
+    return conv_dgrad_launch(cx.ws(y.g), y.e, y.c, pl.B, cx.w(layer), cx.ws(pl.wt_bwd[layer]), cx.ws(pl.wu_bwd[layer]), t.e, t.c, pl.pad[l], cx.ws(pl.g_ts[l]),
+                             nullptr, nullptr, u.e, u.c, cx.ws(u.g), nullptr, cx.st);
+}
+
+static int stage_transforms(Ctx &cx, int stage, Prep &prep)
+{
+    PrepScope scope(&prep);
+    for (int i = UNET_N_LAYERS - 1; i >= 0; --i) {
+        if (LAYERS[i].stage != stage) continue;
+        int rc = LAYERS[i].kind == K_CONV ? conv_backward(cx, i) : LAYERS[i].kind == K_CAT ? cat_backward(cx, i) : 0;
+        if (rc) return rc;
+    }
+    prep.mode = PREP_READY;
+    char nm[40]; snprintf(nm, sizeof(nm), "stage%d.transform", stage);
+    ProfScope ps(nm);
+    return wino_transform_launch(prep.tab, cx.st);
 }
 
 static int backward_stage_body(Ctx &cx, int stage, const void *dlogits)
@@ -737,6 +825,9 @@
     hipStream_t st = cx.st;
     const int B = pl.B;
     int rc;
+    Prep prep;
+    PrepScope scope(g_batch_prep ? &prep : nullptr);
+    if (g_batch_prep && (rc = stage_transforms(cx, stage, prep))) return rc;
     for (int i = UNET_N_LAYERS - 1; i >= 0; --i) {
         const Layer &L = LAYERS[i];
         if (L.stage != stage) continue;
@@ -752,15 +843,9 @@
         case K_CONV:
             if ((rc = conv_backward(cx, i))) return rc;
             break;
-        case K_CAT: {
-            const int l = L.level;
-            const Act &t = pl.t[l], &u = pl.u[l], &y = pl.d1[l];
-            if ((rc = wgrad_backward(cx, i))) return rc;
-            RowScope rs(i, "dgrad");
-            if ((rc = conv_dgrad_launch(cx.ws(y.g), y.e, y.c, B, cx.w(i), cx.ws(pl.wt_bwd[i]), cx.ws(pl.wu_bwd[i]), t.e, t.c, pl.pad[l], cx.ws(pl.g_ts[l]), nullptr, nullptr,
-                                        u.e, u.c, cx.ws(u.g), nullptr, st))) return rc;
+        case K_CAT:
+            if ((rc = cat_backward(cx, i))) return rc;
             break;
-        }
         case K_UP: {
             const Act &x = pl.in(L), &u = pl.u[L.level];
             if ((rc = wgrad_backward(cx, i))) return rc;
@@ -800,7 +885,11 @@
         HIP_TRY(hipEventCreateWithFlags(&h->ev_join, hipEventDisableTiming));
     }
     Ctx cx(h, pl, workspace, stream, params, grads, overlap);
+    cx.batch_reduce = g_batch_prep != 0; cx.stage = stage;
+    wgrad_reduce_defer(cx.batch_reduce ? &cx.red : nullptr);
     int rc = backward_stage_body(cx, stage, dlogits);
+    wgrad_reduce_defer(nullptr);
+    if (rc == 0) rc = stage_reduce(cx);
     cx.wst.join();
     if (rc == 0 && cx.wst.err != hipSuccess) {
         set_error("unet_backward: ordering the weight-gradient stream against the caller's failed: %s", hipGetErrorString(cx.wst.err));
diff --git a/dl-unet_amd/csrc/reduce.hip b/dl-unet_amd/csrc/reduce.hip
--- /dev/null
+++ b/dl-unet_amd/csrc/reduce.hip
@@ -0,0 +1,169 @@
+#include "common.hpp"
+#include <cstdio>
+
+namespace unet {
+
+template <int PG>
+__device__ __forceinline__ void reduce_wino_unit(const ReduceEntry &E, unsigned unit, int tid, float *redp)
+{
+    float(*red)[3][64] = (float(*)[3][64])redp;
+    const bool active = unit < E.units;
+    const int tile = (int)(unit >> 6), jb = (int)(unit & 63);
+    const int j = tid & 63, grp = tid >> 6;
+    const int nsplit = E.nP;
+    const size_t pstride = E.pstride;
+    const float *__restrict__ slab = E.slab;
+    const float *src = slab + (size_t)tile * nsplit * pstride + (size_t)jb * 64 + j;
+    float m[9];
+#pragma unroll
+    for (int x = 0; x < 9; ++x) m[x] = 0.f;
+    if (active)
+        for (int P = grp; P < nsplit; P += PG) {
+            const float *s = src + (size_t)P * pstride;
+#pragma unroll
+            for (int x = 0; x < 9; ++x) m[x] += s[x * 4096];
+        }
+#pragma unroll
+    for (int xq = 0; xq < 3; ++xq) {
+        if (xq) __syncthreads();
+#pragma unroll
+        for (int x = 0; x < 3; ++x) red[grp][x][j] = m[3 * xq + x];
+        __syncthreads();
+        if (grp == 0) {
+#pragma unroll
+            for (int x = 0; x < 3; ++x) {
+                float v = red[0][x][j];
+#pragma unroll
+                for (int g = 1; g < PG; ++g) v += red[g][x][j];
+                m[3 * xq + x] = v;
+            }
+        }
+    }
+    const int it = tile / E.ntile_j, jt = tile - it * E.ntile_j;
+    if (grp == 0 && active) {
+        float *o = E.out + (size_t)(it * 64 + j) * E.si + (size_t)(jt * 64 + jb) * E.sj;
+#pragma unroll
+        for (int t = 0; t < 9; ++t) o[t * E.st] = m[t];
+    }
+    if (E.db && (jb & ~3) == 0 && it == 0) {
+        const bool mine = jb == 0 && active;
+        __syncthreads();
+        if (mine) {
+            float v = 0.f;
+            for (int P = grp; P < nsplit; P += PG) v += slab[((size_t)tile * nsplit + P) * pstride + 9 * 64 * 64 + j];
+            red[grp][0][j] = v;
+        }
+        __syncthreads();
+        if (mine && grp == 0) {
+            float t = red[0][0][j];
+#pragma unroll
+            for (int g = 1; g < PG; ++g) t += red[g][0][j];
+            E.db[E.db_c0 + jt * 64 + j] = t;
+        }
+    }
+}
+
+template <int PG>
+__device__ __forceinline__ void reduce_direct_unit(const ReduceEntry &E, unsigned unit, int tid, f32x4 *redp)
+{
+    f32x4(*red)[64] = (f32x4(*)[64])redp;
+    const int T = E.T, nP = E.nP;
+    const size_t pstride = E.pstride;
+    const size_t nw = (size_t)T * E.Ci * E.Cj;
+    const size_t total = nw + (E.db ? (size_t)E.ndb : 0);
+    const int lane_e = tid & 63, grp = tid >> 6;
+    const size_t e = (size_t)unit * 256 + 4 * lane_e;
+    f32x4 s0 = {0.f, 0.f, 0.f, 0.f}, s1 = s0, s2 = s0, s3 = s0;
+    if (e < total) {
+        const float *src = E.slab + e;
+        int P = grp;
+        for (; P + 3 * PG < nP; P += 4 * PG) {
+            s0 += *(const f32x4 *)(src + (size_t)P * pstride);
+            s1 += *(const f32x4 *)(src + (size_t)(P + PG) * pstride);
+            s2 += *(const f32x4 *)(src + (size_t)(P + 2 * PG) * pstride);
+            s3 += *(const f32x4 *)(src + (size_t)(P + 3 * PG) * pstride);
+        }
+        for (; P < nP; P += PG) s0 += *(const f32x4 *)(src + (size_t)P * pstride);
+    }
+    red[grp][lane_e] = (s0 + s1) + (s2 + s3);
+    __syncthreads();
+    if (grp == 0 && e < total) {
+        f32x4 v = red[0][lane_e];
+#pragma unroll
+        for (int g = 1; g < PG; ++g) v += red[g][lane_e];
+        if (e < nw) {
+            const int ln = (int)((e >> 2) & 63), rq = (int)((e >> 8) & 3);
+            const size_t hi = e >> 10;
+            const int t = (int)(hi % T);
+            const int wv = (int)((hi / T) & 3);
+            const int tile = (int)(hi / T / 4);
+            const int ntj = E.Cj >> 6;
+            const int it = tile / ntj, jt = tile - it * ntj;
+            const int i0 = it * 64 + (wv >> 1) * 32 + 8 * rq + 4 * (ln >> 5);
+            const int j = jt * 64 + (wv & 1) * 32 + (ln & 31);
+#pragma unroll
+            for (int ri = 0; ri < 4; ++ri)
+                if (i0 + ri < E.ci_real && j < E.cj_real) E.out[(i0 + ri) * E.si + j * E.sj + t * E.st] = v[ri];
+        } else {
+#pragma unroll
+            for (int ri = 0; ri < 4; ++ri)
+                if (e - nw + ri < (size_t)E.ndb) E.db[e - nw + ri] = v[ri];
+        }
+    }
+}
+
+__global__ __launch_bounds__(1024) void wgrad_reduce_kernel(const ReduceTable tb)
+{
+    __shared__ f32x4 red[16 * 64];
+    int t = 0;
+    while (t + 1 < tb.n && tb.e[t + 1].b0 <= blockIdx.x) ++t;
+    const ReduceEntry &E = tb.e[t];
+    const unsigned blk = blockIdx.x - E.b0;
+    const int tid = threadIdx.x;
+    if (E.pg == 16) {
+        if (E.wino) reduce_wino_unit<16>(E, blk, tid, (float *)red);
+        else reduce_direct_unit<16>(E, blk, tid, red);
+    } else {
+        const int q = tid >> 8;
+        if (E.wino) reduce_wino_unit<4>(E, blk * 4 + q, tid & 255, (float *)(red + q * 256));
+        else reduce_direct_unit<4>(E, blk * 4 + q, tid & 255, red + q * 256);
+    }
+}
+
+static int reduce_add(ReduceTable &tb, const ReduceEntry &e, double bytes)
+{
+    ARG_CHECK(tb.n < REDUCE_MAX, "wgrad reduce: more than %d entries in one launch", REDUCE_MAX);
+    ARG_CHECK((e.pg == 4 || e.pg == 16) && e.units > 0 && e.nP > 0, "wgrad reduce: bad entry");
+    ARG_CHECK(!e.wino || e.units % 64 == 0, "wgrad reduce: a Winograd entry has 64 units per tile");
+    ReduceEntry &d = tb.e[tb.n++];
+    d = e;
+    d.b0 = tb.nblocks;
+    tb.nblocks += e.pg == 16 ? e.units : (e.units + 3) / 4;
+    tb.bytes += bytes;
+    return 0;
+}
+
+int wgrad_reduce_launch(ReduceTable &tb, hipStream_t st)
+{
+    if (!tb.n) return 0;
+    char tag[32];
+    if (tb.n == 1) snprintf(tag, sizeof(tag), "%s", tb.e[0].wino ? "wgradw_reduce" : "wgrad_reduce");
+    else snprintf(tag, sizeof(tag), "wgrad_reduce n=%d", tb.n);
+    const int rc = profiled(PK_REDUCE, tag, st, 0.0, 0.0, tb.bytes,
+                            [&] { hipLaunchKernelGGL(wgrad_reduce_kernel, dim3(tb.nblocks), dim3(1024), 0, st, tb); });
+    tb = ReduceTable();
+    return rc;
+}
+
+static thread_local ReduceTable *t_defer = nullptr;
+void wgrad_reduce_defer(ReduceTable *tb) { t_defer = tb; }
+
+int wgrad_reduce_submit(const ReduceEntry &e, double bytes, hipStream_t st)
+{
+    if (t_defer) return reduce_add(*t_defer, e, bytes);
+    ReduceTable one;
+    if (int rc = reduce_add(one, e, bytes)) return rc;
+    return wgrad_reduce_launch(one, st);
+}
+
+}
diff --git a/dl-unet_amd/csrc/wgrad.hip b/dl-unet_amd/csrc/wgrad.hip
--- a/dl-unet_amd/csrc/wgrad.hip
+++ b/dl-unet_amd/csrc/wgrad.hip
@@ -612,58 +612,6 @@
 #pragma unroll
         for (int rq = 0; rq < 4; ++rq)
             dst4[(t * 4 + rq) * 64] = f32x4{acc[t][4 * rq], acc[t][4 * rq + 1], acc[t][4 * rq + 2], acc[t][4 * rq + 3]};
-}
-
-template <int PG>
-__global__ __launch_bounds__(64 * PG) void wgrad_reduce_kernel(const float *__restrict__ slab, int nP, size_t pstride, int T, int Ci, int Cj,
-                                                               int ci_real, int cj_real,
-                                                               float *__restrict__ out, long si, long sj, long st, float *__restrict__ db, int ndb)
-{
-    const size_t nw = (size_t)T * Ci * Cj;
-    const size_t total = nw + (db ? (size_t)ndb : 0);
-    const int lane_e = threadIdx.x & 63, grp = threadIdx.x >> 6;
-    __shared__ f32x4 red[PG][64];
-    for (size_t base = (size_t)blockIdx.x * 256; base < total; base += (size_t)gridDim.x * 256) {
-        const size_t e = base + 4 * lane_e;
-        f32x4 s0 = {0.f, 0.f, 0.f, 0.f}, s1 = s0, s2 = s0, s3 = s0;
-        if (e < total) {
-            const float *src = slab + e;
-            int P = grp;
-            for (; P + 3 * PG < nP; P += 4 * PG) {
-                s0 += *(const f32x4 *)(src + (size_t)P * pstride);
-                s1 += *(const f32x4 *)(src + (size_t)(P + PG) * pstride);
-                s2 += *(const f32x4 *)(src + (size_t)(P + 2 * PG) * pstride);
-                s3 += *(const f32x4 *)(src + (size_t)(P + 3 * PG) * pstride);
-            }
-            for (; P < nP; P += PG) s0 += *(const f32x4 *)(src + (size_t)P * pstride);
-        }
-        red[grp][lane_e] = (s0 + s1) + (s2 + s3);
-        __syncthreads();
-        if (grp == 0 && e < total) {
-            f32x4 v = red[0][lane_e];
-#pragma unroll
-            for (int g = 1; g < PG; ++g) v += red[g][lane_e];
-            if (e < nw) {
-                const int ln = (int)((e >> 2) & 63), rq = (int)((e >> 8) & 3);
-                const size_t hi = e >> 10;
-                const int t = (int)(hi % T);
-                const int wv = (int)((hi / T) & 3);
-                const int tile = (int)(hi / T / 4);
-                const int ntj = Cj >> 6;
-                const int it = tile / ntj, jt = tile - it * ntj;
-                const int i0 = it * 64 + (wv >> 1) * 32 + 8 * rq + 4 * (ln >> 5);
-                const int j = jt * 64 + (wv & 1) * 32 + (ln & 31);
-#pragma unroll
-                for (int ri = 0; ri < 4; ++ri)
-                    if (i0 + ri < ci_real && j < cj_real) out[(i0 + ri) * si + j * sj + t * st] = v[ri];
-            } else {
-#pragma unroll
-                for (int ri = 0; ri < 4; ++ri)
-                    if (e - nw + ri < (size_t)ndb) db[e - nw + ri] = v[ri];
-            }
-        }
-        __syncthreads();
-    }
 }
 
 static void decompose(const WgradP &p, WgradK &k)
@@ -885,17 +833,12 @@
     if (rc) return rc;
     const int ndb = p.db ? (p.db_on_x ? ci_real : cj_real) : 0;
     const size_t total = (size_t)T * p.Ci * p.Cj + ndb;
-    size_t blocks = (total + 255) / 256;
-    if (blocks > 16384) blocks = 16384;
     ARG_CHECK(k.pstride % 4 == 0 && ndb % 4 == 0 && ((uintptr_t)p.slab & 15) == 0, "wgrad: the reduce needs 16-byte aligned slabs");
-    prof_begin(PK_REDUCE, "wgrad_reduce", st, 0.0, 0.0, (double)nP * k.pstride * 4.0 + (double)total * 4.0);
-    if (nP >= 64)
-        hipLaunchKernelGGL(wgrad_reduce_kernel<16>, dim3((unsigned)blocks), dim3(1024), 0, st, p.slab, nP, k.pstride, T, p.Ci, p.Cj, ci_real, cj_real, p.out, p.si, p.sj, p.st, p.db, ndb);
-    else
-        hipLaunchKernelGGL(wgrad_reduce_kernel<4>, dim3((unsigned)blocks), dim3(256), 0, st, p.slab, nP, k.pstride, T, p.Ci, p.Cj, ci_real, cj_real, p.out, p.si, p.sj, p.st, p.db, ndb);
-    prof_end(st);
-    HIP_TRY(hipGetLastError());
-    return 0;
-}
-
-}
+    ReduceEntry e{};
+    e.slab = p.slab; e.out = p.out; e.db = p.db; e.pstride = k.pstride; e.si = p.si; e.sj = p.sj; e.st = p.st;
+    e.wino = 0; e.pg = nP >= 64 ? 16 : 4; e.nP = nP; e.T = T; e.Ci = p.Ci; e.Cj = p.Cj; e.ci_real = ci_real; e.cj_real = cj_real; e.ndb = ndb;
+    e.units = (unsigned)((total + 255) / 256);
+    return wgrad_reduce_submit(e, (double)nP * k.pstride * 4.0 + (double)total * 4.0, st);
+}
+
+}
diff --git a/dl-unet_amd/csrc/wgradw.hip b/dl-unet_amd/csrc/wgradw.hip
--- a/dl-unet_amd/csrc/wgradw.hip
+++ b/dl-unet_amd/csrc/wgradw.hip
@@ -309,61 +309,6 @@
     }
 }
 
-template <int PG>
-__global__ __launch_bounds__(64 * PG) void wgradw_reduce_kernel(const float *__restrict__ slab, int nsplit, size_t pstride, int ntile_j,
-                                                            float *__restrict__ out, long si, long sj, long st,
-                                                            float *__restrict__ db, int db_c0)
-{
-    const int tile = blockIdx.x >> 6, jb = blockIdx.x & 63;
-    const int j = threadIdx.x & 63, grp = threadIdx.x >> 6;
-    const float *src = slab + (size_t)tile * nsplit * pstride + (size_t)jb * 64 + j;
-    float m[9];
-#pragma unroll
-    for (int x = 0; x < 9; ++x) m[x] = 0.f;
-    for (int P = grp; P < nsplit; P += PG) {
-        const float *s = src + (size_t)P * pstride;
-#pragma unroll
-        for (int x = 0; x < 9; ++x) m[x] += s[x * 4096];
-    }
-    __shared__ float red[PG][3][64];
-#pragma unroll
-    for (int xq = 0; xq < 3; ++xq) {
-        if (xq) __syncthreads();
-#pragma unroll
-        for (int x = 0; x < 3; ++x) red[grp][x][j] = m[3 * xq + x];
-        __syncthreads();
-        if (grp == 0) {
-#pragma unroll
-            for (int x = 0; x < 3; ++x) {
-                float v = red[0][x][j];
-#pragma unroll
-                for (int g = 1; g < PG; ++g) v += red[g][x][j];
-                m[3 * xq + x] = v;
-            }
-        }
-    }
-    if (grp == 0) {
-        const int it = tile / ntile_j, jt = tile - it * ntile_j;
-        float *o = out + (size_t)(it * 64 + j) * si + (size_t)(jt * 64 + jb) * sj;
-#pragma unroll
-        for (int t = 0; t < 9; ++t) o[t * st] = m[t];
-    }
-    if (db && jb == 0 && (tile / ntile_j) == 0) {
-        __syncthreads();
-        const int jt = tile % ntile_j;
-        float v = 0.f;
-        for (int P = grp; P < nsplit; P += PG) v += slab[((size_t)tile * nsplit + P) * pstride + 9 * 64 * 64 + j];
-        red[grp][0][j] = v;
-        __syncthreads();
-        if (grp == 0) {
-            float t = red[0][0][j];
-#pragma unroll
-            for (int g = 1; g < PG; ++g) t += red[g][0][j];
-            db[db_c0 + jt * 64 + j] = t;
-        }
-    }
-}
-
 bool wgradw_applicable(const WgradP &p)
 {
     if (p.TY != 3 || p.TX != 3 || p.stride != 1) return false;
@@ -419,16 +364,11 @@
     char tag[96];
     snprintf(tag, sizeof(tag), "wgradw<%d> Ci=%d Cj=%d Y=%dx%d tiles=%dx%d steps=%d split=%d", (int)buf, p.Ci, p.Cj, p.YH, p.YW, k.TYn, k.TXn, k.nsteps, k.nsplit);
     if (int rc_ = launch(ntile * k.nsplit, 512, WW_LDS, st, PK_WGRAD, tag, wgrad_alg_flops(p), 2.0 * k.nsteps * 16.0 * 16.0 * p.Ci * p.Cj, wgrad_alg_bytes(p), k)) return rc_;
-    prof_begin(PK_REDUCE, "wgradw_reduce", st, 0.0, 0.0, (double)ntile * k.nsplit * k.pstride * 4.0 + 9.0 * p.Ci * p.Cj * 4.0);
-    if (ntile <= 4 && k.nsplit >= 32)
-        hipLaunchKernelGGL(wgradw_reduce_kernel<16>, dim3(ntile * 64), dim3(1024), 0, st, p.slab, k.nsplit, k.pstride, k.ntile_j,
-                           p.out, p.si, p.sj, p.st, p.db, p.yc0);
-    else
-        hipLaunchKernelGGL(wgradw_reduce_kernel<4>, dim3(ntile * 64), dim3(256), 0, st, p.slab, k.nsplit, k.pstride, k.ntile_j,
-                           p.out, p.si, p.sj, p.st, p.db, p.yc0);
-    prof_end(st);
-    HIP_TRY(hipGetLastError());
-    return 0;
-}
-
-}
+    ReduceEntry e{};
+    e.slab = p.slab; e.out = p.out; e.db = p.db; e.pstride = k.pstride; e.si = p.si; e.sj = p.sj; e.st = p.st;
+    e.wino = 1; e.pg = ntile <= 4 && k.nsplit >= 32 ? 16 : 4; e.nP = k.nsplit; e.ntile_j = k.ntile_j; e.db_c0 = p.yc0;
+    e.units = (unsigned)ntile * 64;
+    return wgrad_reduce_submit(e, (double)ntile * k.nsplit * k.pstride * 4.0 + 9.0 * p.Ci * p.Cj * 4.0, st);
+}
+
+}
diff --git a/dl-unet_amd/csrc/wino.hip b/dl-unet_amd/csrc/wino.hip
--- a/dl-unet_amd/csrc/wino.hip
+++ b/dl-unet_amd/csrc/wino.hip
@@ -17,54 +17,78 @@
 };
 
 
-__global__ __launch_bounds__(256) void wino_transform_ref_kernel(const float *__restrict__ w, int I, int dgrad, int n0, int Nn, int k0, int Kc,
-                                                                 float *__restrict__ U)
-{
-    const size_t total = (size_t)Nn * Kc;
-    const size_t idx = (size_t)blockIdx.x * 256 + threadIdx.x;
-    if (idx >= total) return;
-    int n, c;
-    if (dgrad) { c = (int)(idx / Nn); n = (int)(idx - (size_t)c * Nn); }
-    else       { n = (int)(idx / Kc); c = (int)(idx - (size_t)n * Kc); }
-    const int o = dgrad ? k0 + c : n0 + n, i = dgrad ? n0 + n : k0 + c;
-    const float *src = w + ((size_t)o * I + i) * 9;
-    float g[3][3];
-#pragma unroll
-    for (int t = 0; t < 9; ++t) g[t / 3][t % 3] = src[dgrad ? 8 - t : t];
-    float r[4][3];
-#pragma unroll
-    for (int j = 0; j < 3; ++j) {
-        r[0][j] = g[0][j];
-        r[1][j] = 0.5f * (g[0][j] + g[1][j] + g[2][j]);
-        r[2][j] = 0.5f * (g[0][j] - g[1][j] + g[2][j]);
-        r[3][j] = g[2][j];
-    }
-    float u[16];
-#pragma unroll
-    for (int a = 0; a < 4; ++a) {
-        u[4 * a + 0] = r[a][0];
-        u[4 * a + 1] = 0.5f * (r[a][0] + r[a][1] + r[a][2]);
-        u[4 * a + 2] = 0.5f * (r[a][0] - r[a][1] + r[a][2]);
-        u[4 * a + 3] = r[a][2];
-    }
-    const int nsteps = Kc >> 3;
-    const int nt = n >> 6, n16 = (n >> 4) & 3, nl = n & 15;
-    const int step = c >> 3, kk = c & 7, kg = kk >> 1, h = kk & 1;
-    float *blk = U + ((size_t)nt * nsteps + step) * 8192;
-#pragma unroll
-    for (int xg = 0; xg < 4; ++xg) {
-        f32x4 v = {u[4 * xg], u[4 * xg + 1], u[4 * xg + 2], u[4 * xg + 3]};
-        *(f32x4 *)(blk + ((n16 * 4 + xg) * 2 + h) * 256 + (kg * 16 + nl) * 4) = v;
-    }
-}
-
-int wino_transform_ref(const float *w_oihw, int I, int dgrad, int n0, int Nn, int k0, int Kc, float *U, hipStream_t st)
-{
-    ARG_CHECK(w_oihw && U && Nn % 32 == 0 && Kc % 8 == 0 && Kc > 0, "wino_transform_ref: bad shape");
-    const size_t total = (size_t)Nn * Kc;
-    hipLaunchKernelGGL(wino_transform_ref_kernel, dim3((unsigned)((total + 255) / 256)), dim3(256), 0, st, w_oihw, I, dgrad, n0, Nn, k0, Kc, U);
-    HIP_TRY(hipGetLastError());
+__device__ __forceinline__ int wino_xf_slot(int p, int lane) { return p * 64 + (lane ^ ((((p >> 3) * 2 + (p & 1)) * 2) & 15)); }
+
+__global__ __launch_bounds__(256) void wino_transform_kernel(const WinoXformTable tb)
+{
+    __shared__ f32x4 stage[32 * 64];
+    int t = 0;
+    while (t + 1 < tb.n && tb.e[t + 1].b0 <= blockIdx.x) ++t;
+    const float *__restrict__ w = tb.e[t].w;
+    float *__restrict__ U = tb.e[t].U;
+    const int I = tb.e[t].I, dgrad = tb.e[t].dgrad, n0 = tb.e[t].n0, k0 = tb.e[t].k0;
+    const int nsteps = tb.e[t].Kc >> 3, nsg = (nsteps + 3) >> 2;
+    const int unit = (int)(blockIdx.x - tb.e[t].b0);
+    const int n16g = unit / nsg, sg = unit - n16g * nsg;
+    const int steps = nsteps - 4 * sg < 4 ? nsteps - 4 * sg : 4;
+    const int ncol = 8 * steps;
+    for (int e = threadIdx.x; e < 16 * ncol; e += 256) {
+        int nl, cl;
+        if (dgrad) { cl = e >> 4; nl = e & 15; }
+        else       { nl = e / ncol; cl = e - nl * ncol; }
+        const int n = n16g * 16 + nl, c = sg * 32 + cl;
+        const int o = dgrad ? k0 + c : n0 + n, i = dgrad ? n0 + n : k0 + c;
+        const float *src = w + ((size_t)o * I + i) * 9;
+        float g[3][3];
+#pragma unroll
+        for (int q = 0; q < 9; ++q) g[q / 3][q % 3] = src[dgrad ? 8 - q : q];
+        float r[4][3];
+#pragma unroll
+        for (int j = 0; j < 3; ++j) {
+            r[0][j] = g[0][j];
+            r[1][j] = 0.5f * (g[0][j] + g[1][j] + g[2][j]);
+            r[2][j] = 0.5f * (g[0][j] - g[1][j] + g[2][j]);
+            r[3][j] = g[2][j];
+        }
+        float u[16];
+#pragma unroll
+        for (int a = 0; a < 4; ++a) {
+            u[4 * a + 0] = r[a][0];
+            u[4 * a + 1] = 0.5f * (r[a][0] + r[a][1] + r[a][2]);
+            u[4 * a + 2] = 0.5f * (r[a][0] - r[a][1] + r[a][2]);
+            u[4 * a + 3] = r[a][2];
+        }
+        const int sl = cl >> 3, kk = cl & 7, kg = kk >> 1, h = kk & 1;
+#pragma unroll
+        for (int xg = 0; xg < 4; ++xg) {
+            f32x4 v = {u[4 * xg], u[4 * xg + 1], u[4 * xg + 2], u[4 * xg + 3]};
+            stage[wino_xf_slot((sl * 4 + xg) * 2 + h, kg * 16 + nl)] = v;
+        }
+    }
+    __syncthreads();
+    const int nt = n16g >> 2, n16 = n16g & 3;
+    const int wave = threadIdx.x >> 6, lane = threadIdx.x & 63;
+    for (int p = wave; p < 8 * steps; p += 4) {
+        float *blk = U + ((size_t)nt * nsteps + 4 * sg + (p >> 3)) * 8192;
+        *(f32x4 *)(blk + (n16 * 8 + (p & 7)) * 256 + lane * 4) = stage[wino_xf_slot(p, lane)];
+    }
+}
+
+int wino_transform_add(WinoXformTable &tb, const float *w_oihw, int I, int dgrad, int n0, int Nn, int k0, int Kc, float *U)
+{
+    ARG_CHECK(w_oihw && U && Nn % 32 == 0 && Kc % 8 == 0 && Kc > 0, "wino_transform: bad shape");
+    ARG_CHECK(tb.n < WINO_XF_MAX, "wino_transform: more than %d sub-matrices in one launch", WINO_XF_MAX);
+    tb.e[tb.n++] = WinoXform{w_oihw, U, I, dgrad, n0, Nn, k0, Kc, tb.nblocks};
+    tb.nblocks += (unsigned)(Nn / 16) * (unsigned)((Kc / 8 + 3) / 4);
+    tb.bytes += (double)Nn * Kc * (9 + 16) * 4.0;
     return 0;
+}
+
+int wino_transform_launch(const WinoXformTable &tb, hipStream_t st)
+{
+    if (!tb.n) return 0;
+    return profiled(PK_ELEMWISE, "wino_transform", st, 0.0, 0.0, tb.bytes,
+                    [&] { hipLaunchKernelGGL(wino_transform_kernel, dim3(tb.nblocks), dim3(256), 0, st, tb); });
 }
 
 constexpr int WINO_ROW = 72 * 32;
diff --git a/include/unet_hip.h b/include/unet_hip.h
--- a/include/unet_hip.h
+++ b/include/unet_hip.h
@@ -52,6 +52,7 @@
 int unet_backward(unet_handle *h, const void *const *params, const void *dlogits,
                   void *const *grads, void *workspace, size_t workspace_bytes, void *stream);
 int unet_set_overlap(int on);
+int unet_set_batch_prep(int on);
 int unet_backward_stages(void);
 int unet_backward_stage(unet_handle *h, int stage, const void *const *params,
                         const void *dlogits, void *const *grads, void *workspace,
```

Result: no change. 255.9 tiles/s (median of 6 runs) (+0.3%).
